# alpenlabs/dv-pari

Hardware: AMD Instinct MI355X
Metric: R1CS constraints/sec (prove) (higher is better)
Workload: dtype u32; 1 GPU; Proof::prove, synthetic dense R1CS, 2^20 constraints (BASELINE config #4); log2_constraints=20, n_wires=1048576, msm_pairs_per_proof=6291456, witness=resident in HBM, entry=dvp_prove_dev (Proof::prove with the witness resident), proofs_in_flight=1

## Files before the change

### dv-pari_amd/_native.py

```python
import ctypes as C
import os

import numpy as np

_HERE = os.path.dirname(os.path.abspath(__file__))
LIB_PATH = os.environ.get("DVP_LIB") or os.path.join(_HERE, "libdvpari_hip.so")

if not os.environ.get("DVP_NO_TORCH_PRELOAD"):
    try:
        import torch
    except Exception:
        pass

if not os.path.exists(LIB_PATH):
    raise ImportError(
        f"{LIB_PATH} is missing: build it with `python -c 'import __graft_entry__ as g; g.build()'` "
        "(hipcc --offload-arch=gfx950).  dv-pari_amd has no CPU fallback."
    )
lib = C.CDLL(LIB_PATH)

vp, u32, u64p, u8p, sz = C.c_void_p, C.c_uint32, C.c_void_p, C.c_void_p, C.c_size_t

_SIGS = {
    "dvp_strerror": (C.c_char_p, [C.c_int]),
    "dvp_version": (C.c_int, []),
    "dvp_device_count": (C.c_int, []),
    "dvp_set_device": (C.c_int, [C.c_int]),
    "dvp_set_devices": (C.c_int, [C.POINTER(C.c_int), C.c_int]),
    "dvp_points_sum_dev": (C.c_int, [vp, u32, vp, vp, vp]),
    "dvp_last_error_index": (C.c_int64, []),
    "dvp_tune_set": (C.c_int, [C.c_char_p, C.c_longlong]),
    "dvp_tune_get": (C.c_int, [C.c_char_p, C.POINTER(C.c_longlong)]),
    "dvp_tune_reset": (None, []),
    "dvp_ubench_gather": (C.c_int, [vp, C.c_size_t, C.c_int, C.POINTER(C.c_double)]),
    "dvp_prover_msm_table_ptr": (C.c_int, [vp, C.c_int, C.POINTER(vp), C.POINTER(C.c_uint64)]),
    "dvp_debug_ecfft_matrices": (C.c_int, [vp, C.c_int, C.c_int, u64p]),
    "dvp_debug_ecfft_layer": (C.c_int, [vp, u32, u64p]),
    "dvp_ubench_gf_mul": (C.c_int, [C.c_int, C.POINTER(C.c_double)]),
    "dvp_ubench_fr_mul": (C.c_int, [C.c_int, C.POINTER(C.c_double)]),
    "dvp_setup_scalars": (C.c_int, [u64p, u64p, u64p, u32, u32, u32, u32, u64p, u32, C.POINTER(vp), C.POINTER(vp), C.POINTER(vp), u64p, sz]),
    "dvp_debug_wave_trace": (C.c_int, [vp, u32]),
    "dvp_profile_enable": (None, [C.c_int]),
    "dvp_profile_reset": (None, []),
    "dvp_profile_read": (C.c_int, [C.c_char_p, C.POINTER(C.c_double), C.POINTER(C.c_uint64)]),
    "dvp_profile_round0_shapes": (C.c_int, [C.POINTER(C.c_uint64), C.POINTER(C.c_double), C.POINTER(C.c_uint64), C.c_int]),
    "dvp_ecfft_create": (C.c_int, [u32, C.c_int, u32, C.POINTER(vp)]),
    "dvp_ecfft_destroy": (None, [vp]),
    "dvp_ecfft_log2_leaves": (u32, [vp]),
    "dvp_ecfft_leaves": (C.c_int, [vp, u64p]),
    "dvp_ecfft_extend": (C.c_int, [vp, u64p, u32, u64p]),
    "dvp_ecfft_extend_dev": (C.c_int, [vp, vp, u32, vp, vp]),
    "dvp_ecfft_enter": (C.c_int, [vp, u64p, u64p]),
    "dvp_ecfft_exit": (C.c_int, [vp, u64p, u64p]),
    "dvp_ecfft_enter_dev": (C.c_int, [vp, vp, vp, vp]),
    "dvp_ecfft_exit_dev": (C.c_int, [vp, vp, vp, vp]),
    "dvp_ecfft_vanish_at": (C.c_int, [vp, C.c_int, u64p, u64p]),
    "dvp_fr_batch_inverse": (C.c_int, [u64p, sz]),
    "dvp_fr_batch_inverse_dev": (C.c_int, [vp, sz, vp]),
    "dvp_fr_vec_mul": (C.c_int, [u64p, u64p, sz, u64p]),
    "dvp_fr_vec_scale": (C.c_int, [u64p, u64p, sz, u64p]),
    "dvp_fr_vec_scalar_sub": (C.c_int, [u64p, u64p, sz, u64p]),
    "dvp_fr_vec_axpy": (C.c_int, [u64p, u64p, u64p, sz, u64p]),
    "dvp_fr_vec_dot": (C.c_int, [u64p, u64p, sz, u64p]),
    "dvp_fr_spmv": (C.c_int, [vp, vp, vp, u32, u64p, u32, u64p, u32, u64p]),
    "dvp_barycentric_eval": (C.c_int, [u64p, u64p, u64p, u64p, sz, u64p, u64p]),
    "dvp_msm_affine": (C.c_int, [u64p, u64p, u8p, sz, u64p, C.POINTER(C.c_int)]),
    "dvp_msm_affine_dev": (C.c_int, [vp, vp, vp, sz, vp, vp, vp]),
    "dvp_msm_ctx_create": (C.c_int, [u64p, u8p, sz, sz, C.POINTER(vp)]),
    "dvp_msm_ctx_destroy": (None, [vp]),
    "dvp_msm_ctx_plan": (C.c_int, [vp, C.POINTER(C.c_int), C.POINTER(C.c_int)]),
    "dvp_msm_ctx_table_bytes": (C.c_uint64, [vp, C.POINTER(C.c_int)]),
    "dvp_debug_recode_signed": (C.c_int, [vp, C.c_size_t, C.c_int, vp, C.POINTER(C.c_int)]),
    "dvp_msm_ctx_run": (C.c_int, [vp, u64p, sz, sz, u64p, C.POINTER(C.c_int)]),
    "dvp_msm_ctx_run_dev": (C.c_int, [vp, vp, sz, sz, vp, vp, vp]),
    "dvp_msm_xsk233": (C.c_int, [u8p, u8p, sz, u8p]),
    "dvp_mulgen_batch": (C.c_int, [u64p, sz, u8p]),
    "dvp_mulgen_batch_affine": (C.c_int, [u64p, sz, u64p, u8p]),
    "dvp_points_encode": (C.c_int, [u64p, u8p, sz, u8p]),
    "dvp_points_decode": (C.c_int, [u8p, sz, u64p, u8p]),
    "dvp_codec_set_rule": (C.c_int, [C.c_int]),
    "dvp_codec_get_rule": (C.c_int, []),
    "dvp_points_add": (C.c_int, [u64p, u8p, u64p, u8p, sz, u64p, u8p]),
    "dvp_prover_create": (C.c_int, [u32, u32, u32, C.POINTER(vp)]),
    "dvp_prover_destroy": (None, [vp]),
    "dvp_prover_set_coeffs": (C.c_int, [vp, u64p, u32]),
    "dvp_prover_set_matrix": (C.c_int, [vp, C.c_int, u32, vp, vp, vp]),
    "dvp_prover_set_srs_encoded": (C.c_int, [vp, C.c_int, u8p, sz]),
    "dvp_prover_set_srs_affine": (C.c_int, [vp, C.c_int, u64p, u8p, sz]),
    "dvp_prover_set_srs_affine_dev": (C.c_int, [vp, C.c_int, vp, vp, sz]),
    "dvp_prove": (C.c_int, [vp, u64p, u32, u64p, u32, u8p]),
    "dvp_prove_dev": (C.c_int, [vp, vp, u8p, vp]),
    "dvp_prove_begin": (C.c_int, [vp, vp, vp]),
    "dvp_prove_begin_partial": (C.c_int, [vp, vp, C.c_int, vp]),
    "dvp_prover_extend_count": (u32, [vp]),
    "dvp_prove_extend_vectors": (C.c_int, [vp, u32, vp]),
    "dvp_prover_extended_ptr": (C.c_int, [vp, u32, C.POINTER(vp)]),
    "dvp_prove_quotient": (C.c_int, [vp, vp]),
    "dvp_prove_mark_extended": (C.c_int, [vp, u32]),
    "dvp_prover_msm_size": (C.c_size_t, [vp, C.c_int]),
    "dvp_prover_msm_plan": (C.c_int, [vp, C.c_int, C.POINTER(C.c_int), C.POINTER(C.c_int)]),
    "dvp_prover_msm_table_bytes": (C.c_uint64, [vp, C.c_int, C.POINTER(C.c_int)]),
    "dvp_prover_msm_partial": (C.c_int, [vp, C.c_int, sz, sz, vp, vp, vp]),
    "dvp_prove_challenge": (C.c_int, [vp, vp, vp, vp]),
    "dvp_prove_challenge_partial": (C.c_int, [vp, vp, vp, C.c_size_t, C.c_size_t, C.c_size_t, C.c_size_t, vp, vp]),
    "dvp_prove_challenge_finish": (C.c_int, [vp, vp, C.c_uint32, C.c_size_t, C.c_size_t, vp]),
    "dvp_prove_finish": (C.c_int, [vp, vp, vp, u8p, vp]),
    "dvp_prover_debug_read": (C.c_int, [vp, C.c_char_p, u64p, sz]),
    "dvp_prover_debug_transcript_dev": (C.c_int, [vp, u8p, u64p, u32, u64p, u64p]),
    "dvp_prover_domains": (C.c_int, [vp, u64p, u64p]),
    "dvp_prover_domain_tables": (C.c_int, [vp, C.c_int, u64p, u64p]),
    "dvp_ecfft_domain_tables": (C.c_int, [vp, C.c_int, u64p, u64p]),
    "dvp_file_fr_vec_write": (C.c_int, [C.c_char_p, u64p, sz]),
    "dvp_file_fr_vec_read": (C.c_int, [C.c_char_p, u64p, sz, C.POINTER(C.c_size_t)]),
    "dvp_file_point_vec_write": (C.c_int, [C.c_char_p, u8p, sz]),
    "dvp_file_point_vec_read": (C.c_int, [C.c_char_p, u8p, sz, C.POINTER(C.c_size_t)]),
    "dvp_file_witness_read": (C.c_int, [C.c_char_p, u64p, sz, C.POINTER(C.c_size_t)]),
    "dvp_file_witness_write": (C.c_int, [C.c_char_p, u64p, sz]),
    "dvp_r1cs_dump_sizes": (C.c_int, [u8p, sz, C.POINTER(u32), C.POINTER(u32), C.POINTER(C.c_uint64 * 3), C.POINTER(u32)]),
    "dvp_r1cs_dump_fill": (C.c_int, [u8p, sz, u64p, C.POINTER(vp * 3), C.POINTER(vp * 3), C.POINTER(vp * 3)]),
    "dvp_fftr_sections": (C.c_int, [C.c_char_p, u32, u8p, u64p, C.POINTER(u32)]),
    "dvp_fftr_read_fr": (C.c_int, [C.c_char_p, u32, C.c_uint8, u64p, sz, C.POINTER(C.c_size_t)]),
    "dvp_fftr_write": (C.c_int, [C.c_char_p, u32, u8p, vp, u64p]),
    "dvp_setup_cache_dir": (C.c_int, [u64p, u64p, u64p, C.c_char_p, u32, C.c_int]),
    "dvp_setup_cache_dir_ex": (C.c_int, [u64p, u64p, u64p, C.c_char_p, u32, C.c_int, u64p, sz, C.POINTER(u32), C.POINTER(u32)]),
    "dvp_prover_prepares_precomputes": (C.c_int, [C.c_char_p, C.c_int, C.POINTER(u32)]),
    "dvp_ecfft_write_tree_file": (C.c_int, [vp, C.c_char_p]),
    "dvp_ecfft_check_tree_file": (C.c_int, [vp, C.c_char_p, C.c_int, C.POINTER(C.c_int), C.POINTER(C.c_int64)]),
    "dvp_prover_open_cache_dir": (C.c_int, [C.c_char_p, u32, C.POINTER(vp)]),
    "dvp_prove_cache_dir": (C.c_int, [C.c_char_p, u64p, u32, u64p, u32, u8p]),
    "dvp_cache_dir_release": (None, [C.c_char_p]),
    "dvp_cache_dir_prover": (C.c_int, [C.c_char_p, u32, C.POINTER(vp)]),
    "dvp_transcript_challenge": (C.c_int, [u8p, u64p, u32, u64p]),
    "dvp_blake3": (C.c_int, [u8p, sz, u8p]),
    "dvp_verify": (C.c_int, [u64p, u64p, u64p, u64p, u32, u8p, C.POINTER(C.c_int), C.POINTER(C.c_uint32)]),
    "dvp_verify_batch": (C.c_int, [u64p, u64p, u64p, u64p, u32, u8p, sz, u8p]),
    "dvp_verify_batch_dev": (C.c_int, [u64p, u64p, u64p, vp, u32, vp, sz, vp, vp]),
    "dvp_verify_batch_rlc": (C.c_int, [u64p, u64p, u64p, u64p, u32, u8p, sz, u8p, u8p, C.POINTER(C.c_uint32)]),
    "dvp_verify_batch_rlc_dev": (C.c_int, [u64p, u64p, u64p, vp, u32, vp, sz, u8p, vp, vp, vp]),
    "dvp_sp1_public_input": (C.c_int, [C.c_uint64, u64p]),
}
EXPORTED = []
for _name, (_res, _args) in _SIGS.items():
    try:
        _f = getattr(lib, _name)
    except AttributeError:
        continue
    _f.restype, _f.argtypes = _res, _args
    EXPORTED.append(_name)


class DvpError(RuntimeError):
    def __init__(self, status, where=""):
        self.status = status
        self.index = lib.dvp_last_error_index()
        super().__init__(f"{where}: {lib.dvp_strerror(status).decode()} (status {status}, index {self.index})")


def check(status, where=""):
    if status != 0:
        raise DvpError(status, where)


def set_devices(ids):
    ids = list(ids or [])
    arr = (C.c_int * max(len(ids), 1))(*ids)
    check(lib.dvp_set_devices(arr, len(ids)), "dvp_set_devices")


class tune:

    def __init__(self, **knobs):
        self.knobs = knobs
        self.saved = {}

    def __enter__(self):
        for k, v in self.knobs.items():
            old = C.c_longlong(0)
            check(lib.dvp_tune_get(k.encode(), C.byref(old)), f"dvp_tune_get({k})")
            self.saved[k] = old.value
            check(lib.dvp_tune_set(k.encode(), int(v)), f"dvp_tune_set({k})")
        return self

    def __exit__(self, *exc):
        for k, v in self.saved.items():
            lib.dvp_tune_set(k.encode(), v)
        self.saved = {}
        return False


def ints_to_limbs(vals, words=4) -> np.ndarray:
    out = np.empty((len(vals), words), dtype=np.uint64)
    buf = b"".join(int(v).to_bytes(8 * words, "little") for v in vals)
    out[:] = np.frombuffer(buf, dtype="<u8").reshape(len(vals), words)
    return out


def limbs_to_ints(arr) -> list:
    a = np.ascontiguousarray(arr, dtype="<u8")
    a = a.reshape(-1, a.shape[-1])
    w = a.shape[1] * 8
    raw = a.tobytes()
    return [int.from_bytes(raw[i * w:(i + 1) * w], "little") for i in range(a.shape[0])]


def ptr(a: np.ndarray):
    assert a.flags["C_CONTIGUOUS"]
    return a.ctypes.data_as(C.c_void_p)
```

### dv-pari_amd/csrc/capi.cpp

```cpp
#include "common.h"

#include <atomic>
#include <map>
#include <mutex>
#include <vector>
#include <cstring>
#include <cstdlib>

namespace dvp {
thread_local int64_t g_last_error_index = -1;
thread_local hipError_t g_last_hip_error = hipSuccess;

bool g_prof_enabled = false;
static unsigned g_prof_mask = ~0u;
static std::mutex g_prof_mu;
static double g_prof_ms[PROF_NSLOTS] = {0};
static uint64_t g_prof_n[PROF_NSLOTS] = {0};
struct Pending { int slot; hipEvent_t e0, e1; uint64_t key; };
struct Shape { double ms = 0; uint64_t n = 0; };
static std::map<uint64_t, Shape> g_prof_round0;
static std::vector<Pending> g_prof_pending;
static const char* kProfNames[PROF_NSLOTS] = {"msm_affine_round0", "msm_total", "extend_total", "prove_total", "msm_affine_rest", "msm_sort", "msm_tail"};

ProfScope::ProfScope(int slot_, hipStream_t st_, uint64_t key_) : slot(slot_), st(st_), key(key_) {
  if (!g_prof_enabled || slot_ < 0 || !((g_prof_mask >> slot_) & 1u)) return;
  if (hipEventCreate(&e0) != hipSuccess || hipEventCreate(&e1) != hipSuccess) { e0 = e1 = nullptr; return; }
  (void)hipEventRecord(e0, st);
}
void ProfScope::stop() {
  if (!e0) return;
  (void)hipEventRecord(e1, st);
  std::lock_guard<std::mutex> g(g_prof_mu);
  g_prof_pending.push_back({slot, e0, e1, key});
  e0 = e1 = nullptr;
}
void prof_collect() {
  std::lock_guard<std::mutex> g(g_prof_mu);
  for (auto& p : g_prof_pending) {
    float ms = 0;
    if (hipEventSynchronize(p.e1) == hipSuccess && hipEventElapsedTime(&ms, p.e0, p.e1) == hipSuccess) {
      g_prof_ms[p.slot] += ms;
      g_prof_n[p.slot] += (p.slot == PROF_MSM_AFFINE_REST && p.key) ? p.key : 1;
      if (p.slot == PROF_MSM_ACCUM_AFFINE && p.key) { Shape& sh = g_prof_round0[p.key]; sh.ms += ms; sh.n += 1; }
    }
    (void)hipEventDestroy(p.e0);
    (void)hipEventDestroy(p.e1);
  }
  g_prof_pending.clear();
}

static std::atomic<uint64_t> g_host_waits[2];
void count_host_wait(int kind) { g_host_waits[kind & 1].fetch_add(1, std::memory_order_relaxed); }

static void tune_from_env(Tune& t) {
  t = Tune();
  auto geti = [](const char* name, long long dflt) { const char* e = getenv(name); return e ? atoll(e) : dflt; };
  t.msm_c = geti("DVP_MSM_C", t.msm_c);
  t.msm_k = geti("DVP_MSM_K", t.msm_k);
  t.msm_fixed_c = geti("DVP_MSM_FIXED_C", t.msm_fixed_c);
  t.fx_hi = geti("DVP_FX_HI", t.fx_hi);
  const char* m = getenv("DVP_MSM_MODE");
  t.msm_proj = (m && !strcmp(m, "proj")) ? 1 : 0;
  t.msm_aff_min = geti("DVP_MSM_AFF_MIN", t.msm_aff_min);
  t.msm_hex_max = geti("DVP_MSM_HEX_MAX", t.msm_hex_max);
  t.msm_round_pipeline = geti("DVP_MSM_ROUND_PIPELINE", t.msm_round_pipeline);
  t.msm_sort_fused = geti("DVP_MSM_SORT_FUSED", t.msm_sort_fused);
  t.msm_bucket_pairs_max = geti("DVP_MSM_BUCKET_PAIRS_MAX", t.msm_bucket_pairs_max);
  t.msm_aff_bmax = geti("DVP_MSM_AFF_BMAX", t.msm_aff_bmax);
  t.msm_aff_bmin = geti("DVP_MSM_AFF_BMIN", t.msm_aff_bmin);
  t.ecfft_radix4 = geti("DVP_ECFFT_RADIX4", t.ecfft_radix4);
  t.ecfft_fold = geti("DVP_ECFFT_FOLD", t.ecfft_fold);
  t.msm_accum_fast = geti("DVP_MSM_ACCUM_FAST", t.msm_accum_fast);
  t.msm_tail_groups = geti("DVP_MSM_TAIL_GROUPS", t.msm_tail_groups);
  t.msm_accum_hex_max = geti("DVP_MSM_ACCUM_HEX_MAX", t.msm_accum_hex_max);
  t.gf_inv_tabs = geti("DVP_GF_INV_TABS", t.gf_inv_tabs);
  t.msm_ws_slots = geti("DVP_MSM_WS_SLOTS", t.msm_ws_slots);
  t.msm_gate_min = geti("DVP_MSM_GATE_MIN", t.msm_gate_min);
  t.msm_aff_tpb = geti("DVP_MSM_AFF_TPB", t.msm_aff_tpb);
  t.cache_replicas = geti("DVP_CACHE_REPLICAS", t.cache_replicas);
  t.msm_quad_max = geti("DVP_MSM_QUAD_MAX", t.msm_quad_max);
  t.msm_accum_quad_max = geti("DVP_MSM_ACCUM_QUAD_MAX", t.msm_accum_quad_max);
  t.msm_fixed_min = geti("DVP_MSM_FIXED_MIN", t.msm_fixed_min);
  t.horner_max_pub = geti("DVP_HORNER_MAX_PUB", t.horner_max_pub);
  t.fr_bi_shape = geti("DVP_FR_BI_SHAPE", t.fr_bi_shape);
  t.msm_aligned_signed = geti("DVP_MSM_ALIGNED_SIGNED", t.msm_aligned_signed);
  t.prove_host_transcript = geti("DVP_PROVE_HOST_TRANSCRIPT", t.prove_host_transcript);
}
static std::mutex g_dev_mu;
static std::vector<int> g_devices;
std::vector<int> mgpu_devices() {
  std::lock_guard<std::mutex> g(g_dev_mu);
  return g_devices;
}
Tune& tune() {
  static Tune t = [] { Tune x; tune_from_env(x); return x; }();
  return t;
}
}

static long long* tune_slot(const char* name) {
  dvp::Tune& t = dvp::tune();
  struct { const char* n; long long* v; } tab[] = {
      {"DVP_MSM_C", &t.msm_c}, {"DVP_MSM_K", &t.msm_k}, {"DVP_MSM_FIXED_C", &t.msm_fixed_c}, {"DVP_FX_HI", &t.fx_hi},
      {"DVP_MSM_PROJ", &t.msm_proj}, {"DVP_MSM_AFF_MIN", &t.msm_aff_min}, {"DVP_MSM_HEX_MAX", &t.msm_hex_max}, {"DVP_MSM_ROUND_PIPELINE", &t.msm_round_pipeline}, {"DVP_MSM_SORT_FUSED", &t.msm_sort_fused}, {"DVP_MSM_BUCKET_PAIRS_MAX", &t.msm_bucket_pairs_max}, {"DVP_MSM_AFF_BMAX", &t.msm_aff_bmax}, {"DVP_MSM_AFF_BMIN", &t.msm_aff_bmin}, {"DVP_ECFFT_RADIX4", &t.ecfft_radix4}, {"DVP_ECFFT_FOLD", &t.ecfft_fold}, {"DVP_MSM_ACCUM_FAST", &t.msm_accum_fast}, {"DVP_MSM_TAIL_GROUPS", &t.msm_tail_groups}, {"DVP_MSM_ACCUM_HEX_MAX", &t.msm_accum_hex_max}, {"DVP_GF_INV_TABS", &t.gf_inv_tabs}, {"DVP_MSM_WS_SLOTS", &t.msm_ws_slots}, {"DVP_MSM_GATE_MIN", &t.msm_gate_min}, {"DVP_MSM_AFF_TPB", &t.msm_aff_tpb}, {"DVP_CACHE_REPLICAS", &t.cache_replicas},
      {"DVP_MSM_QUAD_MAX", &t.msm_quad_max}, {"DVP_MSM_ACCUM_QUAD_MAX", &t.msm_accum_quad_max}, {"DVP_MSM_FIXED_MIN", &t.msm_fixed_min}, {"DVP_HORNER_MAX_PUB", &t.horner_max_pub}, {"DVP_FR_BI_SHAPE", &t.fr_bi_shape},
      {"DVP_MSM_ALIGNED_SIGNED", &t.msm_aligned_signed}, {"DVP_PROVE_HOST_TRANSCRIPT", &t.prove_host_transcript}};
  for (auto& e : tab)
    if (!strcmp(name, e.n)) return e.v;
  return nullptr;
}
extern "C" int dvp_tune_set(const char* name, long long value) {
  long long* v = name ? tune_slot(name) : nullptr;
  if (!v) return DVP_EINVAL;
  *v = value;
  return DVP_OK;
}
extern "C" int dvp_tune_get(const char* name, long long* value) {
  long long* v = name ? tune_slot(name) : nullptr;
  if (!v || !value) return DVP_EINVAL;
  *value = *v;
  return DVP_OK;
}
extern "C" void dvp_tune_reset(void) { dvp::tune_from_env(dvp::tune()); }

extern "C" void dvp_profile_enable(int on) {
  dvp::g_prof_mask = on == 2 ? (1u << dvp::PROF_MSM_ACCUM_AFFINE) : ~0u;
  dvp::g_prof_enabled = on != 0;
}
extern "C" void dvp_profile_reset(void) {
  dvp::prof_collect();
  std::lock_guard<std::mutex> g(dvp::g_prof_mu);
  for (int i = 0; i < dvp::PROF_NSLOTS; ++i) { dvp::g_prof_ms[i] = 0; dvp::g_prof_n[i] = 0; }
  dvp::g_prof_round0.clear();
  dvp::g_host_waits[0] = 0;
  dvp::g_host_waits[1] = 0;
}
extern "C" int dvp_profile_round0_shapes(uint64_t* pairs, double* total_ms, uint64_t* launches, int cap) {
  if (cap < 0 || (cap > 0 && (!pairs || !total_ms || !launches))) return DVP_EINVAL;
  dvp::prof_collect();
  std::lock_guard<std::mutex> g(dvp::g_prof_mu);
  int k = 0;
  for (auto& e : dvp::g_prof_round0) {
    if (k < cap) { pairs[k] = e.first; total_ms[k] = e.second.ms; launches[k] = e.second.n; }
    ++k;
  }
  return k;
}
extern "C" int dvp_profile_read(const char* name, double* total_ms, uint64_t* launches) {
  if (!name || !total_ms || !launches) return DVP_EINVAL;
  if (!strcmp(name, "host_waits_stream") || !strcmp(name, "host_waits_side")) {
    *total_ms = 0;
    *launches = dvp::g_host_waits[name[11] == 's' && name[12] == 'i' ? 1 : 0].load();
    return DVP_OK;
  }
  dvp::prof_collect();
  std::lock_guard<std::mutex> g(dvp::g_prof_mu);
  for (int i = 0; i < dvp::PROF_NSLOTS; ++i)
    if (!strcmp(name, dvp::kProfNames[i])) { *total_ms = dvp::g_prof_ms[i]; *launches = dvp::g_prof_n[i]; return DVP_OK; }
  return DVP_EINVAL;
}

extern "C" const char* dvp_strerror(int s) {
  switch (s) {
    case DVP_OK: return "ok";
    case DVP_EINVAL: return "invalid argument (size, null pointer or non-canonical field element)";
    case DVP_EDECODE: return "invalid xsk233 point encoding";
    case DVP_EUNSAT: return "R1CS constraint not satisfied by the witness";
    case DVP_EHIP: return "HIP runtime error";
    case DVP_EIO: return "I/O error";
    case DVP_ENOMEM: return "out of memory";
    case DVP_ECHALLENGE: return "Fiat-Shamir challenge lies in the evaluation domain";
    default: return "unknown status";
  }
}

extern "C" int dvp_version(void) { return 100; }

extern "C" int dvp_device_count(void) {
  int n = 0;
  hipError_t e = hipGetDeviceCount(&n);
  if (e != hipSuccess) return DVP_EHIP;
  return n;
}

extern "C" int dvp_set_devices(const int* ids, int n) {
  int cnt = 0;
  DVP_HIP(hipGetDeviceCount(&cnt));
  if (n < 0 || n > 64 || (n > 0 && !ids)) return DVP_EINVAL;
  for (int i = 0; i < n; ++i)
    if (ids[i] < 0 || ids[i] >= cnt) return DVP_EINVAL;
  std::lock_guard<std::mutex> g(dvp::g_dev_mu);
  dvp::g_devices.assign(ids, ids + (n > 1 ? n : 0));
  return DVP_OK;
}

extern "C" int dvp_set_device(int id) {
  DVP_HIP(hipSetDevice(id));
  return DVP_OK;
}

extern "C" int64_t dvp_last_error_index(void) { return dvp::g_last_error_index; }
```

### dv-pari_amd/csrc/common.h

```cpp
#pragma once
#include <hip/hip_runtime.h>
#include <stdint.h>
#include <stdio.h>

#include <vector>

#include "../../include/dvpari_internal.h"

namespace dvp {

extern thread_local int64_t g_last_error_index;
extern thread_local hipError_t g_last_hip_error;

inline int hip_fail(hipError_t e, const char* what, const char* file, int line) {
  g_last_hip_error = e;
  fprintf(stderr, "[dvpari] HIP error %d (%s) at %s:%d: %s\n", (int)e, hipGetErrorString(e), file, line, what);
  return DVP_EHIP;
}

#define DVP_HIP(call)                                                        \
  do {                                                                       \
    hipError_t _e = (call);                                                  \
    if (_e != hipSuccess) return ::dvp::hip_fail(_e, #call, __FILE__, __LINE__); \
  } while (0)

#define DVP_TRY(call)        \
  do {                       \
    int _s = (call);         \
    if (_s != DVP_OK) return _s; \
  } while (0)

struct DevBuf {
  void* p = nullptr;
  size_t bytes = 0;
  DevBuf() = default;
  DevBuf(const DevBuf&) = delete;
  DevBuf& operator=(const DevBuf&) = delete;
  ~DevBuf() { release(); }
  int alloc(size_t n) {
    release();
    if (n == 0) n = 16;
    hipError_t e = hipMalloc(&p, n);
    if (e != hipSuccess) {
      p = nullptr;
      return hip_fail(e, "hipMalloc", __FILE__, __LINE__);
    }
    bytes = n;
    return DVP_OK;
  }
  void release() {
    if (p) (void)hipFree(p);
    p = nullptr;
    bytes = 0;
  }
  template <class T>
  T* as() const {
    return reinterpret_cast<T*>(p);
  }
};

struct Tune {
  long long msm_c = 0;
  long long msm_k = 0;
  long long msm_fixed_c = 0;
  long long fx_hi = -1;
  long long msm_proj = 0;
  long long msm_aff_min = 1ll << 19;
  long long msm_gate_min = 1;
  long long msm_ws_slots = 2;
  long long cache_replicas = 1;
  long long msm_aff_tpb = 256;
  long long msm_aff_bmin = 8;
  long long msm_aff_bmax = 136;
  long long ecfft_radix4 = 3;
  long long ecfft_fold = 1;
  long long msm_accum_fast = 1;
  long long msm_tail_groups = 1;
  long long msm_accum_hex_max = -1;
  long long gf_inv_tabs = 1;
  long long msm_accum_quad_max = 0;
  long long msm_bucket_pairs_max = 12;
  long long msm_sort_fused = 1;
  long long msm_round_pipeline = 2;
  long long msm_hex_max = -1;
  long long msm_quad_max = 0;
  long long msm_fixed_min = 1ll << 16;
  long long fr_bi_shape = 6;
  long long horner_max_pub = -1;
  long long prove_host_transcript = 0;
  long long msm_aligned_signed = 1;
};
Tune& tune();

std::vector<int> mgpu_devices();

inline unsigned cdiv(size_t a, size_t b) { return (unsigned)((a + b - 1) / b); }

enum ProfSlot { PROF_MSM_ACCUM_AFFINE = 0, PROF_MSM_TOTAL, PROF_EXTEND_TOTAL, PROF_PROVE_TOTAL, PROF_MSM_AFFINE_REST, PROF_MSM_SORT, PROF_MSM_TAIL, PROF_NSLOTS };
extern bool g_prof_enabled;
struct ProfScope {
  int slot;
  hipStream_t st;
  hipEvent_t e0 = nullptr, e1 = nullptr;
  uint64_t key = 0;
  ProfScope(int slot_, hipStream_t st_, uint64_t key_ = 0);
  void stop();
};
void prof_collect();
void count_host_wait(int kind);

}
```

### dv-pari_amd/csrc/msm.hip

```cpp
#include <algorithm>
#include <cstdlib>
#include <cstring>
#include <atomic>
#include <chrono>
#include <mutex>
#include <type_traits>
#include <vector>

#include "common.h"
#include "k233.cuh"
#include "tau.cuh"
#include "codec.cuh"

namespace dvp {

constexpr uint32_t FXW_VALID = 0x80000000u, FXW_KEY_MASK = 0xfffffu, FXW_NEG = 0x10000000u, ITEM_NEG = 0x80000000u;
constexpr int FXW_ROW_SHIFT = 20;
__host__ __device__ __forceinline__ uint32_t fxw_key(uint32_t d) { return d & FXW_KEY_MASK; }
__host__ __device__ __forceinline__ uint32_t fxw_row(uint32_t d) { return (d >> FXW_ROW_SHIFT) & 0xffu; }

template <class DIGIT>
__global__ void __launch_bounds__(256)
k_recode(const uint32_t* __restrict__ scalars, const uint8_t* __restrict__ inf, uint32_t n, int c, int W, int n_narrow,
         DIGIT* __restrict__ digits, unsigned long long* __restrict__ err) {
  uint32_t i = blockIdx.x * blockDim.x + threadIdx.x;
  if (i >= n) return;
  uint32_t s[8];
#pragma unroll
  for (int k = 0; k < 8; ++k) s[k] = scalars[(size_t)i * 8 + k];
  bool skip = inf && inf[i];
  if (!tau_scalar_is_canonical(s)) {
    atomicMin(err, (unsigned long long)i);
    skip = true;
  }
  uint32_t r0[5], r1[5];
  tau_partial_reduce(s, r0, r1);
  if (skip) {
#pragma unroll
    for (int k = 0; k < 5; ++k) r0[k] = r1[k] = 0;
  }
  const int total = W * c - n_narrow;
  uint64_t buf = 0;
  int nb = 0, w = 0, width = n_narrow > 0 ? c - 1 : c;
  for (int done = 0; done < total; done += 16) {
    buf |= (uint64_t)tau_step16(r0, r1) << nb;
    nb += 16;
    while (nb >= width && w < W) {
      const uint32_t dv = (uint32_t)(buf & ((1ull << width) - 1));
      if (sizeof(DIGIT) == 4)
        digits[(size_t)w * n + i] = (DIGIT)(dv ? (FXW_VALID | ((uint32_t)w << FXW_ROW_SHIFT) | dv) : 0u);
      else
        digits[(size_t)w * n + i] = (DIGIT)dv;
      buf >>= width;
      nb -= width;
      ++w;
      width = w < n_narrow ? c - 1 : c;
    }
  }
  uint32_t rest = (uint32_t)buf | (uint32_t)(buf >> 32);
#pragma unroll
  for (int k = 0; k < 5; ++k) rest |= r0[k] | r1[k];
  if (rest) atomicMin(err, (unsigned long long)i | (1ull << 62));
}

template <class F>
__device__ __forceinline__ uint32_t fx_recode_signed_each(const uint32_t* s , int c, int W, int n_narrow, F&& f) {
  uint32_t carry = 0;
  int bit = 0;
#pragma unroll 1
  for (int w = 0; w < W; ++w) {
    const int width = w < n_narrow ? c - 1 : c;
    const uint32_t half = 1u << (width - 1), mask = (1u << width) - 1;
    const int wd = bit >> 5, sh = bit & 31;
    uint32_t lo = wd < 8 ? s[wd] : 0u, hi = wd + 1 < 9 ? s[wd + 1] : 0u;
    uint32_t d = (uint32_t)((((uint64_t)hi << 32) | lo) >> sh) & mask;
    bit += width;
    d += carry;
    carry = 0;
    uint32_t word = 0;
    if (d > mask) {
      carry = 1;
    } else if (d > half) {
      carry = 1;
      d = (1u << width) - d;
      word = FXW_VALID | FXW_NEG | ((uint32_t)w << FXW_ROW_SHIFT) | d;
    } else if (d) {
      word = FXW_VALID | ((uint32_t)w << FXW_ROW_SHIFT) | (d & ((1u << (c - 1)) - 1));
    }
    f(w, word);
  }
  return carry;
}
__device__ __forceinline__ bool fx_load_scalar(const uint32_t* __restrict__ scalars, const uint8_t* __restrict__ inf, uint32_t i, uint32_t* s,
                                               unsigned long long* __restrict__ err, bool report) {
#pragma unroll
  for (int k = 0; k < 8; ++k) s[k] = scalars[(size_t)i * 8 + k];
  s[8] = 0;
  bool skip = inf && inf[i];
  if (!tau_scalar_is_canonical(s)) {
    if (report) atomicMin(err, (unsigned long long)i);
    skip = true;
  }
  return !skip;
}
__global__ void __launch_bounds__(256)
k_recode_signed(const uint32_t* __restrict__ scalars, const uint8_t* __restrict__ inf, uint32_t n, int c, int W, int n_narrow,
                uint32_t* __restrict__ words, unsigned long long* __restrict__ err) {
  uint32_t i = blockIdx.x * blockDim.x + threadIdx.x;
  if (i >= n) return;
  uint32_t s[9];
  const bool live = fx_load_scalar(scalars, inf, i, s, err, true);
  const uint32_t carry = fx_recode_signed_each(s, c, W, n_narrow, [&](int w, uint32_t word) { words[(size_t)w * n + i] = live ? word : 0u; });
  if (carry && live) atomicMin(err, (unsigned long long)i | (1ull << 62));
}

constexpr int SCAN_TPB = 256, SCAN_EPT = 4, SCAN_BLK = SCAN_TPB * SCAN_EPT;

template <int NW>
__device__ __forceinline__ uint32_t block_scan_waves(uint32_t v, uint32_t* total, uint32_t* sh) {
  const int t = threadIdx.x, lane = t & 63, w = t >> 6;
  uint32_t x = v;
#pragma unroll
  for (int o = 1; o < 64; o <<= 1) {
    const uint32_t y = (uint32_t)__shfl_up((int)x, o);
    if (lane >= o) x += y;
  }
  if (lane == 63) sh[w] = x;
  __syncthreads();
  if (w == 0) {
    uint32_t z = lane < NW ? sh[lane] : 0u;
#pragma unroll
    for (int o = 1; o < NW; o <<= 1) {
      const uint32_t y = (uint32_t)__shfl_up((int)z, o);
      if (lane >= o) z += y;
    }
    if (lane < NW) sh[16 + lane] = z;
  }
  __syncthreads();
  const uint32_t base = w ? sh[16 + w - 1] : 0u;
  *total = sh[16 + NW - 1];
  __syncthreads();
  return base + x - v;
}
__device__ __forceinline__ uint32_t block_exclusive_scan(uint32_t v, uint32_t* total, uint32_t* sh) {
  return block_scan_waves<SCAN_TPB / 64>(v, total, sh);
}

template <bool PAD2>
__global__ void __launch_bounds__(SCAN_TPB) k_scan_local(const uint32_t* __restrict__ in, uint32_t* __restrict__ out,
                                                         uint32_t* __restrict__ bsum, uint32_t m) {
  __shared__ uint32_t sh[SCAN_TPB];
  uint32_t base = blockIdx.x * SCAN_BLK + threadIdx.x * SCAN_EPT;
  uint32_t v[SCAN_EPT], s = 0;
#pragma unroll
  for (int k = 0; k < SCAN_EPT; ++k) {
    v[k] = (base + k < m) ? in[base + k] : 0;
    if (PAD2) v[k] = (v[k] + 1u) & ~1u;
    s += v[k];
  }
  uint32_t tot;
  uint32_t ex = block_exclusive_scan(s, &tot, sh);
#pragma unroll
  for (int k = 0; k < SCAN_EPT; ++k) {
    if (base + k < m) out[base + k] = ex;
    ex += v[k];
  }
  if (threadIdx.x == 0) bsum[blockIdx.x] = tot;
}

__global__ void __launch_bounds__(SCAN_TPB) k_scan_local_div(const uint32_t* __restrict__ in, uint32_t K, uint32_t* __restrict__ vout,
                                                             uint32_t* __restrict__ out, uint32_t* __restrict__ bsum, uint32_t m) {
  __shared__ uint32_t sh[SCAN_TPB];
  uint32_t base = blockIdx.x * SCAN_BLK + threadIdx.x * SCAN_EPT;
  uint32_t v[SCAN_EPT], s = 0;
#pragma unroll
  for (int k = 0; k < SCAN_EPT; ++k) {
    v[k] = (base + k < m) ? (in[base + k] + K - 1) / K : 0;
    if (base + k < m) vout[base + k] = v[k];
    s += v[k];
  }
  uint32_t tot;
  uint32_t ex = block_exclusive_scan(s, &tot, sh);
#pragma unroll
  for (int k = 0; k < SCAN_EPT; ++k) {
    if (base + k < m) out[base + k] = ex;
    ex += v[k];
  }
  if (threadIdx.x == 0) bsum[blockIdx.x] = tot;
}

__global__ void __launch_bounds__(SCAN_TPB) k_scan_bsums(uint32_t* __restrict__ bsum, uint32_t nb, uint32_t* total_out) {
  __shared__ uint32_t sh[SCAN_TPB];
  uint32_t carry = 0;
  for (uint32_t base = 0; base < nb; base += SCAN_TPB) {
    uint32_t idx = base + threadIdx.x;
    uint32_t v = idx < nb ? bsum[idx] : 0;
    uint32_t tot;
    uint32_t ex = block_exclusive_scan(v, &tot, sh);
    if (idx < nb) bsum[idx] = ex + carry;
    carry += tot;
  }
  if (threadIdx.x == 0) *total_out = carry;
}

__global__ void __launch_bounds__(SCAN_TPB) k_scan_add(uint32_t* __restrict__ out, const uint32_t* __restrict__ bsum, uint32_t m) {
  uint32_t base = blockIdx.x * SCAN_BLK + threadIdx.x * SCAN_EPT;
  uint32_t add = bsum[blockIdx.x];
#pragma unroll
  for (int k = 0; k < SCAN_EPT; ++k)
    if (base + k < m) out[base + k] += add;
}

constexpr uint32_t SCAN_FOLD_NB = 64;
__global__ void __launch_bounds__(SCAN_TPB) k_scan_add_fold(uint32_t* __restrict__ out, const uint32_t* __restrict__ bsum_raw, uint32_t m,
                                                           uint32_t* __restrict__ total_out) {
  uint32_t add = 0;
  for (uint32_t b = 0; b < blockIdx.x; ++b) add += bsum_raw[b];
  const uint32_t base = blockIdx.x * SCAN_BLK + threadIdx.x * SCAN_EPT;
#pragma unroll
  for (int k = 0; k < SCAN_EPT; ++k)
    if (base + k < m) out[base + k] += add;
  if (blockIdx.x == gridDim.x - 1 && threadIdx.x == 0) *total_out = add + bsum_raw[blockIdx.x];
}

static int scan_exclusive(const uint32_t* in, uint32_t* out, uint32_t m, uint32_t* bsum, hipStream_t st, bool pad2 = false) {
  uint32_t nb = cdiv(m, SCAN_BLK);
  if (pad2)
    hipLaunchKernelGGL(k_scan_local<true>, dim3(nb), dim3(SCAN_TPB), 0, st, in, out, bsum, m);
  else
    hipLaunchKernelGGL(k_scan_local<false>, dim3(nb), dim3(SCAN_TPB), 0, st, in, out, bsum, m);
  if (nb <= SCAN_FOLD_NB)
    hipLaunchKernelGGL(k_scan_add_fold, dim3(nb), dim3(SCAN_TPB), 0, st, out, bsum, m, out + m);
  else {
    hipLaunchKernelGGL(k_scan_bsums, dim3(1), dim3(SCAN_TPB), 0, st, bsum, nb, out + m);
    hipLaunchKernelGGL(k_scan_add, dim3(nb), dim3(SCAN_TPB), 0, st, out, bsum, m);
  }
  DVP_HIP(hipGetLastError());
  return DVP_OK;
}

static int scan_exclusive_div(const uint32_t* in, uint32_t K, uint32_t* vout, uint32_t* out, uint32_t m, uint32_t* bsum, hipStream_t st) {
  uint32_t nb = cdiv(m, SCAN_BLK);
  hipLaunchKernelGGL(k_scan_local_div, dim3(nb), dim3(SCAN_TPB), 0, st, in, K, vout, out, bsum, m);
  if (nb <= SCAN_FOLD_NB)
    hipLaunchKernelGGL(k_scan_add_fold, dim3(nb), dim3(SCAN_TPB), 0, st, out, bsum, m, out + m);
  else {
    hipLaunchKernelGGL(k_scan_bsums, dim3(1), dim3(SCAN_TPB), 0, st, bsum, nb, out + m);
    hipLaunchKernelGGL(k_scan_add, dim3(nb), dim3(SCAN_TPB), 0, st, out, bsum, m);
  }
  DVP_HIP(hipGetLastError());
  return DVP_OK;
}

constexpr uint32_t SORT_CHUNK = 32768;
constexpr int SORT_TPB = 1024;

__global__ void __launch_bounds__(SORT_TPB)
k_hist_local(const uint16_t* __restrict__ digits, uint32_t n, int c, uint16_t* __restrict__ hist) {
  extern __shared__ uint32_t lds_cnt[];
  const uint32_t chunk = blockIdx.x, w = blockIdx.y, nb = 1u << c, nchunks = gridDim.x;
  for (uint32_t k = threadIdx.x; k < (nb >> 1); k += SORT_TPB) lds_cnt[k] = 0;
  __syncthreads();
  uint32_t lo = chunk * SORT_CHUNK, hi = min(n, lo + SORT_CHUNK);
  const uint16_t* dg = digits + (size_t)w * n;
  for (uint32_t i = lo + threadIdx.x; i < hi; i += SORT_TPB) {
    uint32_t d = dg[i];
    if (d) atomicAdd(&lds_cnt[d >> 1], 1u << (16 * (d & 1)));
  }
  __syncthreads();
  uint32_t* out = (uint32_t*)(hist + ((size_t)w * nchunks + chunk) * nb);
  for (uint32_t k = threadIdx.x; k < (nb >> 1); k += SORT_TPB) out[k] = lds_cnt[k];
}

__global__ void __launch_bounds__(256)
k_hist_scan(const uint16_t* __restrict__ hist, uint32_t nchunks, int c, int W, uint32_t* __restrict__ chunk_off,
            uint32_t* __restrict__ cnt) {
  uint32_t key = blockIdx.x * blockDim.x + threadIdx.x;
  uint32_t nb = 1u << c;
  if (key >= ((uint32_t)W << c)) return;
  uint32_t w = key >> c, b = key & (nb - 1);
  uint32_t run = 0;
  for (uint32_t ch = 0; ch < nchunks; ++ch) {
    size_t idx = ((size_t)w * nchunks + ch) * nb + b;
    uint32_t v = hist[idx];
    chunk_off[idx] = run;
    run += v;
  }
  cnt[key] = run;
}

__global__ void __launch_bounds__(SORT_TPB)
k_scatter_local(const uint16_t* __restrict__ digits, uint32_t n, int c, const uint32_t* __restrict__ off,
                const uint32_t* __restrict__ chunk_off, uint32_t* __restrict__ items) {
  extern __shared__ uint32_t lds_cur[];
  const uint32_t chunk = blockIdx.x, w = blockIdx.y, nb = 1u << c, nchunks = gridDim.x;
  const uint32_t* co = chunk_off + ((size_t)w * nchunks + chunk) * nb;
  const uint32_t* of = off + ((size_t)w << c);
  for (uint32_t k = threadIdx.x; k < nb; k += SORT_TPB) lds_cur[k] = of[k] + co[k];
  __syncthreads();
  uint32_t lo = chunk * SORT_CHUNK, hi = min(n, lo + SORT_CHUNK);
  const uint16_t* dg = digits + (size_t)w * n;
  for (uint32_t i = lo + threadIdx.x; i < hi; i += SORT_TPB) {
    uint32_t d = dg[i];
    if (d) items[atomicAdd(&lds_cur[d], 1u)] = i;
  }
}

constexpr int FX_C_MAX = 20, FX_NP_MAX = 1 << (FX_C_MAX / 2);
constexpr uint32_t FX_CHUNK = 8192;
struct FxBits {
  int lo, hi;
  __host__ __device__ uint32_t np() const { return 1u << hi; }
};

__global__ void __launch_bounds__(SORT_TPB)
k_part_hist(const uint32_t* __restrict__ digits, size_t total, FxBits fb, uint32_t* __restrict__ phist) {
  __shared__ uint32_t h[FX_NP_MAX];
  const uint32_t FX_NP = fb.np();
  const int FX_LO = fb.lo;
  for (uint32_t k = threadIdx.x; k < FX_NP; k += SORT_TPB) h[k] = 0;
  __syncthreads();
  size_t lo = (size_t)blockIdx.x * FX_CHUNK, hi = min(total, lo + FX_CHUNK);
  for (size_t e = lo + threadIdx.x; e < hi; e += SORT_TPB) {
    uint32_t d = digits[e];
    if (d) atomicAdd(&h[fxw_key(d) >> FX_LO], 1u);
  }
  __syncthreads();
  for (uint32_t k = threadIdx.x; k < FX_NP; k += SORT_TPB) phist[(size_t)blockIdx.x * FX_NP + k] = h[k];
}
constexpr uint32_t FX_SCAN_CB = 32;
__global__ void __launch_bounds__(256)
k_part_scan_chunks(const uint32_t* __restrict__ phist, uint32_t nblk, FxBits fb, uint32_t* __restrict__ pbase, uint32_t* __restrict__ ctot, uint32_t nch) {
  const uint32_t FX_NP = fb.np();
  const uint32_t ch = blockIdx.x, b0 = ch * FX_SCAN_CB, b1 = min(nblk, b0 + FX_SCAN_CB);
  for (uint32_t part = threadIdx.x; part < FX_NP; part += 256) {
    uint32_t run = 0;
#pragma unroll 8
    for (uint32_t b = b0; b < b1; ++b) {
      const uint32_t v = phist[(size_t)b * FX_NP + part];
      pbase[(size_t)b * FX_NP + part] = run;
      run += v;
    }
    ctot[(size_t)part * nch + ch] = run;
  }
}
__global__ void __launch_bounds__(256)
k_part_scan_totals(uint32_t* __restrict__ ctot, uint32_t nch, FxBits fb, uint32_t* __restrict__ pcount) {
  const uint32_t part = (blockIdx.x * 256 + threadIdx.x) >> 6, lane = threadIdx.x & 63u;
  if (part >= fb.np()) return;
  uint32_t* row = ctot + (size_t)part * nch;
  uint32_t carry = 0;
  for (uint32_t base = 0; base < nch; base += 64) {
    const uint32_t idx = base + lane;
    const uint32_t v = idx < nch ? row[idx] : 0;
    uint32_t x = v;
#pragma unroll
    for (int o = 1; o < 64; o <<= 1) {
      const uint32_t y = __shfl_up(x, o);
      if ((int)lane >= o) x += y;
    }
    if (idx < nch) row[idx] = carry + x - v;
    carry += __shfl(x, 63);
  }
  if (lane == 0) pcount[part] = carry;
}
__global__ void __launch_bounds__(FX_NP_MAX)
k_part_starts(const uint32_t* __restrict__ pcount, FxBits fb, uint32_t* __restrict__ pstart, uint32_t* __restrict__ cstart) {
  __shared__ uint32_t sp[FX_NP_MAX], sc[FX_NP_MAX];
  const uint32_t FX_NP = fb.np(), t = threadIdx.x;
  uint32_t pc = t < FX_NP ? pcount[t] : 0, cc = (pc + FX_CHUNK - 1) / FX_CHUNK;
  sp[t] = pc;
  sc[t] = cc;
  __syncthreads();
  for (uint32_t o = 1; o < FX_NP_MAX; o <<= 1) {
    uint32_t a = t >= o ? sp[t - o] : 0, b = t >= o ? sc[t - o] : 0;
    __syncthreads();
    sp[t] += a;
    sc[t] += b;
    __syncthreads();
  }
  if (t < FX_NP) {
    pstart[t] = sp[t] - pc;
    cstart[t] = sc[t] - cc;
  }
  if (t == FX_NP - 1) {
    pstart[FX_NP] = sp[t];
    cstart[FX_NP] = sc[t];
  }
}
__global__ void __launch_bounds__(SORT_TPB)
k_part_scatter(const uint32_t* __restrict__ digits, size_t total, uint32_t n, uint32_t n_total, uint32_t i0, FxBits fb,
               const uint32_t* __restrict__ pbase, const uint32_t* __restrict__ cbase, uint32_t nch, const uint32_t* __restrict__ pstart,
               uint16_t* __restrict__ plo, uint32_t* __restrict__ pid) {
  __shared__ uint32_t cur[FX_NP_MAX];
  const uint32_t FX_NP = fb.np();
  const int FX_LO = fb.lo;
  const uint32_t ch = blockIdx.x / FX_SCAN_CB;
  for (uint32_t k = threadIdx.x; k < FX_NP; k += SORT_TPB) cur[k] = pstart[k] + cbase[(size_t)k * nch + ch] + pbase[(size_t)blockIdx.x * FX_NP + k];
  __syncthreads();
  size_t lo = (size_t)blockIdx.x * FX_CHUNK, hi = min(total, lo + FX_CHUNK);
  for (size_t e = lo + threadIdx.x; e < hi; e += SORT_TPB) {
    uint32_t d = digits[e];
    if (!d) continue;
    const uint32_t i = (uint32_t)(e % n), key = fxw_key(d);
    uint32_t pos = atomicAdd(&cur[key >> FX_LO], 1u);
    plo[pos] = (uint16_t)(key & ((1u << FX_LO) - 1));
    pid[pos] = (fxw_row(d) * n_total + i0 + i) | ((d & FXW_NEG) ? ITEM_NEG : 0u);
  }
}
__device__ __forceinline__ uint32_t fx_chunk_partition(const uint32_t* __restrict__ cstart, uint32_t FX_NP, uint32_t g) {
  uint32_t lo = 0, hi = FX_NP;
  while (hi - lo > 1) {
    uint32_t mid = (lo + hi) >> 1;
    if (cstart[mid] <= g) lo = mid; else hi = mid;
  }
  return lo;
}
__global__ void __launch_bounds__(SORT_TPB)
k_hist_local2(const uint16_t* __restrict__ plo, const uint32_t* __restrict__ pstart, const uint32_t* __restrict__ cstart, FxBits fb,
              uint16_t* __restrict__ hist) {
  extern __shared__ uint32_t lds_cnt[];
  const uint32_t FX_NP = fb.np();
  const uint32_t g = blockIdx.x, nb = 1u << fb.lo;
  if (g >= cstart[FX_NP]) return;
  for (uint32_t k = threadIdx.x; k < (nb >> 1); k += SORT_TPB) lds_cnt[k] = 0;
  __syncthreads();
  uint32_t hi = fx_chunk_partition(cstart, FX_NP, g);
  uint32_t lo_e = pstart[hi] + (g - cstart[hi]) * FX_CHUNK, hi_e = min(pstart[hi + 1], lo_e + FX_CHUNK);
  auto count = [&](uint32_t d) { atomicAdd(&lds_cnt[d >> 1], 1u << (16 * (d & 1))); };
  const uint32_t body_lo = min(hi_e, (lo_e + 7u) & ~7u), body_hi = max(body_lo, hi_e & ~7u);
  for (uint32_t j = lo_e + threadIdx.x; j < body_lo; j += SORT_TPB) count(plo[j]);
  for (uint32_t j = body_lo + 8u * threadIdx.x; j < body_hi; j += 8u * SORT_TPB) {
    const uint4 v = *(const uint4*)(plo + j);
    count(v.x & 0xffffu); count(v.x >> 16); count(v.y & 0xffffu); count(v.y >> 16);
    count(v.z & 0xffffu); count(v.z >> 16); count(v.w & 0xffffu); count(v.w >> 16);
  }
  for (uint32_t j = body_hi + threadIdx.x; j < hi_e; j += SORT_TPB) count(plo[j]);
  __syncthreads();
  uint32_t* out = (uint32_t*)(hist + (size_t)g * nb);
  for (uint32_t k = threadIdx.x; k < (nb >> 1); k += SORT_TPB) out[k] = lds_cnt[k];
}
__global__ void __launch_bounds__(256)
k_hist_scan2(const uint16_t* __restrict__ hist, const uint32_t* __restrict__ cstart, FxBits fb, uint32_t* __restrict__ chunk_off,
             uint32_t* __restrict__ cnt) {
  uint32_t key = blockIdx.x * blockDim.x + threadIdx.x;
  if (key >= (1u << (fb.lo + fb.hi))) return;
  const uint32_t nb = 1u << fb.lo;
  uint32_t hi = key >> fb.lo, b = key & (nb - 1);
  uint32_t run = 0;
  for (uint32_t g = cstart[hi]; g < cstart[hi + 1]; ++g) {
    size_t idx = (size_t)g * nb + b;
    uint32_t v = hist[idx];
    chunk_off[idx] = run;
    run += v;
  }
  cnt[key] = run;
}
__global__ void __launch_bounds__(SORT_TPB)
k_scatter_local2(const uint16_t* __restrict__ plo, const uint32_t* __restrict__ pid, const uint32_t* __restrict__ pstart,
                 const uint32_t* __restrict__ cstart, FxBits fb, const uint32_t* __restrict__ off, const uint32_t* __restrict__ chunk_off,
                 uint32_t* __restrict__ items) {
  extern __shared__ uint32_t lds_cur[];
  const uint32_t FX_NP = fb.np();
  const int FX_LO = fb.lo;
  const uint32_t g = blockIdx.x, nb = 1u << FX_LO;
  if (g >= cstart[FX_NP]) return;
  uint32_t hi = fx_chunk_partition(cstart, FX_NP, g);
  const uint32_t* co = chunk_off + (size_t)g * nb;
  const uint32_t* of = off + ((size_t)hi << FX_LO);
  for (uint32_t k = threadIdx.x; k < nb; k += SORT_TPB) lds_cur[k] = of[k] + co[k];
  __syncthreads();
  uint32_t lo_e = pstart[hi] + (g - cstart[hi]) * FX_CHUNK, hi_e = min(pstart[hi + 1], lo_e + FX_CHUNK);
  for (uint32_t j = lo_e + threadIdx.x; j < hi_e; j += SORT_TPB) items[atomicAdd(&lds_cur[plo[j]], 1u)] = pid[j];
}

__device__ __forceinline__ uint32_t block_scan_tpb(uint32_t v, uint32_t* sh, uint32_t* total) {
  return block_scan_waves<SORT_TPB / 64>(v, total, sh);
}
constexpr unsigned FX_STAGE1_LDS = (2 * FX_NP_MAX + SORT_TPB + 2 * FX_CHUNK) * 4;
constexpr unsigned FX_STAGE2_LDS = (2 * FX_NP_MAX + SORT_TPB + FX_CHUNK) * 4 + FX_CHUNK * 2;

__global__ void __launch_bounds__(SORT_TPB)
k_part_scatter_staged(const uint32_t* __restrict__ digits, size_t total, uint32_t n, uint32_t n_total, uint32_t i0, FxBits fb,
                      const uint32_t* __restrict__ phist, const uint32_t* __restrict__ pbase, const uint32_t* __restrict__ cbase, uint32_t nch,
                      const uint32_t* __restrict__ pstart, uint16_t* __restrict__ plo, uint32_t* __restrict__ pid) {
  extern __shared__ uint32_t lds_st[];
  uint32_t* cur = lds_st;
  uint32_t* gdst = cur + FX_NP_MAX;
  uint32_t* sh = gdst + FX_NP_MAX;
  uint32_t* st_d = sh + SORT_TPB;
  uint32_t* st_id = st_d + FX_CHUNK;
  const uint32_t FX_NP = fb.np(), t = threadIdx.x;
  const int FX_LO = fb.lo;
  const size_t hb = (size_t)blockIdx.x * FX_NP;
  uint32_t h = t < FX_NP ? phist[hb + t] : 0, tot;
  uint32_t ex = block_scan_tpb(h, sh, &tot);
  if (t < FX_NP) {
    cur[t] = ex;
    gdst[t] = pstart[t] + cbase[(size_t)t * nch + blockIdx.x / FX_SCAN_CB] + pbase[hb + t] - ex;
  }
  __syncthreads();
  const size_t lo = (size_t)blockIdx.x * FX_CHUNK, hi = min(total, lo + FX_CHUNK);
  const uint32_t w0 = (uint32_t)(lo / n);
  for (size_t e = lo + t; e < hi; e += SORT_TPB) {
    uint32_t d = digits[e];
    if (!d) continue;
    size_t i = e - (size_t)w0 * n;
    while (i >= n) i -= n;
    const uint32_t key = fxw_key(d);
    uint32_t pos = atomicAdd(&cur[key >> FX_LO], 1u);
    st_d[pos] = key;
    st_id[pos] = (fxw_row(d) * n_total + i0 + (uint32_t)i) | ((d & FXW_NEG) ? ITEM_NEG : 0u);
  }
  __syncthreads();
  const uint32_t mask = (1u << FX_LO) - 1;
  for (uint32_t pos = t; pos < tot; pos += SORT_TPB) {
    uint32_t d = st_d[pos], dst = gdst[d >> FX_LO] + pos;
    plo[dst] = (uint16_t)(d & mask);
    pid[dst] = st_id[pos];
  }
}

__global__ void __launch_bounds__(SORT_TPB)
k_part_hist_signed(const uint32_t* __restrict__ scalars, const uint8_t* __restrict__ inf, uint32_t n, int c, int W, int n_narrow, uint32_t S,
                   FxBits fb, uint32_t* __restrict__ phist, unsigned long long* __restrict__ err) {
  __shared__ uint32_t h[FX_NP_MAX];
  const uint32_t FX_NP = fb.np();
  const int FX_LO = fb.lo;
  for (uint32_t k = threadIdx.x; k < FX_NP; k += SORT_TPB) h[k] = 0;
  __syncthreads();
  const uint32_t lo = blockIdx.x * S, hi = min(n, lo + S);
  for (uint32_t i = lo + threadIdx.x; i < hi; i += SORT_TPB) {
    uint32_t s[9];
    if (!fx_load_scalar(scalars, inf, i, s, err, true)) continue;
    const uint32_t carry = fx_recode_signed_each(s, c, W, n_narrow, [&](int, uint32_t word) {
      if (word) atomicAdd(&h[fxw_key(word) >> FX_LO], 1u);
    });
    if (carry) atomicMin(err, (unsigned long long)i | (1ull << 62));
  }
  __syncthreads();
  for (uint32_t k = threadIdx.x; k < FX_NP; k += SORT_TPB) phist[(size_t)blockIdx.x * FX_NP + k] = h[k];
}
template <bool STAGED>
__global__ void __launch_bounds__(SORT_TPB)
k_part_scatter_signed(const uint32_t* __restrict__ scalars, const uint8_t* __restrict__ inf, uint32_t n, int c, int W, int n_narrow, uint32_t S,
                      uint32_t n_total, uint32_t i0, FxBits fb, const uint32_t* __restrict__ phist, const uint32_t* __restrict__ pbase,
                      const uint32_t* __restrict__ cbase, uint32_t nch, const uint32_t* __restrict__ pstart, uint16_t* __restrict__ plo,
                      uint32_t* __restrict__ pid) {
  extern __shared__ uint32_t lds_st[];
  uint32_t* cur = lds_st;
  uint32_t* gdst = cur + FX_NP_MAX;
  uint32_t* sh = gdst + FX_NP_MAX;
  uint32_t* st_d = sh + SORT_TPB;
  uint32_t* st_id = st_d + FX_CHUNK;
  const uint32_t FX_NP = fb.np(), t = threadIdx.x;
  const int FX_LO = fb.lo;
  const size_t hb = (size_t)blockIdx.x * FX_NP;
  const uint32_t mask = (1u << FX_LO) - 1;
  uint32_t tot = 0;
  const uint32_t ch = blockIdx.x / FX_SCAN_CB;
  if (STAGED) {
    uint32_t h = t < FX_NP ? phist[hb + t] : 0;
    uint32_t ex = block_scan_tpb(h, sh, &tot);
    if (t < FX_NP) {
      cur[t] = ex;
      gdst[t] = pstart[t] + cbase[(size_t)t * nch + ch] + pbase[hb + t] - ex;
    }
  } else {
    for (uint32_t k = t; k < FX_NP; k += SORT_TPB) cur[k] = pstart[k] + cbase[(size_t)k * nch + ch] + pbase[hb + k];
  }
  __syncthreads();
  const uint32_t lo = blockIdx.x * S, hi = min(n, lo + S);
  for (uint32_t i = lo + t; i < hi; i += SORT_TPB) {
    uint32_t s[9];
    if (!fx_load_scalar(scalars, inf, i, s, nullptr, false)) continue;
    fx_recode_signed_each(s, c, W, n_narrow, [&](int w, uint32_t word) {
      if (!word) return;
      const uint32_t key = fxw_key(word);
      const uint32_t id = ((uint32_t)w * n_total + i0 + i) | ((word & FXW_NEG) ? ITEM_NEG : 0u);
      const uint32_t pos = atomicAdd(&cur[key >> FX_LO], 1u);
      if (STAGED) {
        st_d[pos] = key;
        st_id[pos] = id;
      } else {
        plo[pos] = (uint16_t)(key & mask);
        pid[pos] = id;
      }
    });
  }
  if (!STAGED) return;
  __syncthreads();
  for (uint32_t pos = t; pos < tot; pos += SORT_TPB) {
    uint32_t d = st_d[pos], dst = gdst[d >> FX_LO] + pos;
    plo[dst] = (uint16_t)(d & mask);
    pid[dst] = st_id[pos];
  }
}

__global__ void __launch_bounds__(SORT_TPB)
k_scatter_local2_staged(const uint16_t* __restrict__ plo, const uint32_t* __restrict__ pid, const uint32_t* __restrict__ pstart,
                        const uint32_t* __restrict__ cstart, FxBits fb, const uint32_t* __restrict__ off,
                        const uint32_t* __restrict__ chunk_off, const uint16_t* __restrict__ hist, uint32_t* __restrict__ items) {
  extern __shared__ uint32_t lds_st[];
  uint32_t* cur = lds_st;
  uint32_t* gdst = cur + FX_NP_MAX;
  uint32_t* sh = gdst + FX_NP_MAX;
  uint32_t* st_id = sh + SORT_TPB;
  uint16_t* st_b = (uint16_t*)(st_id + FX_CHUNK);
  const uint32_t FX_NP = fb.np(), t = threadIdx.x;
  const int FX_LO = fb.lo;
  const uint32_t g = blockIdx.x, nb = 1u << FX_LO;
  if (g >= cstart[FX_NP]) return;
  const uint32_t hi = fx_chunk_partition(cstart, FX_NP, g);
  uint32_t h = t < nb ? hist[(size_t)g * nb + t] : 0, tot;
  uint32_t ex = block_scan_tpb(h, sh, &tot);
  if (t < nb) {
    cur[t] = ex;
    gdst[t] = off[((size_t)hi << FX_LO) + t] + chunk_off[(size_t)g * nb + t] - ex;
  }
  __syncthreads();
  const uint32_t lo_e = pstart[hi] + (g - cstart[hi]) * FX_CHUNK, hi_e = min(pstart[hi + 1], lo_e + FX_CHUNK);
  auto place = [&](uint32_t b, uint32_t id) {
    const uint32_t pos = atomicAdd(&cur[b], 1u);
    st_id[pos] = id;
    st_b[pos] = (uint16_t)b;
  };
  const uint32_t body_lo = min(hi_e, (lo_e + 7u) & ~7u), body_hi = max(body_lo, hi_e & ~7u);
  for (uint32_t j = lo_e + t; j < body_lo; j += SORT_TPB) place(plo[j], pid[j]);
  for (uint32_t j = body_lo + 8u * t; j < body_hi; j += 8u * SORT_TPB) {
    const uint4 k = *(const uint4*)(plo + j), a = *(const uint4*)(pid + j), c = *(const uint4*)(pid + j + 4);
    place(k.x & 0xffffu, a.x); place(k.x >> 16, a.y); place(k.y & 0xffffu, a.z); place(k.y >> 16, a.w);
    place(k.z & 0xffffu, c.x); place(k.z >> 16, c.y); place(k.w & 0xffffu, c.z); place(k.w >> 16, c.w);
  }
  for (uint32_t j = body_hi + t; j < hi_e; j += SORT_TPB) place(plo[j], pid[j]);
  __syncthreads();
  for (uint32_t pos = t; pos < tot; pos += SORT_TPB) items[gdst[st_b[pos]] + pos] = st_id[pos];
}

__global__ void __launch_bounds__(256)
k_frob_table(const Aff* __restrict__ bases, uint32_t n, int FX_C, int FX_W, int n_narrow, Aff* __restrict__ table) {
  uint32_t i = blockIdx.x * blockDim.x + threadIdx.x;
  if (i >= n) return;
  Aff p = bases[i];
  table[i] = p;
#pragma unroll 1
  for (int w = 1; w < FX_W; ++w) {
    int width = (w - 1) < n_narrow ? FX_C - 1 : FX_C;
    p.x = gf_sqr_n(p.x, width);
    p.y = gf_sqr_n(p.y, width);
    table[(size_t)w * n + i] = p;
  }
}

__global__ void __launch_bounds__(256) __attribute__((amdgpu_waves_per_eu(3, 3)))
k_dbl_table(const Aff* __restrict__ bases, uint32_t n, int c, int W, int n_narrow, GfSqrTables T, Aff* __restrict__ table, Gf* __restrict__ zs,
            Gf* __restrict__ pre) {
  extern __shared__ char lds_raw[];
  GfLdsK L = gf_ldsk_init(lds_raw);
  uint32_t i = blockIdx.x * blockDim.x + threadIdx.x;
  if (i >= n) return;
  const Aff p0 = bases[i];
  table[i] = p0;
  Ld p = ld_from_aff(p0);
  Gf run = gf_one();
#pragma unroll 1
  for (int w = 1; w < W; ++w) {
    const int width = (w - 1) < n_narrow ? c - 1 : c;
#pragma unroll 1
    for (int k = 0; k < width; ++k) p = ld_dbl(p, L);
    Aff raw;
    raw.x = p.X;
    raw.y = p.Y;
    table[(size_t)w * n + i] = raw;
    zs[(size_t)(w - 1) * n + i] = p.Z;
    pre[(size_t)(w - 1) * n + i] = run;
    run = gf_mul(run, p.Z, L);
  }
  Gf inv = gf_inv_fast(run, T, L);
#pragma unroll 1
  for (int w = W - 1; w >= 1; --w) {
    const Gf z = zs[(size_t)(w - 1) * n + i];
    Gf zi, inv_next;
    gf_mul2(pre[(size_t)(w - 1) * n + i], z, inv, L, zi, inv_next);
    inv = inv_next;
    Aff a = table[(size_t)w * n + i];
    a.x = gf_mul(a.x, zi, L);
    a.y = gf_mul(a.y, gf_sqr(zi), L);
    table[(size_t)w * n + i] = a;
  }
}

constexpr int EC_TPB = 256;
constexpr unsigned EC_LDS = (EC_TPB / 64) * GF_LDSK_BYTES_PER_WAVE;
constexpr unsigned EC_LDS_Q = (EC_TPB / 64) * GF_LDS_BYTES_PER_WAVE;
constexpr uint32_t MERGE_HEX_MAX = 8192;
constexpr uint32_t MERGE_QUAD_MAX = 16384;

template <class LT> struct MergeMul;
template <> struct MergeMul<GfLdsK> { static __device__ __forceinline__ GfLdsK init(char* l) { return gf_ldsk_init(l); } static __device__ __forceinline__ bool lead(const GfLdsK&) { return true; } };
template <> struct MergeMul<GfLdsQ> { static __device__ __forceinline__ GfLdsQ init(char* l) { return gf_ldsq_init(l); } static __device__ __forceinline__ bool lead(const GfLdsQ& c) { return c.r == 0; } };
template <> struct MergeMul<GfLdsH> { static __device__ __forceinline__ GfLdsH init(char* l) { return gf_ldsh_init(l); } static __device__ __forceinline__ bool lead(const GfLdsH& c) { return c.r == 0; } };
__device__ __forceinline__ uint32_t find_key(const uint32_t* __restrict__ toff, uint32_t nkeys, uint32_t tid) {
  uint32_t lo = 0, hi = nkeys;
  while (hi - lo > 1) {
    uint32_t mid = (lo + hi) >> 1;
    if (toff[mid] <= tid) lo = mid; else hi = mid;
  }
  return lo;
}

constexpr uint32_t ACCUM_QUAD_MAX = 49152;
constexpr uint32_t ACCUM_HEX_MAX = 32768;
template <bool INDIRECT, bool QUAD>
__global__ void __launch_bounds__(EC_TPB) __attribute__((amdgpu_waves_per_eu(2, 2)))
k_accum_affine(const Aff* __restrict__ bases, const uint32_t* __restrict__ items, const uint32_t* __restrict__ cnt,
               const uint32_t* __restrict__ off, const uint32_t* __restrict__ toff, uint32_t nkeys, uint32_t K,
               Ld* __restrict__ out, uint32_t sign_mask) {
  extern __shared__ char lds_raw[];
  uint32_t tid = blockIdx.x * blockDim.x + threadIdx.x;
  if (QUAD) tid >>= 2;
  if (tid >= toff[nkeys]) return;
  uint32_t key = find_key(toff, nkeys, tid);
  uint32_t j = tid - toff[key];
  uint32_t start = off[key] + j * K;
  uint32_t len = min(K, cnt[key] - j * K);
  auto item_point = [&](uint32_t v) -> Aff {
    Aff q = bases[v & ~sign_mask];
    if (v & sign_mask) q.y = gf_add(q.y, q.x);
    return q;
  };
  Aff first = INDIRECT ? item_point(items[start]) : bases[start];
  Ld acc = (!INDIRECT && gf_is_zero(first.x)) ? ld_infinity() : ld_from_aff(first);
  if (QUAD) {
    GfLdsQ L = gf_ldsq_init(lds_raw);
#pragma unroll 1
    for (uint32_t t = 1; t < len; ++t) {
      Aff q = INDIRECT ? item_point(items[start + t]) : bases[start + t];
      if (!INDIRECT && gf_is_zero(q.x)) continue;
      ld_madd_ip(acc, q, L);
    }
    if (L.r == 0) out[tid] = acc;
  } else {
    GfLdsK L = gf_ldsk_init(lds_raw);
#pragma unroll 1
    for (uint32_t t = 1; t < len; ++t) {
      Aff q = INDIRECT ? item_point(items[start + t]) : bases[start + t];
      if (!INDIRECT && gf_is_zero(q.x)) continue;
      ld_madd_ip(acc, q, L);
    }
    out[tid] = acc;
  }
}

template <bool INDIRECT, bool QUAD>
__global__ void __launch_bounds__(EC_TPB) __attribute__((amdgpu_waves_per_eu(2, 2)))
k_accum_affine_fast(const Aff* __restrict__ bases, const uint32_t* __restrict__ items, const uint32_t* __restrict__ cnt,
                    const uint32_t* __restrict__ off, const uint32_t* __restrict__ toff, uint32_t nkeys, uint32_t K,
                    Ld* __restrict__ out, uint32_t sign_mask, uint32_t* __restrict__ rest_n, uint32_t* __restrict__ rest) {
  extern __shared__ char lds_raw[];
  using LT = typename std::conditional<QUAD, GfLdsQ, GfLdsK>::type;
  LT L = MergeMul<LT>::init(lds_raw);
  uint32_t tid = blockIdx.x * blockDim.x + threadIdx.x;
  if (QUAD) tid >>= 2;
  if (tid >= toff[nkeys]) return;
  const uint32_t key = find_key(toff, nkeys, tid);
  const uint32_t j = tid - toff[key];
  const uint32_t start = off[key] + j * K;
  const uint32_t len = min(K, cnt[key] - j * K);
  auto point = [&](uint32_t t) -> Aff {
    if (!INDIRECT) return bases[start + t];
    const uint32_t v = items[start + t];
    Aff q = bases[v & ~sign_mask];
    if (v & sign_mask) q.y = gf_add(q.y, q.x);
    return q;
  };
  const Aff first = point(0);
  bool ok = INDIRECT || !gf_is_zero(first.x);
  Ld acc = ld_from_aff(first);
  if (ok && len > 1) {
    const Aff q = point(1);
    ok = (INDIRECT || !gf_is_zero(q.x)) && !gf_eq(first.x, q.x);
    if (ok) ld_add_aff_aff(first, q, acc, L);
  }
#pragma unroll 1
  for (uint32_t t = 2; t < len && ok; ++t) {
    const Aff q = point(t);
    if (!INDIRECT && gf_is_zero(q.x)) continue;
    ok = ld_madd_fast(acc, q, L);
  }
  if (!MergeMul<LT>::lead(L)) return;
  if (ok)
    out[tid] = acc;
  else
    rest[atomicAdd(rest_n, 1u)] = tid;
}
template <bool INDIRECT>
__global__ void __launch_bounds__(EC_TPB) __attribute__((amdgpu_waves_per_eu(2, 2)))
k_accum_affine_rest(const Aff* __restrict__ bases, const uint32_t* __restrict__ items, const uint32_t* __restrict__ cnt,
                    const uint32_t* __restrict__ off, const uint32_t* __restrict__ toff, uint32_t nkeys, uint32_t K,
                    Ld* __restrict__ out, uint32_t sign_mask, const uint32_t* __restrict__ rest_n, const uint32_t* __restrict__ rest) {
  extern __shared__ char lds_raw[];
  GfLdsK L = gf_ldsk_init(lds_raw);
  const uint32_t r = blockIdx.x * blockDim.x + threadIdx.x;
  if (r >= *rest_n) return;
  const uint32_t tid = rest[r];
  const uint32_t key = find_key(toff, nkeys, tid);
  const uint32_t j = tid - toff[key];
  const uint32_t start = off[key] + j * K;
  const uint32_t len = min(K, cnt[key] - j * K);
  auto point = [&](uint32_t t) -> Aff {
    if (!INDIRECT) return bases[start + t];
    const uint32_t v = items[start + t];
    Aff q = bases[v & ~sign_mask];
    if (v & sign_mask) q.y = gf_add(q.y, q.x);
    return q;
  };
  const Aff first = point(0);
  Ld acc = (!INDIRECT && gf_is_zero(first.x)) ? ld_infinity() : ld_from_aff(first);
#pragma unroll 1
  for (uint32_t t = 1; t < len; ++t) {
    const Aff q = point(t);
    if (!INDIRECT && gf_is_zero(q.x)) continue;
    ld_madd_ip(acc, q, L);
  }
  out[tid] = acc;
}

template <int GROUP>
__global__ void __launch_bounds__(EC_TPB) __attribute__((amdgpu_waves_per_eu(2, 2)))
k_accum_proj(const Ld* __restrict__ in, const uint32_t* __restrict__ cnt, const uint32_t* __restrict__ off,
             const uint32_t* __restrict__ toff, uint32_t nkeys, uint32_t K, Ld* __restrict__ out) {
  extern __shared__ char lds_raw[];
  uint32_t tid = blockIdx.x * blockDim.x + threadIdx.x;
  tid /= (uint32_t)GROUP;
  if (tid >= toff[nkeys]) return;
  uint32_t key = find_key(toff, nkeys, tid);
  uint32_t j = tid - toff[key];
  uint32_t start = off[key] + j * K;
  uint32_t len = min(K, cnt[key] - j * K);
  Ld acc = in[start];
  using LT = typename std::conditional<GROUP == 16, GfLdsH, typename std::conditional<GROUP == 4, GfLdsQ, GfLdsK>::type>::type;
  LT L = MergeMul<LT>::init(lds_raw);
#pragma unroll 1
  for (uint32_t t = 1; t < len; ++t) {
    if (!ld_add_nodbl(acc, in[start + t], L)) {
      acc = in[start + t];
      acc = ld_dbl(acc, L);
    }
  }
  if (MergeMul<LT>::lead(L)) out[tid] = acc;
}

__global__ void __launch_bounds__(EC_TPB) __attribute__((amdgpu_waves_per_eu(2, 2)))
k_bucket_pairs(const Aff* __restrict__ pts, const uint32_t* __restrict__ cnt, const uint32_t* __restrict__ off, uint32_t nkeys,
               Ld* __restrict__ A, uint32_t* __restrict__ rest_n, uint32_t* __restrict__ rest) {
  extern __shared__ char lds_raw[];
  GfLdsK L = gf_ldsk_init(lds_raw);
  const uint32_t key = blockIdx.x * blockDim.x + threadIdx.x;
  if (key >= nkeys) return;
  const uint32_t c = cnt[key];
  if (c == 0) {
    A[key] = ld_infinity();
    return;
  }
  const uint32_t o = off[key];
  const Aff p = pts[o];
  if (c == 1) {
    A[key] = gf_is_zero(p.x) ? ld_infinity() : ld_from_aff(p);
    return;
  }
  Aff q = pts[o + 1];
  bool ok = !(gf_is_zero(p.x) || gf_is_zero(q.x) || gf_eq(p.x, q.x));
  Ld r;
  if (ok) {
    ld_add_aff_aff(p, q, r, L);
#pragma unroll 1
    for (uint32_t t = 2; t < c && ok; ++t) {
      q = pts[o + t];
      if (gf_is_zero(q.x)) continue;
      ok = ld_madd_fast(r, q, L);
    }
  }
  if (ok)
    A[key] = r;
  else
    rest[atomicAdd(rest_n, 1u)] = key;
}
__global__ void __launch_bounds__(EC_TPB) __attribute__((amdgpu_waves_per_eu(2, 2)))
k_bucket_rest(const Aff* __restrict__ pts, const uint32_t* __restrict__ cnt, const uint32_t* __restrict__ off,
              const uint32_t* __restrict__ rest_n, const uint32_t* __restrict__ rest, Ld* __restrict__ A) {
  extern __shared__ char lds_raw[];
  GfLdsK L = gf_ldsk_init(lds_raw);
  const uint32_t tid = blockIdx.x * blockDim.x + threadIdx.x;
  if (tid >= *rest_n) return;
  const uint32_t key = rest[tid];
  const uint32_t c = cnt[key], o = off[key];
  const Aff first = pts[o];
  Ld acc = gf_is_zero(first.x) ? ld_infinity() : ld_from_aff(first);
#pragma unroll 1
  for (uint32_t t = 1; t < c; ++t) {
    const Aff q = pts[o + t];
    if (gf_is_zero(q.x)) continue;
    ld_madd_ip(acc, q, L);
  }
  A[key] = acc;
}

__global__ void __launch_bounds__(256)
k_build_sqr_tables(Gf* __restrict__ tabs ) {
  uint32_t tid = blockIdx.x * blockDim.x + threadIdx.x;
  if (tid >= 6 * 30 * 256) return;
  uint32_t which = tid / (30 * 256), e = tid - which * 30 * 256, pos = e >> 8, byte = e & 255;
  Gf v = gf_zero();
  v.w[pos >> 2] = byte << (8 * (pos & 3));
  if (pos == 29) v.w[7] &= 0x1FFu;
  if (which == 3) {
    tabs[tid] = gf_halftrace(v);
    return;
  }
  const int k = which == 0 ? 29 : which == 1 ? 58 : which == 2 ? 116 : which == 4 ? 14 : 7;
  tabs[tid] = gf_sqr_n(v, k);
}
static std::mutex g_sqr_mu;
static Gf* g_sqr_tab[16] = {nullptr};
int gf_sqr_tables(GfSqrTables* out, hipStream_t st) {
  int dev;
  DVP_HIP(hipGetDevice(&dev));
  if (dev < 0 || dev >= 16) return DVP_EINVAL;
  std::lock_guard<std::mutex> g(g_sqr_mu);
  if (!g_sqr_tab[dev]) {
    Gf* t;
    DVP_HIP(hipMalloc((void**)&t, (size_t)6 * 30 * 256 * sizeof(Gf)));
    hipLaunchKernelGGL(k_build_sqr_tables, dim3(cdiv(6 * 30 * 256, 256)), dim3(256), 0, st, t);
    DVP_HIP(hipGetLastError());
    DVP_HIP(hipStreamSynchronize(st));
    g_sqr_tab[dev] = t;
  }
  out->t29 = g_sqr_tab[dev];
  out->t58 = g_sqr_tab[dev] + 30 * 256;
  out->t116 = g_sqr_tab[dev] + 2 * 30 * 256;
  out->th = g_sqr_tab[dev] + 3 * 30 * 256;
  const long long tabs = tune().gf_inv_tabs;
  out->t14 = tabs >= 1 ? g_sqr_tab[dev] + 4 * 30 * 256 : nullptr;
  out->t7 = tabs >= 2 ? g_sqr_tab[dev] + 5 * 30 * 256 : nullptr;
  return DVP_OK;
}

constexpr uint32_t AFF_NONE = 0xffffffffu;
constexpr uint32_t DESC_PAIR = 0x80000000u;

__global__ void __launch_bounds__(256)
k_post_sort(uint32_t* __restrict__ items, const uint32_t* __restrict__ cnt, const uint32_t* __restrict__ off , uint32_t nkeys,
            uint32_t* __restrict__ ocnt, uint32_t* __restrict__ ooff , uint32_t* __restrict__ d_max) {
  const uint32_t k = blockIdx.x * blockDim.x + threadIdx.x;
  uint32_t m = 0;
  if (k <= nkeys) {
    const uint32_t o = off[k];
    ooff[k] = o >> 1;
    if (k < nkeys) {
      const uint32_t c = cnt[k];
      if (c & 1) items[o + c] = AFF_NONE;
      ocnt[k] = (c + 1) >> 1;
      m = c;
    }
  }
  for (int o = 32; o > 0; o >>= 1) m = max(m, (uint32_t)__shfl_xor((int)m, o));
  if ((threadIdx.x & 63) == 0 && m) atomicMax(d_max, m);
}
__global__ void __launch_bounds__(256)
k_round0_offsets(const uint32_t* __restrict__ cnt, const uint32_t* __restrict__ off , uint32_t nkeys,
                 uint32_t* __restrict__ ocnt, uint32_t* __restrict__ ooff ) {
  uint32_t k = blockIdx.x * blockDim.x + threadIdx.x;
  if (k > nkeys) return;
  ooff[k] = off[k] >> 1;
  if (k < nkeys) ocnt[k] = (cnt[k] + 1) >> 1;
}

__global__ void __launch_bounds__(SCAN_TPB) k_mscan_local(const uint32_t* __restrict__ cnt0, uint32_t m, int R, uint32_t* __restrict__ rp,
                                                          uint32_t* __restrict__ bs ) {
  __shared__ uint32_t sh[SCAN_TPB];
  const uint32_t base = blockIdx.x * SCAN_BLK + threadIdx.x * SCAN_EPT;
  uint32_t v[SCAN_EPT];
#pragma unroll
  for (int k = 0; k < SCAN_EPT; ++k) v[k] = (base + k < m) ? cnt0[base + k] : 0;
  {
    uint32_t mx = 0;
#pragma unroll
    for (int k = 0; k < SCAN_EPT; ++k) mx = max(mx, v[k]);
    for (int d = 32; d > 0; d >>= 1) mx = max(mx, (uint32_t)__shfl_xor((int)mx, d));
    if ((threadIdx.x & 63) == 0) sh[threadIdx.x >> 6] = mx;
    __syncthreads();
    if (threadIdx.x == 0) {
      for (int w = 1; w < SCAN_TPB / 64; ++w) mx = max(mx, sh[w]);
      bs[(size_t)R * gridDim.x + blockIdx.x] = mx;
    }
    __syncthreads();
  }
  for (int r = 1; r <= R; ++r) {
    uint32_t* c = rp + (size_t)(2 * (r - 1)) * ((size_t)m + 1);
    uint32_t* o = c + ((size_t)m + 1);
    uint32_t s = 0;
#pragma unroll
    for (int k = 0; k < SCAN_EPT; ++k) {
      v[k] = (v[k] + 1u) >> 1;
      s += v[k];
    }
    uint32_t tot;
    uint32_t ex = block_exclusive_scan(s, &tot, sh);
#pragma unroll
    for (int k = 0; k < SCAN_EPT; ++k) {
      if (base + k < m) {
        c[base + k] = v[k];
        o[base + k] = ex;
      }
      ex += v[k];
    }
    if (threadIdx.x == 0) bs[(size_t)(r - 1) * gridDim.x + blockIdx.x] = tot;
  }
}
__global__ void __launch_bounds__(SCAN_TPB) k_mscan_bsums(uint32_t* __restrict__ bs, uint32_t nb, uint32_t m, uint32_t* __restrict__ rp,
                                                          uint32_t* __restrict__ off0 ,
                                                          uint32_t* __restrict__ dmax ) {
  __shared__ uint32_t sh[SCAN_TPB];
  const int r = blockIdx.x + 1;
  uint32_t* row = bs + (size_t)(r - 1) * nb;
  uint32_t carry = 0;
  for (uint32_t base = 0; base < nb; base += SCAN_TPB) {
    uint32_t idx = base + threadIdx.x;
    uint32_t v = idx < nb ? row[idx] : 0;
    uint32_t tot;
    uint32_t ex = block_exclusive_scan(v, &tot, sh);
    if (idx < nb) row[idx] = ex + carry;
    carry += tot;
  }
  if (threadIdx.x == 0) {
    rp[(size_t)(2 * (r - 1) + 1) * ((size_t)m + 1) + m] = carry;
    if (r == 1 && off0) off0[m] = 2u * carry;
  }
  if (r == 1 && dmax) {
    const uint32_t* bm = bs + (size_t)gridDim.x * nb;
    uint32_t mx = 0;
    for (uint32_t i = threadIdx.x; i < nb; i += SCAN_TPB) mx = max(mx, bm[i]);
    for (int d = 32; d > 0; d >>= 1) mx = max(mx, (uint32_t)__shfl_xor((int)mx, d));
    __syncthreads();
    if ((threadIdx.x & 63) == 0) sh[threadIdx.x >> 6] = mx;
    __syncthreads();
    if (threadIdx.x == 0) {
      for (int w = 1; w < SCAN_TPB / 64; ++w) mx = max(mx, sh[w]);
      *dmax = mx;
    }
  }
}
__global__ void __launch_bounds__(SCAN_TPB) k_mscan_add(uint32_t* __restrict__ rp, const uint32_t* __restrict__ bs, uint32_t m, int R,
                                                        const uint32_t* __restrict__ cnt0, uint32_t* __restrict__ off0, uint32_t* __restrict__ items) {
  const uint32_t base = blockIdx.x * SCAN_BLK + threadIdx.x * SCAN_EPT;
  for (int r = 1; r <= R; ++r) {
    uint32_t* o = rp + (size_t)(2 * (r - 1) + 1) * ((size_t)m + 1);
    const uint32_t add = bs[(size_t)(r - 1) * gridDim.x + blockIdx.x];
    if (r == 1 && off0) {
#pragma unroll
      for (int k = 0; k < SCAN_EPT; ++k)
        if (base + k < m) {
          const uint32_t v = o[base + k] + add, c = cnt0[base + k];
          o[base + k] = v;
          off0[base + k] = 2u * v;
          if (c & 1u) items[2u * v + c] = AFF_NONE;
        }
      continue;
    }
#pragma unroll
    for (int k = 0; k < SCAN_EPT; ++k)
      if (base + k < m) o[base + k] += add;
  }
}
struct DescPlan {
  unsigned long long at[40];
};
template <int LPK>
__global__ void __launch_bounds__(1024)
k_round_desc_all(const uint32_t* __restrict__ rp, uint32_t nkeys, int R, DescPlan plan, uint32_t* __restrict__ desc) {
  const uint32_t gid = blockIdx.x * blockDim.x + threadIdx.x;
  const uint32_t key = gid / LPK, lane = gid % LPK;
  if (key >= nkeys) return;
  const size_t stride = (size_t)nkeys + 1;
  for (int r0 = 1; r0 < R; r0 += 8) {
    uint32_t cr[8], o[8], oo[8];
#pragma unroll
    for (int q = 0; q < 8; ++q) {
      const int r = r0 + q;
      if (r < R) {
        const uint32_t* c = rp + (size_t)(2 * (r - 1)) * stride;
        cr[q] = c[key];
        o[q] = c[stride + key];
        oo[q] = c[3 * stride + key];
      } else {
        cr[q] = 0; o[q] = 0; oo[q] = 0;
      }
    }
#pragma unroll
    for (int q = 0; q < 8; ++q) {
      const int r = r0 + q;
      if (r >= R) break;
      const uint32_t nout = (cr[q] + 1) >> 1;
      uint32_t* d = desc + plan.at[r];
      for (uint32_t j = lane; j < nout; j += LPK) d[oo[q] + j] = (o[q] + 2 * j) | ((2 * j + 1 < cr[q]) ? DESC_PAIR : 0u);
    }
  }
}

template <int LPK>
__global__ void __launch_bounds__(256)
k_round_desc(const uint32_t* __restrict__ cnt, const uint32_t* __restrict__ off, const uint32_t* __restrict__ ooff ,
             uint32_t nkeys, uint32_t* __restrict__ desc) {
  const uint32_t gid = blockIdx.x * blockDim.x + threadIdx.x;
  const uint32_t key = gid / LPK, lane = gid % LPK;
  if (key >= nkeys) return;
  const uint32_t c = cnt[key], o = off[key], oo = ooff[key], nout = (c + 1) >> 1;
  for (uint32_t j = lane; j < nout; j += LPK) desc[oo + j] = (o + 2 * j) | ((2 * j + 1 < c) ? DESC_PAIR : 0u);
}

#ifndef AFF_PRIO
#define AFF_PRIO 1
#endif
#ifndef AFF_XY
#define AFF_XY 1
#endif
__device__ __forceinline__ void aff_set_prio(uint32_t v) {
  switch (v % 3u) {
    case 0: __builtin_amdgcn_s_setprio(0); break;
    case 1: __builtin_amdgcn_s_setprio(1); break;
    default: __builtin_amdgcn_s_setprio(2); break;
  }
}
constexpr uint32_t AFF_BMAX = 136;
__device__ __forceinline__ uint32_t aff_slots_per_thread(uint32_t total, uint32_t cap, uint32_t bmax_bmin) {
  const uint32_t bmax = bmax_bmin & 0xffu, bmin = (bmax_bmin >> 8) & 0xffu;
  const uint32_t units = (total + cap - 1) / cap;
  const uint32_t R = (units + bmax - 1) / bmax;
  const uint32_t B = R ? (units + R - 1) / R : 1;
  return B < bmin ? bmin : B;
}
struct WaveTrace {
  unsigned long long* buf;
  uint32_t cap, tag;
};
template <bool FIRST, bool TRACE = false>
__global__ void __launch_bounds__(EC_TPB) __attribute__((amdgpu_waves_per_eu(3, 3)))
k_affine_round(const Aff* __restrict__ pts, const uint2* __restrict__ desc, const uint32_t* __restrict__ total_ptr ,
               uint32_t cap, uint32_t bmax, GfSqrTables T, Gf* __restrict__ prefix, Aff* __restrict__ out, uint32_t sign_mask, WaveTrace wt) {
  extern __shared__ char lds_raw[];
  unsigned long long tr_t0 = 0, tr_c0 = 0, tr_t1 = 0, tr_t2 = 0;
  if (TRACE) { tr_t0 = wall_clock64(); tr_c0 = clock64(); }
  GfLdsK L = gf_ldsk_init(lds_raw);
#if AFF_PRIO
  const uint32_t wslot = __builtin_amdgcn_s_getreg(((4 - 1) << 11) | 4);
#endif
  const uint32_t sm = FIRST ? sign_mask : 0u;
  auto ldx = [&](uint32_t v) -> Gf { return pts[v & ~sm].x; };
  auto ldy = [&](uint32_t v, const Gf& x) -> Gf {
    Gf y = pts[v & ~sm].y;
    if (v & sm) y = gf_add(y, x);
    return y;
  };
  const uint32_t total = *total_ptr;
  const int B = (int)aff_slots_per_thread(total, cap, bmax);
  const uint32_t nthr = (total + B - 1) / B;
  const uint32_t tid = blockIdx.x * blockDim.x + threadIdx.x;
  if (tid >= nthr) return;
  const uint2 none = make_uint2(AFF_NONE, AFF_NONE);
  auto ld_desc = [&](int k) -> uint2 {
    const uint32_t sk = (uint32_t)k * nthr + tid;
    const bool ok = k >= 0 && k < B && sk < total;
    if (FIRST) {
      uint2 v = none;
      if (ok) v = desc[sk];
      return v;
    }
    const uint32_t d = ((const uint32_t*)desc)[ok ? sk : 0u], a = d & ~DESC_PAIR;
    return make_uint2(ok ? a : AFF_NONE, (ok && (d & DESC_PAIR)) ? a + 1 : AFF_NONE);
  };
  const Gf one = gf_one();
  Gf run = one;
  {
    uint2 d0 = ld_desc(0), d1 = ld_desc(1);
    Gf xa = gf_zero(), xb = gf_zero();
    if (d0.y != AFF_NONE) { xa = ldx(d0.x); xb = ldx(d0.y); }
#pragma unroll 1
    for (int k = 0; k < B; ++k) {
#if AFF_PRIO
      aff_set_prio(wslot + (uint32_t)k);
#endif
      const uint2 d2 = ld_desc(k + 2);
      Gf nxa = gf_zero(), nxb = gf_zero();
      if (d1.y != AFF_NONE) { nxa = ldx(d1.x); nxb = ldx(d1.y); }
      Gf den = one;
      if (d0.y != AFF_NONE && !gf_is_zero(xa) && !gf_is_zero(xb)) {
        Gf dd = gf_add(xa, xb);
        if (!gf_is_zero(dd)) den = dd;
        else if (gf_eq(ldy(d0.x, xa), ldy(d0.y, xb))) den = xa;
      }
      prefix[(size_t)k * nthr + tid] = run;
      run = gf_mul(run, den, L);
      d0 = d1; d1 = d2; xa = nxa; xb = nxb;
    }
  }
  if (TRACE) tr_t1 = wall_clock64();
  Gf inv = gf_inv_fast(run, T, L);
  if (TRACE) tr_t2 = wall_clock64();
  {
    uint2 e0 = ld_desc(B - 1), e1 = ld_desc(B - 2);
    Gf px = gf_zero(), qx = gf_zero(), pre = one;
    if (e0.x != AFF_NONE) px = ldx(e0.x);
    if (e0.y != AFF_NONE) { qx = ldx(e0.y); pre = prefix[(size_t)(B - 1) * nthr + tid]; }
#if AFF_XY
    Gf py = gf_zero(), qy = gf_zero();
    if (e0.x != AFF_NONE) py = ldy(e0.x, px);
    if (e0.y != AFF_NONE) qy = ldy(e0.y, qx);
#endif
#pragma unroll 1
    for (int k = B - 1; k >= 0; --k) {
#if AFF_PRIO
      aff_set_prio(wslot + (uint32_t)k);
#endif
      const uint2 e2 = ld_desc(k - 2);
#if AFF_XY
      Gf npx = gf_zero(), nqx = gf_zero(), npy = gf_zero(), nqy = gf_zero(), npre = one;
      if (e1.x != AFF_NONE) { npx = ldx(e1.x); npy = ldy(e1.x, npx); }
      if (e1.y != AFF_NONE) { nqx = ldx(e1.y); nqy = ldy(e1.y, nqx); npre = prefix[(size_t)(k - 1) * nthr + tid]; }
#else
      Gf py = gf_zero(), qy = gf_zero();
      if (e0.x != AFF_NONE) py = ldy(e0.x, px);
      if (e0.y != AFF_NONE) qy = ldy(e0.y, qx);
      Gf npx = gf_zero(), nqx = gf_zero(), npre = one;
      if (e1.x != AFF_NONE) npx = ldx(e1.x);
      if (e1.y != AFF_NONE) { nqx = ldx(e1.y); npre = prefix[(size_t)(k - 1) * nthr + tid]; }
#endif
      if (e0.x != AFF_NONE) {
        const uint32_t sidx = (uint32_t)k * nthr + tid;
        Gf ox = px, oy = py;
        if (e0.y != AFF_NONE) {
          if (gf_is_zero(px)) { ox = qx; oy = qy; }
          else if (!gf_is_zero(qx)) {
            Gf dd = gf_add(px, qx);
            const bool same_x = gf_is_zero(dd);
            const bool dbl = same_x && gf_eq(py, qy);
            if (same_x && !dbl) {
              ox = gf_zero(); oy = gf_zero();
            } else {
              Gf den = dbl ? px : dd;
              Gf dinv, inv_next;
              gf_mul2(pre, den, inv, L, dinv, inv_next);
              inv = inv_next;
              Gf num = dbl ? py : gf_add(py, qy);
              Gf lam = gf_mul(num, dinv, L);
              if (dbl) lam = gf_add(lam, px);
              ox = gf_add(gf_add(gf_sqr(lam), lam), dd);
              oy = gf_add(gf_add(gf_mul(gf_add(px, ox), lam, L), ox), py);
            }
          }
        }
        out[sidx].x = ox; out[sidx].y = oy;
      }
      e0 = e1; e1 = e2; px = npx; qx = nqx; pre = npre;
#if AFF_XY
      py = npy; qy = nqy;
#endif
    }
  }
#if AFF_PRIO
  __builtin_amdgcn_s_setprio(0);
#endif
  if (TRACE) {
    const unsigned long long t3 = wall_clock64(), c3 = clock64();
    if ((threadIdx.x & 63u) == 0) {
      const unsigned long long i = atomicAdd(wt.buf, 1ull);
      if (i < wt.cap) {
        unsigned long long* r = wt.buf + 8 + 8 * i;
        r[0] = tr_t0; r[1] = tr_t1; r[2] = tr_t2; r[3] = t3;
        r[4] = tr_c0; r[5] = c3;
        r[6] = (unsigned long long)__builtin_amdgcn_s_getreg((31 << 11) | 4) | ((unsigned long long)__builtin_amdgcn_s_getreg((31 << 11) | 20) << 32);
        r[7] = (unsigned long long)blockIdx.x | ((unsigned long long)wt.tag << 32) | ((unsigned long long)(uint32_t)B << 48);
      }
    }
  }
}

__global__ void __launch_bounds__(256)
k_bucket_gather_aff(const Aff* __restrict__ in, const uint32_t* __restrict__ cnt, const uint32_t* __restrict__ off,
                    uint32_t nkeys, Ld* __restrict__ A) {
  uint32_t k = blockIdx.x * blockDim.x + threadIdx.x;
  if (k >= nkeys) return;
  Ld r = ld_infinity();
  if (cnt[k]) {
    Aff p = in[off[k]];
    if (!gf_is_zero(p.x)) r = ld_from_aff(p);
  }
  A[k] = r;
}
__global__ void __launch_bounds__(256)
k_bucket_gather_items(const Aff* __restrict__ bases, const uint32_t* __restrict__ items, const uint32_t* __restrict__ cnt,
                      const uint32_t* __restrict__ off, uint32_t nkeys, Ld* __restrict__ A, uint32_t sign_mask) {
  uint32_t k = blockIdx.x * blockDim.x + threadIdx.x;
  if (k >= nkeys) return;
  Ld r = ld_infinity();
  if (cnt[k]) {
    const uint32_t v = items[off[k]];
    Aff q = bases[v & ~sign_mask];
    if (v & sign_mask) q.y = gf_add(q.y, q.x);
    r = ld_from_aff(q);
  }
  A[k] = r;
}

__global__ void __launch_bounds__(256)
k_bucket_gather(const Ld* __restrict__ in, const uint32_t* __restrict__ cnt, const uint32_t* __restrict__ off,
                uint32_t nkeys, Ld* __restrict__ A) {
  uint32_t k = blockIdx.x * blockDim.x + threadIdx.x;
  if (k >= nkeys) return;
  A[k] = cnt[k] ? in[off[k]] : ld_infinity();
}

template <int GROUP, bool FIRST>
__global__ void __launch_bounds__(EC_TPB) __attribute__((amdgpu_waves_per_eu(GROUP > 1 ? 1 : 2, 2))) k_merge(Ld* __restrict__ A, int j, uint32_t total , Ld* __restrict__ save0 ) {
  using LT = typename std::conditional<GROUP == 1, GfLdsK, typename std::conditional<GROUP == 4, GfLdsQ, GfLdsH>::type>::type;
  extern __shared__ char lds_raw[];
  uint32_t tid = blockIdx.x * blockDim.x + threadIdx.x;
  tid /= (uint32_t)GROUP;
  if (tid >= total) return;
  uint32_t blk = tid / (uint32_t)(j + 1), s = tid - blk * (uint32_t)(j + 1);
  size_t base = (size_t)blk << (j + 1);
  Ld l = A[base + s], r = A[base + ((size_t)1 << j) + s];
  LT L = MergeMul<LT>::init(lds_raw);
  const bool lead = MergeMul<LT>::lead(L);
  if (FIRST) {
    if (save0 && tid == 0 && lead) *save0 = l;
    lam_from_ld(l, L);
    lam_from_ld(r, L);
  }
  if (lead && s == 0 && j != 1) A[base + 1 + j] = r;
  if (!lam_add_ip(l, r, L)) {
    l = A[base + s];
    if (FIRST) lam_from_ld(l, L);
    lam_dbl_ip(l, L);
  }
  if (lead) A[base + s] = l;
}

__global__ void __launch_bounds__(EC_TPB) k_tail_groups(const Ld* __restrict__ A, int c, int W, int n_narrow, GfSqrTables T, Ld* __restrict__ buf ,
                                                        Ld* __restrict__ part) {
  extern __shared__ char lds_raw[];
  GfLdsH H = gf_ldsh_init(lds_raw);
  const uint32_t cnt0 = (uint32_t)(W * c), g0 = blockIdx.x * 16u;
  const uint32_t cntl = min(16u, cnt0 - g0);
  Ld* in = buf + g0;
  Ld* out = buf + cnt0 + g0;
  {
    const uint32_t row = threadIdx.x >> 4;
    if (row < cntl) {
      const uint32_t tid = g0 + row;
      const uint32_t w = tid / (uint32_t)c, t = tid - w * (uint32_t)c;
      const int k = (int)(w * (uint32_t)c) - min((int)w, n_narrow) + (int)t;
      Ld p = A[((size_t)w << c) + 1 + t];
      lam_to_ld(p, H);
      const uint32_t sel = H.r < 5u ? 0u : (H.r < 10u ? 1u : 2u);
      Gf v = sel == 0u ? p.X : (sel == 1u ? p.Y : p.Z);
      v = gf_sqr_n_fast(v, k, T);
      const int lane0 = (int)(threadIdx.x & 63u) - (int)H.r;
#pragma unroll
      for (int q = 0; q < 8; ++q) {
        p.X.w[q] = (uint32_t)__shfl((int)v.w[q], lane0);
        p.Y.w[q] = (uint32_t)__shfl((int)v.w[q], lane0 + 5);
        p.Z.w[q] = (uint32_t)__shfl((int)v.w[q], lane0 + 10);
      }
      if (H.r == 0) in[row] = p;
    }
  }
  __syncthreads();
  uint32_t cnt = cntl;
  while (cnt > 1) {
    const uint32_t half = (cnt + 1) / 2;
    const uint32_t i = threadIdx.x >> 4;
    if (i < half) {
      Ld a = in[2 * i];
      if (2 * i + 1 < cnt) ld_add_ip(a, in[2 * i + 1], H);
      if (H.r == 0) out[i] = a;
    }
    __syncthreads();
    Ld* t = in; in = out; out = t;
    cnt = half;
  }
  if (threadIdx.x == 0) part[blockIdx.x] = in[0];
}

template <bool HEX>
__global__ void __launch_bounds__(EC_TPB) k_tail(const Ld* __restrict__ A, int c, int W, int n_narrow, GfSqrTables T, Ld* __restrict__ buf,
                                                 uint32_t* __restrict__ out_xy, uint32_t* __restrict__ out_inf, uint8_t* __restrict__ out_enc, int rule,
                                                 unsigned long long* __restrict__ ctrl , unsigned long long* __restrict__ err_dst) {
  using LT = typename std::conditional<HEX, GfLdsH, GfLdsQ>::type;
  constexpr int GS = HEX ? 4 : 2;
  constexpr uint32_t NG = EC_TPB >> GS;
  extern __shared__ char lds_raw[];
  LT L = MergeMul<LT>::init(lds_raw);
  const uint32_t grp = threadIdx.x >> GS;
  const uint32_t cnt0 = (uint32_t)(W * c);
  Ld* in = buf;
  Ld* out = buf + cnt0;
  if (n_narrow == -4) {
  } else if (n_narrow == -3) {
    for (uint32_t q = 0; q * NG < cnt0; ++q) {
      const uint32_t idx = q * NG + ((q & 1u) ? NG - 1 - grp : grp);
      if (idx >= cnt0) continue;
      const uint32_t pt = cnt0 - 1 - idx;
      Ld p = pt + 1 < cnt0 ? A[1 + pt] : buf[2 * cnt0];
      if (pt + 1 < cnt0) lam_to_ld(p, L);
#pragma unroll 1
      for (uint32_t k = 0; k < pt; ++k) p = ld_dbl(p, L);
      if (L.r == 0) in[pt] = p;
    }
  } else {
    for (uint32_t tid = threadIdx.x; tid < cnt0; tid += EC_TPB) {
      uint32_t w = tid / (uint32_t)c, t = tid - w * (uint32_t)c;
      int k = (int)(w * (uint32_t)c) - min((int)w, n_narrow) + (int)t;
      Ld p = A[((size_t)w << c) + 1 + t];
      p.Y = gf_mul(p.X, gf_add(p.Y, p.X));
      p.X = gf_sqr_n_fast(p.X, k, T);
      p.Y = gf_sqr_n_fast(p.Y, k, T);
      p.Z = gf_sqr_n_fast(p.Z, k, T);
      in[tid] = p;
    }
  }
  __syncthreads();
  uint32_t cnt = cnt0;
  while (cnt > 1 && (HEX || (cnt + 1) / 2 > EC_TPB / 16)) {
    const uint32_t half = (cnt + 1) / 2;
    for (uint32_t i = grp; i < half; i += NG) {
      Ld a = in[2 * i];
      if (2 * i + 1 < cnt) ld_add_ip(a, in[2 * i + 1], L);
      if (L.r == 0) out[i] = a;
    }
    __syncthreads();
    Ld* t = in; in = out; out = t;
    cnt = half;
  }
  GfLdsH H;
  H.l = L.l;
  H.r = threadIdx.x & 15u;
  while (cnt > 1) {
    const uint32_t half = (cnt + 1) / 2;
    for (uint32_t i = threadIdx.x >> 4; i < half; i += EC_TPB / 16) {
      Ld a = in[2 * i];
      if (2 * i + 1 < cnt) ld_add_ip(a, in[2 * i + 1], H);
      if (H.r == 0) out[i] = a;
    }
    __syncthreads();
    Ld* t = in; in = out; out = t;
    cnt = half;
  }
  if (threadIdx.x >= 16) return;
  Aff a;
  Ld p = in[0];
  const bool fin = !ld_is_inf(p);
  a.x = gf_zero();
  a.y = gf_zero();
  Gf w = gf_zero();
  if (fin) {
    if (out_enc && !gf_is_zero(p.X)) {
      const Gf inv = gf_inv_fast(gf_mul(p.X, p.Z, H), T, H);
      const Gf zi = gf_mul(inv, p.X, H);
      a.x = gf_mul(p.X, zi, H);
      a.y = gf_mul(p.Y, gf_sqr(zi), H);
      const Gf lam1 = gf_add(gf_add(a.x, gf_mul(p.Y, inv, H)), gf_one());
      w = gf_sqr_tab_wide(gf_sqr_tab_wide(lam1, T.t116), T.t116);
      if (rule) w = codec_present(w, rule, T);
    } else {
      Gf zi = gf_inv_fast(p.Z, T, H);
      a.x = gf_mul(p.X, zi, H);
      a.y = gf_mul(p.Y, gf_sqr(zi), H);
      if (out_enc) {
        const Gf lam1 = gf_add(gf_add(a.x, gf_mul(a.y, gf_inv_fast(a.x, T, H), H)), gf_one());
        w = gf_sqr_tab_wide(gf_sqr_tab_wide(lam1, T.t116), T.t116);
        if (rule) w = codec_present(w, rule, T);
      }
    }
  }
  if (threadIdx.x != 0) return;
#pragma unroll
  for (int k = 0; k < 8; ++k) {
    out_xy[k] = a.x.w[k];
    out_xy[8 + k] = a.y.w[k];
  }
  *out_inf = fin ? 0u : 1u;
  if (out_enc) store30(out_enc, w, rule);
  const unsigned long long e = ctrl[0];
  if (err_dst) *err_dst = e;
  ctrl[2] = e;
  ctrl[0] = ~0ull;
  ctrl[1] = 0ull;
}

__global__ void __launch_bounds__(64) k_sum_points(const char* __restrict__ pts, uint32_t pt_stride_bytes, const uint32_t* __restrict__ inf, uint32_t n,
                                                  uint32_t inf_stride, GfSqrTables T, uint32_t* __restrict__ out_xy, uint32_t* __restrict__ out_inf) {
  extern __shared__ char lds_raw[];
  GfLdsQ L = gf_ldsq_init(lds_raw);
  if (threadIdx.x >= 4 || blockIdx.x != 0) return;
  Ld acc = ld_infinity();
#pragma unroll 1
  for (uint32_t i = 0; i < n; ++i) {
    if (inf[(size_t)i * inf_stride]) continue;
    Aff q = *(const Aff*)(pts + (size_t)i * pt_stride_bytes);
    ld_madd_ip(acc, q, L);
  }
  Aff a;
  a.x = gf_zero();
  a.y = gf_zero();
  const bool fin = !ld_is_inf(acc);
  if (fin) {
    Gf zi = gf_inv_fast(acc.Z, T, L);
    a.x = gf_mul(acc.X, zi, L);
    a.y = gf_mul(acc.Y, gf_sqr(zi), L);
  }
  if (threadIdx.x != 0) return;
#pragma unroll
  for (int k = 0; k < 8; ++k) {
    out_xy[k] = a.x.w[k];
    out_xy[8 + k] = a.y.w[k];
  }
  *out_inf = fin ? 0u : 1u;
}

__global__ void __launch_bounds__(EC_TPB) __attribute__((amdgpu_waves_per_eu(3, 3))) k_ubench_mul(Gf* __restrict__ out, int reps) {
  extern __shared__ char lds_raw[];
  GfLdsK L = gf_ldsk_init(lds_raw);
  const uint32_t t = threadIdx.x + blockIdx.x * blockDim.x;
  Gf x, y;
#pragma unroll
  for (int i = 0; i < 8; ++i) { x.w[i] = t * 2654435761u + i; y.w[i] = t * 40503u + 7 * i; }
  x.w[7] &= 0x1ff; y.w[7] &= 0x1ff;
#pragma unroll 1
  for (int r = 0; r < reps; ++r) { x = gf_mul(x, y, L); y.w[0] ^= x.w[3]; }
  out[t] = x;
}

static std::mutex g_wave_trace_mu;
static unsigned long long* g_wave_trace_buf = nullptr;
static uint32_t g_wave_trace_cap = 0;
static std::atomic<uint32_t> g_wave_trace_tag{0};
static void wave_trace_snapshot(unsigned long long** buf, uint32_t* cap) {
  std::lock_guard<std::mutex> g(g_wave_trace_mu);
  *buf = g_wave_trace_buf;
  *cap = g_wave_trace_cap;
}

struct MsmWorkspace {
  std::mutex mu;
  void* p = nullptr;
  size_t bytes = 0;
  int device = -1;
  hipStream_t aux = nullptr;
  hipEvent_t ev = nullptr;
  hipEvent_t ev_heavy = nullptr;
  hipEvent_t ev_busy = nullptr;
  hipStream_t busy_stream = nullptr;
  bool busy_valid = false;
  bool ctrl_clean = false;
  bool busy_for(hipStream_t st) { return busy_valid && busy_stream != st && hipEventQuery(ev_busy) == hipErrorNotReady; }
  uint32_t* pinned = nullptr;
  hipStream_t side = nullptr;
  hipEvent_t ev_pre = nullptr;
  std::vector<hipEvent_t> ev_side;
  int ensure_side(size_t rounds) {
    if (!side) {
      DVP_HIP(hipStreamCreateWithFlags(&side, hipStreamNonBlocking));
      DVP_HIP(hipEventCreateWithFlags(&ev_pre, hipEventDisableTiming));
    }
    while (ev_side.size() < rounds) {
      hipEvent_t b = nullptr;
      DVP_HIP(hipEventCreateWithFlags(&b, hipEventDisableTiming));
      ev_side.push_back(b);
    }
    return DVP_OK;
  }
  int ensure_aux() {
    if (aux) return DVP_OK;
    DVP_HIP(hipStreamCreateWithFlags(&aux, hipStreamNonBlocking));
    DVP_HIP(hipEventCreateWithFlags(&ev, hipEventDisableTiming));
    DVP_HIP(hipEventCreateWithFlags(&ev_heavy, hipEventDisableTiming));
    DVP_HIP(hipEventCreateWithFlags(&ev_busy, hipEventDisableTiming));
    DVP_HIP(hipHostMalloc((void**)&pinned, 64, hipHostMallocDefault));
    return DVP_OK;
  }
  int ensure(size_t need, std::atomic<size_t>& dev_max) {
    size_t seen = dev_max.load();
    while (seen < need && !dev_max.compare_exchange_weak(seen, need)) {}
    if (seen > need) need = seen;
    int dev;
    DVP_HIP(hipGetDevice(&dev));
    if (p && (dev != device || bytes < need)) {
      if (ev_busy) (void)hipEventSynchronize(ev_busy);
      (void)hipFree(p);
      p = nullptr;
      bytes = 0;
    }
    if (!p) {
      DVP_HIP(hipMalloc(&p, need));
      ctrl_clean = false;
      bytes = need;
      device = dev;
    }
    return DVP_OK;
  }
};
constexpr int MSM_MAX_DEVICES = 16;
constexpr int MSM_WS_SLOTS = 2;
static MsmWorkspace g_ws_dev[MSM_MAX_DEVICES][MSM_WS_SLOTS];
static std::atomic<size_t> g_ws_need[MSM_MAX_DEVICES];
struct HeavyGate {
  std::mutex mu;
  hipEvent_t last = nullptr;
};
static HeavyGate g_heavy[MSM_MAX_DEVICES];

struct MsmPlan {
  uint32_t n;
  int c, W, n_narrow;
  uint32_t K, nkeys;
  size_t e_max, t1_max, t2_max;
};

static MsmPlan msm_plan(size_t n, const struct MsmFixedCtx* fx);
struct MsmFixedCtx {
  Aff* table = nullptr;
  uint32_t n_total = 0;
  int c = FX_C_MAX, W = TAU_DIGITS / FX_C_MAX, n_narrow = 0;
  void set_c(int cc) {
    c = cc;
    int w_main = (234 + cc - 1) / cc;
    n_narrow = w_main * cc - 234;
    W = w_main + 1;
  }
  bool signed_digits = false;
  void set_c_signed(int cc) {
    for (;; --cc) {
      W = (234 + cc - 1) / cc;
      n_narrow = W * cc - 234;
      if (n_narrow < W || cc <= 2) break;
    }
    c = cc;
    signed_digits = true;
  }
  int rows() const { return W; }
  int key_bits() const { return signed_digits ? c - 1 : c; }
  int hi_bits = -1;
  FxBits bits() const { FxBits b; b.hi = hi_bits; b.lo = key_bits() - b.hi; return b; }
};
static MsmPlan msm_plan(size_t n, const MsmFixedCtx* fx) {
  const bool fixed = fx != nullptr;
  MsmPlan p;
  p.n = (uint32_t)n;
  auto windows = [](int c, int* n_narrow) {
    int w_main = (234 + c - 1) / c;
    *n_narrow = w_main * c - 234;
    return w_main + (TAU_DIGITS - 234 + c - 1) / c;
  };
  double best = 1e300;
  p.c = 4;
  int nn;
  for (int c = 4; c <= 15; ++c) {
    int W = windows(c, &nn);
    double cost = W * (8.4 * (double)n + 28.0 * (double)(1u << c));
    if (cost < best) { best = cost; p.c = c; }
  }
  const bool small_latency = !fixed && n >= ((size_t)1 << 15) && n <= ((size_t)1 << 18);
  if (small_latency) p.c = 10;
  if (!fixed && n > ((size_t)1 << 18) && n <= ((size_t)1 << 19)) p.c = 13;
  if (tune().msm_c >= 2 && tune().msm_c <= 15) p.c = (int)tune().msm_c;
  p.W = windows(p.c, &p.n_narrow);
  p.nkeys = (uint32_t)p.W << p.c;
  if (fixed) {
    p.c = fx->c;
    p.W = fx->W;
    p.n_narrow = fx->n_narrow;
    p.nkeys = 1u << fx->key_bits();
  }
  p.e_max = n * (size_t)p.W;
  uint32_t K = (uint32_t)(p.e_max / 262144);
  if (K < 8) K = 8;
  if (K > 16) K = 16;
  if (!fixed && n <= ((size_t)1 << 18)) K = 4;
  if (small_latency) K = 8;
  if (!fixed && n > ((size_t)1 << 18) && n <= ((size_t)1 << 19)) K = 8;
  if (fixed) K = 8;
  if (tune().msm_k >= 2 && tune().msm_k <= 64) K = (uint32_t)tune().msm_k;
  p.K = K;
  p.t1_max = p.e_max / K + p.nkeys + 1;
  p.t2_max = p.t1_max / K + p.nkeys + 1;
  return p;
}

static size_t align_up(size_t v) { return (v + 255) & ~(size_t)255; }

static int msm_core(const void* d_scalars, const void* d_bases, const void* d_inf, size_t n, const MsmFixedCtx* fx, uint32_t i0,
                    void* d_out_xy, void* d_out_inf, hipStream_t st, void* d_out_enc = nullptr ,
                    void* h_copy = nullptr, const void* d_copy = nullptr, size_t copy_bytes = 0 ,
                    unsigned long long* d_err_defer = nullptr ) {
  if (n == 0 && d_err_defer) {
    DVP_HIP(hipMemsetAsync(d_out_xy, 0, 64, st));
    if (d_out_enc) DVP_HIP(hipMemsetAsync(d_out_enc, 0, 30, st));
    DVP_HIP(hipMemsetAsync(d_out_inf, 0, 4, st));
    DVP_HIP(hipMemsetAsync(d_out_inf, 1, 1, st));
    DVP_HIP(hipMemsetAsync(d_err_defer, 0xff, 8, st));
    return DVP_OK;
  }
  if (n == 0) {
    DVP_HIP(hipMemsetAsync(d_out_xy, 0, 64, st));
    if (d_out_enc) DVP_HIP(hipMemsetAsync(d_out_enc, 0, 30, st));
    if (h_copy) DVP_HIP(hipMemcpyAsync(h_copy, d_copy, copy_bytes, hipMemcpyDeviceToHost, st));
    uint32_t one = 1;
    DVP_HIP(hipMemcpyAsync(d_out_inf, &one, 4, hipMemcpyHostToDevice, st));
    DVP_HIP(hipStreamSynchronize(st));
    return DVP_OK;
  }
  if (n > (1u << 27)) return DVP_EINVAL;
  const uint32_t sign_mask = (fx && fx->signed_digits) ? ITEM_NEG : 0u;
  {
    const MsmPlan pl = msm_plan(n, fx);
    const uint64_t tab = fx ? (uint64_t)fx->rows() * fx->n_total : (uint64_t)n;
    if ((uint64_t)pl.e_max >= 0xfffffff0ull || tab >= (sign_mask ? 0x7ffffff0ull : 0xfffffff0ull)) return DVP_EINVAL;
  }
  int cur_dev = 0;
  DVP_HIP(hipGetDevice(&cur_dev));
  if (cur_dev < 0 || cur_dev >= MSM_MAX_DEVICES) return DVP_EINVAL;
  {
    static std::mutex attr_mu;
    static bool attr_done[MSM_MAX_DEVICES] = {false};
    std::lock_guard<std::mutex> ga(attr_mu);
    if (!attr_done[cur_dev]) {
      hipError_t attr_err = hipFuncSetAttribute((const void*)k_scatter_local, hipFuncAttributeMaxDynamicSharedMemorySize, 131072);
      if (attr_err == hipSuccess)
        attr_err = hipFuncSetAttribute((const void*)k_hist_local, hipFuncAttributeMaxDynamicSharedMemorySize, 65536);
      if (attr_err == hipSuccess)
        attr_err = hipFuncSetAttribute((const void*)k_scatter_local2, hipFuncAttributeMaxDynamicSharedMemorySize, 131072);
      if (attr_err == hipSuccess)
        attr_err = hipFuncSetAttribute((const void*)k_hist_local2, hipFuncAttributeMaxDynamicSharedMemorySize, 65536);
      if (attr_err == hipSuccess)
        attr_err = hipFuncSetAttribute((const void*)k_part_scatter_staged, hipFuncAttributeMaxDynamicSharedMemorySize, FX_STAGE1_LDS);
      if (attr_err == hipSuccess)
        attr_err = hipFuncSetAttribute((const void*)k_part_scatter_signed<true>, hipFuncAttributeMaxDynamicSharedMemorySize, FX_STAGE1_LDS);
      if (attr_err == hipSuccess)
        attr_err = hipFuncSetAttribute((const void*)k_scatter_local2_staged, hipFuncAttributeMaxDynamicSharedMemorySize, FX_STAGE2_LDS);
      const void* ec[] = {(const void*)k_accum_affine<true, false>, (const void*)k_accum_affine<false, false>, (const void*)k_accum_affine<true, true>,
                          (const void*)k_accum_affine<false, true>, (const void*)k_accum_proj<1>, (const void*)k_accum_proj<4>, (const void*)k_accum_proj<16>,
                          (const void*)k_accum_affine_fast<true, false>, (const void*)k_accum_affine_fast<false, false>, (const void*)k_accum_affine_fast<true, true>,
                          (const void*)k_accum_affine_fast<false, true>, (const void*)k_accum_affine_rest<true>, (const void*)k_accum_affine_rest<false>,
                          (const void*)k_tail_groups, (const void*)k_merge<1, false>, (const void*)k_merge<4, false>, (const void*)k_merge<16, false>, (const void*)k_merge<1, true>, (const void*)k_merge<4, true>, (const void*)k_merge<16, true>,
                          (const void*)k_affine_round<true, false>, (const void*)k_affine_round<false, false>, (const void*)k_affine_round<true, true>,
                          (const void*)k_affine_round<false, true>, (const void*)k_sum_points, (const void*)k_tail<false>, (const void*)k_tail<true>,
                          (const void*)k_bucket_pairs, (const void*)k_bucket_rest};
      for (const void* f : ec)
        if (attr_err == hipSuccess) attr_err = hipFuncSetAttribute(f, hipFuncAttributeMaxDynamicSharedMemorySize, EC_LDS_Q);
      DVP_HIP(attr_err);
      attr_done[cur_dev] = true;
    }
  }
  MsmPlan p = msm_plan(n, fx);
  const FxBits fb = fx ? fx->bits() : FxBits{0, 0};
  const uint32_t FX_NP = fb.np();
  std::unique_lock<std::mutex> g;
  int ws_slot = 0;
  const int ws_slots = tune().msm_ws_slots >= 1 && tune().msm_ws_slots <= MSM_WS_SLOTS ? (int)tune().msm_ws_slots : 1;
  for (int pass = 0; pass < 2 && !g.owns_lock(); ++pass)
    for (int sl = 0; sl < ws_slots && !g.owns_lock(); ++sl) {
      g = std::unique_lock<std::mutex>(g_ws_dev[cur_dev][sl].mu, std::try_to_lock);
      if (g.owns_lock() && pass == 0 && g_ws_dev[cur_dev][sl].busy_for(st)) g.unlock();
      if (g.owns_lock()) ws_slot = sl;
    }
  if (!g.owns_lock()) g = std::unique_lock<std::mutex>(g_ws_dev[cur_dev][0].mu);
  MsmWorkspace& g_ws = g_ws_dev[cur_dev][ws_slot];
  if (g_ws.busy_valid) {
    if (g_ws.busy_stream != st) DVP_HIP(hipStreamWaitEvent(st, g_ws.ev_busy, 0));
    g_ws.busy_valid = false;
  }
  size_t o = 0;
  auto carve = [&](size_t bytes) { size_t r = o; o = align_up(o + bytes); return r; };
  size_t o_err = carve(32);
  size_t o_digits = carve(fx ? 16 : (size_t)p.W * n * 2);
  const bool fused1 = fx && fx->signed_digits && tune().msm_sort_fused != 0;
  const uint32_t fx_S = fused1 ? (FX_CHUNK / (uint32_t)p.W > 0 ? FX_CHUNK / (uint32_t)p.W : 1u) : 0u;
  const uint32_t fx_nblk = fused1 ? cdiv(n, fx_S) : cdiv(p.e_max, FX_CHUNK);
  size_t o_digits32 = carve(fx && !fused1 ? p.e_max * 4 : 16);
  size_t o_plo = carve(fx ? p.e_max * 2 : 16);
  size_t o_pid = carve(fx ? p.e_max * 4 : 16);
  size_t o_phist = carve(fx ? (size_t)fx_nblk * FX_NP * 4 : 16);
  size_t o_pbase = carve(fx ? (size_t)fx_nblk * FX_NP * 4 : 16);
  const uint32_t fx_nch = cdiv(fx_nblk, FX_SCAN_CB);
  size_t o_ctot = carve(fx ? (size_t)FX_NP * fx_nch * 4 : 16);
  size_t o_pstart = carve((FX_NP_MAX + 1) * 4 * 3);
  size_t o_cnt = carve(((size_t)p.nkeys + 1) * 4);
  size_t o_off = carve(((size_t)p.nkeys + 1) * 4);
  size_t o_ntask = carve(((size_t)p.nkeys + 1) * 4);
  size_t o_toff = carve(((size_t)p.nkeys + 1) * 4);
  size_t o_cnt2 = carve(((size_t)p.nkeys + 1) * 4);
  size_t o_off2 = carve(((size_t)p.nkeys + 1) * 4);
  size_t o_bsum = carve(((size_t)p.nkeys / SCAN_BLK + 8) * 4);
  size_t o_items = carve((p.e_max + (size_t)p.nkeys + 2) * 4);
  const size_t sort_cells = fx ? ((size_t)(fx_nblk + FX_NP + 1) << fb.lo) : ((size_t)p.W * cdiv(n, SORT_CHUNK) << p.c);
  size_t o_hist16 = carve(sort_cells * 2);
  size_t o_choff = carve(sort_cells * 4);
  size_t o_bufA = carve(p.t1_max * sizeof(Ld));
  size_t o_bufB = carve(p.t2_max * sizeof(Ld));
  const Tune tn = tune();
  const bool affine_mode = !tn.msm_proj;
  const size_t affA_n = p.e_max / 2 + p.nkeys + 1, affB_n = p.e_max / 4 + p.nkeys + 1;
  size_t o_affA = carve(affine_mode ? affA_n * sizeof(Aff) : 16);
  size_t o_affB = carve(affine_mode ? affB_n * sizeof(Aff) : 16);
  size_t o_prefix = carve(affine_mode ? (affA_n + 256) * sizeof(Gf) : 16);
  const size_t aff_min = (size_t)(tn.msm_aff_min > 0 ? tn.msm_aff_min : 1);
  const size_t e_est = (size_t)n * (size_t)((fx && fx->signed_digits) ? p.W : (234 + p.c - 1) / p.c);
  int ra_plan = 0;
  while (affine_mode && ra_plan < 40 && (e_est >> (ra_plan + 1)) >= aff_min) ++ra_plan;
  const bool pipelined = affine_mode && tn.msm_round_pipeline != 0 && ra_plan >= 2 && e_est >= 4 * (size_t)p.nkeys;
  const bool side_stream = pipelined && tn.msm_round_pipeline == 1;
  std::vector<size_t> desc_at((size_t)ra_plan + 1, 0);
  size_t desc_n = affA_n + 64;
  if (pipelined) {
    size_t cap_r = p.e_max + p.nkeys, at = 0;
    for (int r = 0; r < ra_plan; ++r) {
      const size_t out_max = cap_r / 2 + p.nkeys + 1;
      if (r >= 1) { desc_at[r] = at; at += out_max + 64; }
      cap_r = out_max;
    }
    if (at > desc_n) desc_n = at;
  }
  size_t o_gdesc = carve(affine_mode ? desc_n * sizeof(uint32_t) : 16);
  size_t o_rp = carve(pipelined ? (size_t)ra_plan * 2 * ((size_t)p.nkeys + 1) * 4 : 16);
  size_t o_bsum2 = carve(((size_t)((ra_plan > 0 ? ra_plan : 1) + 1) * ((size_t)p.nkeys / SCAN_BLK + 1) + 8) * 4);
  size_t o_bkt = carve((size_t)p.nkeys * sizeof(Ld));
  const size_t rest_cap = (size_t)p.nkeys + 2 + p.e_max / (size_t)(p.K > 0 ? p.K : 1);
  size_t o_rest = carve(rest_cap * 4);
  const uint32_t tail_groups = ((uint32_t)(p.W * p.c) + 15u) / 16u;
  size_t o_tail = carve(((size_t)2 * p.W * p.c + 1 + 2 * (size_t)tail_groups) * sizeof(Ld));
  DVP_TRY(g_ws.ensure(o, g_ws_need[cur_dev]));
  char* base = (char*)g_ws.p;
  auto* err = (unsigned long long*)(base + o_err);
  auto* digits = (uint16_t*)(base + o_digits);
  auto* digits32 = (uint32_t*)(base + o_digits32);
  auto* plo = (uint16_t*)(base + o_plo);
  auto* pid = (uint32_t*)(base + o_pid);
  auto* phist = (uint32_t*)(base + o_phist);
  auto* pbase = (uint32_t*)(base + o_pbase);
  auto* ctot = (uint32_t*)(base + o_ctot);
  auto* pstart = (uint32_t*)(base + o_pstart);
  auto* cstart = pstart + FX_NP_MAX + 1;
  auto* pcount = cstart + FX_NP_MAX + 1;
  auto* cnt = (uint32_t*)(base + o_cnt);
  auto* off = (uint32_t*)(base + o_off);
  auto* ntask = (uint32_t*)(base + o_ntask);
  auto* toff = (uint32_t*)(base + o_toff);
  auto* cnt2 = (uint32_t*)(base + o_cnt2);
  auto* off2 = (uint32_t*)(base + o_off2);
  auto* bsum = (uint32_t*)(base + o_bsum);
  auto* items = (uint32_t*)(base + o_items);
  auto* hist16 = (uint16_t*)(base + o_hist16);
  auto* chunk_off = (uint32_t*)(base + o_choff);
  Ld* bufA = (Ld*)(base + o_bufA);
  Ld* bufB = (Ld*)(base + o_bufB);
  Ld* bkt = (Ld*)(base + o_bkt);
  Aff* affA = (Aff*)(base + o_affA);
  Aff* affB = (Aff*)(base + o_affB);
  Gf* prefix = (Gf*)(base + o_prefix);
  uint32_t* gdesc = (uint32_t*)(base + o_gdesc);
  auto* rp = (uint32_t*)(base + o_rp);
  auto* bsum2 = (uint32_t*)(base + o_bsum2);
  Ld* tail = (Ld*)(base + o_tail);
  auto* rest_list = (uint32_t*)(base + o_rest);
  const uint32_t nk = p.nkeys;

  auto bookkeep = [&](int r, const uint32_t* ic, const uint32_t* io, uint32_t* oc, uint32_t* oo, uint32_t* dsc, hipStream_t s, uint32_t* bs) -> int {
    DVP_TRY(scan_exclusive_div(ic, 2u, oc, oo, nk, bs, s));
    const size_t per_key = (e_est >> (r + 1)) / nk;
#define DVP_DESC_LAUNCH(LPK) hipLaunchKernelGGL((k_round_desc<LPK>), dim3(cdiv((size_t)nk * LPK, 256)), dim3(256), 0, s, ic, io, oo, nk, dsc)
    if (per_key >= 48) DVP_DESC_LAUNCH(64); else if (per_key >= 8) DVP_DESC_LAUNCH(16); else DVP_DESC_LAUNCH(4);
#undef DVP_DESC_LAUNCH
    return DVP_OK;
  };
  auto rc = [&](int r) -> uint32_t* { return r == 0 ? cnt : rp + (size_t)(2 * (r - 1)) * ((size_t)nk + 1); };
  auto ro = [&](int r) -> uint32_t* { return r == 0 ? off : rp + (size_t)(2 * (r - 1) + 1) * ((size_t)nk + 1); };
  int prepared = 0;
  uint32_t* d_max = (uint32_t*)(err + 1);
  uint32_t* rest_n = d_max + 1;
  auto read_max = [&]() -> int {
    DVP_TRY(g_ws.ensure_aux());
    DVP_HIP(hipEventRecord(g_ws.ev, st));
    DVP_HIP(hipStreamWaitEvent(g_ws.aux, g_ws.ev, 0));
    DVP_HIP(hipMemcpyAsync(g_ws.pinned, d_max, 4, hipMemcpyDeviceToHost, g_ws.aux));
    return DVP_OK;
  };
  const bool sort_done_by_mscan = pipelined && !side_stream;
  auto prepare_rounds = [&]() -> int {
    if (!pipelined) return DVP_OK;
    hipStream_t bk = st;
    if (side_stream) {
      DVP_TRY(g_ws.ensure_side(1));
      DVP_HIP(hipEventRecord(g_ws.ev_pre, st));
      DVP_HIP(hipStreamWaitEvent(g_ws.side, g_ws.ev_pre, 0));
      bk = g_ws.side;
    }
    const uint32_t nb = cdiv(nk, SCAN_BLK);
    uint32_t* off0 = side_stream ? nullptr : off;
    hipLaunchKernelGGL(k_mscan_local, dim3(nb), dim3(SCAN_TPB), 0, bk, cnt, nk, ra_plan, rp, bsum2);
    hipLaunchKernelGGL(k_mscan_bsums, dim3(ra_plan), dim3(SCAN_TPB), 0, bk, bsum2, nb, nk, rp, off0, off0 ? d_max : (uint32_t*)nullptr);
    if (off0) DVP_TRY(read_max());
    hipLaunchKernelGGL(k_mscan_add, dim3(nb), dim3(SCAN_TPB), 0, bk, rp, bsum2, nk, ra_plan, (const uint32_t*)cnt, off0, items);
    DescPlan plan;
    for (int q = 0; q < 40; ++q) plan.at[q] = q < ra_plan ? desc_at[q] : 0;
    const size_t per_key = (e_est >> 2) / nk;
    if (per_key >= 48)
      hipLaunchKernelGGL((k_round_desc_all<64>), dim3(cdiv((size_t)nk * 64, 1024)), dim3(1024), 0, bk, rp, nk, ra_plan, plan, gdesc);
    else if (per_key >= 8)
      hipLaunchKernelGGL((k_round_desc_all<16>), dim3(cdiv((size_t)nk * 16, 1024)), dim3(1024), 0, bk, rp, nk, ra_plan, plan, gdesc);
    else
      hipLaunchKernelGGL((k_round_desc_all<4>), dim3(cdiv((size_t)nk * 4, 1024)), dim3(1024), 0, bk, rp, nk, ra_plan, plan, gdesc);
    if (side_stream) DVP_HIP(hipEventRecord(g_ws.ev_side[0], g_ws.side));
    DVP_HIP(hipGetLastError());
    prepared = ra_plan;
    return DVP_OK;
  };
  ProfScope ps_total(PROF_MSM_TOTAL, st);
  ProfScope ps_sort(PROF_MSM_SORT, st);
  if (!g_ws.ctrl_clean) {
    DVP_HIP(hipMemsetAsync(err, 0xff, 8, st));
    DVP_HIP(hipMemsetAsync(err + 1, 0, 8, st));
  }
  g_ws.ctrl_clean = false;
  if (fused1)
    ;
  else if (fx && fx->signed_digits)
    hipLaunchKernelGGL(k_recode_signed, dim3(cdiv(n, 256)), dim3(256), 0, st, (const uint32_t*)d_scalars, (const uint8_t*)d_inf, (uint32_t)n,
                       p.c, p.W, p.n_narrow, digits32, err);
  else if (fx)
    hipLaunchKernelGGL((k_recode<uint32_t>), dim3(cdiv(n, 256)), dim3(256), 0, st, (const uint32_t*)d_scalars, (const uint8_t*)d_inf,
                       (uint32_t)n, p.c, p.W, p.n_narrow, digits32, err);
  else
    hipLaunchKernelGGL((k_recode<uint16_t>), dim3(cdiv(n, 256)), dim3(256), 0, st, (const uint32_t*)d_scalars, (const uint8_t*)d_inf,
                       (uint32_t)n, p.c, p.W, p.n_narrow, digits, err);
  if (fx) {
    const uint32_t gmax = fx_nblk + FX_NP;
    if (fused1)
      hipLaunchKernelGGL(k_part_hist_signed, dim3(fx_nblk), dim3(SORT_TPB), 0, st, (const uint32_t*)d_scalars, (const uint8_t*)d_inf, (uint32_t)n,
                         p.c, p.W, p.n_narrow, fx_S, fb, phist, err);
    else
      hipLaunchKernelGGL(k_part_hist, dim3(fx_nblk), dim3(SORT_TPB), 0, st, digits32, p.e_max, fb, phist);
    hipLaunchKernelGGL(k_part_scan_chunks, dim3(fx_nch), dim3(256), 0, st, phist, fx_nblk, fb, pbase, ctot, fx_nch);
    hipLaunchKernelGGL(k_part_scan_totals, dim3(cdiv((size_t)FX_NP * 64, 256)), dim3(256), 0, st, ctot, fx_nch, fb, pcount);
    hipLaunchKernelGGL(k_part_starts, dim3(1), dim3(FX_NP_MAX), 0, st, pcount, fb, pstart, cstart);
    const bool staged1 = FX_NP >= 64;
    const bool staged2 = fb.lo <= 10;
    if (fused1 && staged1)
      hipLaunchKernelGGL(k_part_scatter_signed<true>, dim3(fx_nblk), dim3(SORT_TPB), FX_STAGE1_LDS, st, (const uint32_t*)d_scalars,
                         (const uint8_t*)d_inf, (uint32_t)n, p.c, p.W, p.n_narrow, fx_S, fx->n_total, i0, fb, phist, pbase, ctot, fx_nch, pstart, plo, pid);
    else if (fused1)
      hipLaunchKernelGGL(k_part_scatter_signed<false>, dim3(fx_nblk), dim3(SORT_TPB), (2 * FX_NP_MAX + SORT_TPB) * 4, st, (const uint32_t*)d_scalars,
                         (const uint8_t*)d_inf, (uint32_t)n, p.c, p.W, p.n_narrow, fx_S, fx->n_total, i0, fb, phist, pbase, ctot, fx_nch, pstart, plo, pid);
    else if (staged1)
      hipLaunchKernelGGL(k_part_scatter_staged, dim3(fx_nblk), dim3(SORT_TPB), FX_STAGE1_LDS, st, digits32, p.e_max, (uint32_t)n,
                         fx->n_total, i0, fb, phist, pbase, ctot, fx_nch, pstart, plo, pid);
    else
      hipLaunchKernelGGL(k_part_scatter, dim3(fx_nblk), dim3(SORT_TPB), 0, st, digits32, p.e_max, (uint32_t)n, fx->n_total, i0, fb, pbase,
                         ctot, fx_nch, pstart, plo, pid);
    hipLaunchKernelGGL(k_hist_local2, dim3(gmax), dim3(SORT_TPB), (1u << fb.lo) * 2, st, plo, pstart, cstart, fb, hist16);
    hipLaunchKernelGGL(k_hist_scan2, dim3(cdiv(nk, 256)), dim3(256), 0, st, hist16, cstart, fb, chunk_off, cnt);
    DVP_TRY(prepare_rounds());
    if (!sort_done_by_mscan) DVP_TRY(scan_exclusive(cnt, off, nk, bsum, st, true));
    if (staged2)
      hipLaunchKernelGGL(k_scatter_local2_staged, dim3(gmax), dim3(SORT_TPB), FX_STAGE2_LDS, st, plo, pid, pstart, cstart, fb, off,
                         chunk_off, hist16, items);
    else
      hipLaunchKernelGGL(k_scatter_local2, dim3(gmax), dim3(SORT_TPB), (1u << fb.lo) * 4, st, plo, pid, pstart, cstart, fb, off, chunk_off, items);
  } else {
    const uint32_t nchunks = cdiv(n, SORT_CHUNK), nb = 1u << p.c;
    hipLaunchKernelGGL(k_hist_local, dim3(nchunks, p.W), dim3(SORT_TPB), (nb >> 1) * 4, st, digits, (uint32_t)n, p.c, hist16);
    hipLaunchKernelGGL(k_hist_scan, dim3(cdiv(nk, 256)), dim3(256), 0, st, hist16, nchunks, p.c, p.W, chunk_off, cnt);
    DVP_TRY(prepare_rounds());
    if (!sort_done_by_mscan) DVP_TRY(scan_exclusive(cnt, off, nk, bsum, st, true));
    hipLaunchKernelGGL(k_scatter_local, dim3(nchunks, p.W), dim3(SORT_TPB), nb * 4, st, digits, (uint32_t)n, p.c, off, chunk_off, items);
  }
  ps_sort.stop();
  uint32_t* pc[3] = {cnt, ntask, cnt2};
  uint32_t* po[3] = {off, toff, off2};
  bool r0_offsets_ready = false;
  if (!sort_done_by_mscan) {
    hipLaunchKernelGGL(k_post_sort, dim3(cdiv(nk + 1, 256)), dim3(256), 0, st, items, cnt, off, nk, pc[1], po[1], d_max);
    r0_offsets_ready = true;
    DVP_TRY(read_max());
  }
  int cur = 0;
  const Aff* bases0 = fx ? fx->table : (const Aff*)d_bases;
  const Aff* pts_in = bases0;
  size_t cap = p.e_max + nk;
  GfSqrTables Tsq;
  DVP_TRY(gf_sqr_tables(&Tsq, st));
  int n_cu = 256, blk_per_cu = 3;
  DVP_HIP(hipDeviceGetAttribute(&n_cu, hipDeviceAttributeMultiprocessorCount, cur_dev));
  const uint32_t aff_tpb = (tn.msm_aff_tpb == 64 || tn.msm_aff_tpb == 128 || tn.msm_aff_tpb == 256) ? (uint32_t)tn.msm_aff_tpb : (uint32_t)EC_TPB;
  const uint32_t aff_lds = (aff_tpb / 64) * GF_LDSK_BYTES_PER_WAVE;
  DVP_HIP(hipOccupancyMaxActiveBlocksPerMultiprocessor(&blk_per_cu, (const void*)k_affine_round<false, false>, (int)aff_tpb, aff_lds));
  if (blk_per_cu < 1) blk_per_cu = 1;
  const uint32_t aff_cap = (uint32_t)n_cu * (uint32_t)blk_per_cu * aff_tpb;
  const uint32_t aff_bmax_only = tn.msm_aff_bmax >= 1 && tn.msm_aff_bmax <= 255 ? (uint32_t)tn.msm_aff_bmax : AFF_BMAX;
  const uint32_t aff_bmin = tn.msm_aff_bmin >= 1 && (uint32_t)tn.msm_aff_bmin <= aff_bmax_only ? (uint32_t)tn.msm_aff_bmin : 1u;
  const uint32_t aff_bmax = aff_bmax_only | (aff_bmin << 8);
  unsigned long long* wt_buf = nullptr;
  uint32_t wt_cap = 0;
  wave_trace_snapshot(&wt_buf, &wt_cap);
  const bool wt_on = wt_buf != nullptr;
  auto launch_round = [&](int r, const uint32_t* d_total, const uint2* dsc) -> int {
    size_t out_max = cap / 2 + nk + 1;
    Aff* outp = (r & 1) ? affB : affA;
    const uint32_t r_max = cdiv(cdiv(out_max, aff_cap), aff_bmax_only);
    const uint32_t grid = r_max * (aff_cap / aff_tpb) + 1;
    {
      ProfScope ps0(r == 0 ? PROF_MSM_ACCUM_AFFINE : -1, st, (uint64_t)n);
      WaveTrace wt{wt_buf, wt_cap, g_wave_trace_tag.fetch_add(wt_on ? 1u : 0u)};
      if (r == 0 && wt.buf)
        hipLaunchKernelGGL((k_affine_round<true, true>), dim3(grid), dim3(aff_tpb), aff_lds, st, pts_in, dsc, d_total, aff_cap, aff_bmax, Tsq, prefix, outp, sign_mask, wt);
      else if (r == 0)
        hipLaunchKernelGGL((k_affine_round<true, false>), dim3(grid), dim3(aff_tpb), aff_lds, st, pts_in, dsc, d_total, aff_cap, aff_bmax, Tsq, prefix, outp, sign_mask, wt);
      else if (wt.buf)
        hipLaunchKernelGGL((k_affine_round<false, true>), dim3(grid), dim3(aff_tpb), aff_lds, st, pts_in, dsc, d_total, aff_cap, aff_bmax, Tsq, prefix, outp, 0u, wt);
      else
        hipLaunchKernelGGL((k_affine_round<false, false>), dim3(grid), dim3(aff_tpb), aff_lds, st, pts_in, dsc, d_total, aff_cap, aff_bmax, Tsq, prefix, outp, 0u, wt);
      ps0.stop();
    }
    pts_in = outp;
    cap = out_max;
    return DVP_OK;
  };
  auto run_round = [&](int r) -> int {
    if (pipelined) {
      if (r == 0 && side_stream) DVP_HIP(hipStreamWaitEvent(st, g_ws.ev_side[0], 0));
      DVP_TRY(launch_round(r, ro(r + 1) + nk, r == 0 ? (const uint2*)items : (const uint2*)(const void*)(gdesc + desc_at[r])));
      return DVP_OK;
    }
    const int nxt = (cur + 1) % 3;
    if (r == 0) {
      if (!(r0_offsets_ready && cur == 0))
        hipLaunchKernelGGL(k_round0_offsets, dim3(cdiv(nk + 1, 256)), dim3(256), 0, st, pc[cur], po[cur], nk, pc[nxt], po[nxt]);
    } else
      DVP_TRY(bookkeep(r, pc[cur], po[cur], pc[nxt], po[nxt], gdesc, st, bsum));
    DVP_TRY(launch_round(r, po[nxt] + nk, r == 0 ? (const uint2*)items : (const uint2*)(const void*)gdesc));
    cur = nxt;
    return DVP_OK;
  };
  int launched = 0;
  std::unique_lock<std::mutex> heavy;
  if (ws_slots > 1 && affine_mode) {
    heavy = std::unique_lock<std::mutex>(g_heavy[cur_dev].mu);
    if (g_heavy[cur_dev].last && g_heavy[cur_dev].last != g_ws.ev_heavy) DVP_HIP(hipStreamWaitEvent(st, g_heavy[cur_dev].last, 0));
  }
  if (affine_mode && (e_est >> 1) >= aff_min && e_est >= 4 * (size_t)nk) {
    DVP_TRY(run_round(0));
    launched = 1;
  }
  DVP_HIP(hipStreamSynchronize(g_ws.aux));
  count_host_wait(launched ? 1 : 0);
  const uint32_t max_cnt = *g_ws.pinned;
  int ra = 0;
  if (affine_mode)
    while (((uint64_t)1 << ra) < max_cnt && (e_est >> (ra + 1)) >= aff_min) ++ra;
  if (ra < launched) ra = launched;
  int r_evt = -1;
  if (heavy.owns_lock() && ra > 0) {
    const size_t gate_min = tn.msm_gate_min > 0 ? (size_t)tn.msm_gate_min : 1;
    r_evt = 0;
    while (r_evt + 1 < ra && (e_est >> (r_evt + 2)) >= gate_min) ++r_evt;
  }
  auto gate_event = [&]() -> int {
    DVP_HIP(hipEventRecord(g_ws.ev_heavy, st));
    g_heavy[cur_dev].last = g_ws.ev_heavy;
    return DVP_OK;
  };
  if (r_evt >= 0 && r_evt < launched) DVP_TRY(gate_event());
  {
    int r = launched;
    if (r == 0 && ra > 0) {
      DVP_TRY(run_round(0));
      if (r_evt == 0) DVP_TRY(gate_event());
      r = 1;
    }
    ProfScope ps_rest(ra > r ? PROF_MSM_AFFINE_REST : -1, st, (uint64_t)(ra > r ? ra - r : 0));
    for (; r < ra; ++r) {
      DVP_TRY(run_round(r));
      if (r == r_evt) DVP_TRY(gate_event());
    }
    ps_rest.stop();
  }
  if (pipelined && prepared) {
    if (!launched && side_stream) DVP_HIP(hipStreamWaitEvent(st, g_ws.ev_side[0], 0));
    pc[0] = rc(ra); po[0] = ro(ra);
    cur = 0;
  }
  if (heavy.owns_lock()) heavy.unlock();
  uint64_t rem_max = ((uint64_t)max_cnt + ((uint64_t)1 << ra) - 1) >> ra;
  if (rem_max <= 1) {
    if (ra == 0)
      hipLaunchKernelGGL(k_bucket_gather_items, dim3(cdiv(nk, 256)), dim3(256), 0, st, bases0, items, cnt, off, nk, bkt, sign_mask);
    else
      hipLaunchKernelGGL(k_bucket_gather_aff, dim3(cdiv(nk, 256)), dim3(256), 0, st, pts_in, pc[cur], po[cur], nk, bkt);
  } else if (ra > 0 && rem_max <= (uint64_t)(tn.msm_bucket_pairs_max >= 0 ? tn.msm_bucket_pairs_max : 0)) {
    hipLaunchKernelGGL(k_bucket_pairs, dim3(cdiv(nk, EC_TPB)), dim3(EC_TPB), EC_LDS, st, pts_in, pc[cur], po[cur], nk, bkt, rest_n, rest_list);
    hipLaunchKernelGGL(k_bucket_rest, dim3(cdiv(nk, EC_TPB)), dim3(EC_TPB), EC_LDS, st, pts_in, pc[cur], po[cur], rest_n, rest_list, bkt);
  } else {
    int nxt = (cur + 1) % 3;
    DVP_TRY(scan_exclusive_div(pc[cur], p.K, pc[nxt], po[nxt], nk, bsum, st));
    size_t tmax = cap / p.K + nk + 1;
    const size_t accum_quad_max = tn.msm_accum_quad_max > 0 ? (size_t)tn.msm_accum_quad_max : ACCUM_QUAD_MAX;
    const size_t accum_hex_max = tn.msm_accum_hex_max >= 0 ? (size_t)tn.msm_accum_hex_max : ACCUM_HEX_MAX;
    const bool accum_fast = tn.msm_accum_fast != 0 && tmax <= rest_cap;
#define DVP_ACCUM_AFFINE(IND)                                                                                                                  \
  do {                                                                                                                                         \
    if (accum_fast) {                                                                                                                          \
      if (tmax <= accum_quad_max)                                                                                                              \
        hipLaunchKernelGGL((k_accum_affine_fast<IND, true>), dim3(cdiv(4 * tmax, EC_TPB)), dim3(EC_TPB), EC_LDS_Q, st, pts_in, items, pc[cur], \
                           po[cur], po[nxt], nk, p.K, bufA, sign_mask, rest_n, rest_list);                                                    \
      else                                                                                                                                     \
        hipLaunchKernelGGL((k_accum_affine_fast<IND, false>), dim3(cdiv(tmax, EC_TPB)), dim3(EC_TPB), EC_LDS, st, pts_in, items, pc[cur],      \
                           po[cur], po[nxt], nk, p.K, bufA, sign_mask, rest_n, rest_list);                                                    \
      hipLaunchKernelGGL((k_accum_affine_rest<IND>), dim3(cdiv(tmax, EC_TPB)), dim3(EC_TPB), EC_LDS, st, pts_in, items, pc[cur], po[cur],       \
                         po[nxt], nk, p.K, bufA, sign_mask, rest_n, rest_list);                                                                \
    } else if (tmax <= accum_quad_max)                                                                                                         \
      hipLaunchKernelGGL((k_accum_affine<IND, true>), dim3(cdiv(4 * tmax, EC_TPB)), dim3(EC_TPB), EC_LDS_Q, st, pts_in, items, pc[cur], po[cur], \
                         po[nxt], nk, p.K, bufA, sign_mask);                                                                                   \
    else                                                                                                                                       \
      hipLaunchKernelGGL((k_accum_affine<IND, false>), dim3(cdiv(tmax, EC_TPB)), dim3(EC_TPB), EC_LDS, st, pts_in, items, pc[cur], po[cur],     \
                         po[nxt], nk, p.K, bufA, sign_mask);                                                                                   \
  } while (0)
    if (ra == 0) {
      ProfScope ps0(PROF_MSM_ACCUM_AFFINE, st);
      DVP_ACCUM_AFFINE(true);
      ps0.stop();
    } else
      DVP_ACCUM_AFFINE(false);
#undef DVP_ACCUM_AFFINE
    cur = nxt;
    cap = tmax;
    Ld *in = bufA, *outb = bufB;
    for (uint64_t left = (rem_max + p.K - 1) / p.K; left > 1; left = (left + p.K - 1) / p.K) {
      nxt = (cur + 1) % 3;
      DVP_TRY(scan_exclusive_div(pc[cur], p.K, pc[nxt], po[nxt], nk, bsum, st));
      tmax = cap / p.K + nk + 1;
      if (left <= p.K && tmax <= accum_hex_max)
        hipLaunchKernelGGL(k_accum_proj<16>, dim3(cdiv(16 * tmax, EC_TPB)), dim3(EC_TPB), EC_LDS_Q, st, in, pc[cur], po[cur], po[nxt], nk, p.K, outb);
      else if (tmax <= accum_quad_max)
        hipLaunchKernelGGL(k_accum_proj<4>, dim3(cdiv(4 * tmax, EC_TPB)), dim3(EC_TPB), EC_LDS_Q, st, in, pc[cur], po[cur], po[nxt], nk, p.K, outb);
      else
        hipLaunchKernelGGL(k_accum_proj<1>, dim3(cdiv(tmax, EC_TPB)), dim3(EC_TPB), EC_LDS, st, in, pc[cur], po[cur], po[nxt], nk, p.K, outb);
      cap = tmax;
      cur = nxt;
      Ld* t = in; in = outb; outb = t;
    }
    hipLaunchKernelGGL(k_bucket_gather, dim3(cdiv(nk, 256)), dim3(256), 0, st, in, pc[cur], po[cur], nk, bkt);
  }
  ProfScope ps_tail(PROF_MSM_TAIL, st);
  const int merge_levels = fx ? fx->key_bits() : p.c;
  Ld* save0 = sign_mask ? tail + 2 * (size_t)p.c : nullptr;
  for (int j = 0; j < merge_levels; ++j) {
    uint32_t total = (nk >> (j + 1)) * (uint32_t)(j + 1);
    const uint32_t quad_max = tn.msm_quad_max > 0 ? (uint32_t)tn.msm_quad_max : MERGE_QUAD_MAX;
    const uint32_t hex_max = tn.msm_hex_max >= 0 ? (uint32_t)tn.msm_hex_max : MERGE_HEX_MAX;
#define DVP_MERGE(G, F, LDSB) hipLaunchKernelGGL((k_merge<G, F>), dim3(cdiv((size_t)G * total, EC_TPB)), dim3(EC_TPB), LDSB, st, bkt, j, total, save0)
    if (total <= hex_max) { if (j == 0) DVP_MERGE(16, true, EC_LDS_Q); else DVP_MERGE(16, false, EC_LDS_Q); }
    else if (total <= quad_max) { if (j == 0) DVP_MERGE(4, true, EC_LDS_Q); else DVP_MERGE(4, false, EC_LDS_Q); }
    else { if (j == 0) DVP_MERGE(1, true, EC_LDS); else DVP_MERGE(1, false, EC_LDS); }
#undef DVP_MERGE
  }
  const int w_tail = fx ? 1 : p.W;
  uint32_t cntT = (uint32_t)(w_tail * p.c);
  Ld* ta = tail;
  if (sign_mask && tn.msm_hex_max != 0)
    hipLaunchKernelGGL(k_tail<true>, dim3(1), dim3(EC_TPB), EC_LDS_Q, st, bkt, p.c, w_tail, -3, Tsq, ta, (uint32_t*)d_out_xy, (uint32_t*)d_out_inf,
                       (uint8_t*)d_out_enc, d_out_enc ? dvp_codec_get_rule() : 0, err, d_err_defer);
  else if (!sign_mask && cntT > 32 && tn.msm_tail_groups != 0) {
    Ld* part = tail + 2 * (size_t)cntT + 1;
    const int nparts = (int)cdiv(cntT, 16);
    hipLaunchKernelGGL(k_tail_groups, dim3(nparts), dim3(EC_TPB), EC_LDS_Q, st, bkt, p.c, w_tail, fx ? 0 : p.n_narrow, Tsq, ta, part);
    hipLaunchKernelGGL(k_tail<false>, dim3(1), dim3(EC_TPB), EC_LDS_Q, st, bkt, nparts, 1, -4, Tsq, part, (uint32_t*)d_out_xy,
                       (uint32_t*)d_out_inf, (uint8_t*)d_out_enc, d_out_enc ? dvp_codec_get_rule() : 0, err, d_err_defer);
  } else
    hipLaunchKernelGGL(k_tail<false>, dim3(1), dim3(EC_TPB), EC_LDS_Q, st, bkt, p.c, w_tail, sign_mask ? -3 : (fx ? 0 : p.n_narrow), Tsq, ta, (uint32_t*)d_out_xy,
                       (uint32_t*)d_out_inf, (uint8_t*)d_out_enc, d_out_enc ? dvp_codec_get_rule() : 0, err, d_err_defer);
  ps_tail.stop();
  ps_total.stop();
  DVP_HIP(hipGetLastError());
  g_ws.ctrl_clean = true;
  if (d_err_defer) {
    DVP_HIP(hipEventRecord(g_ws.ev_busy, st));
    g_ws.busy_stream = st;
    g_ws.busy_valid = true;
    return DVP_OK;
  }
  volatile unsigned long long* h_err = (volatile unsigned long long*)(g_ws.pinned + 2);
  if (h_copy) DVP_HIP(hipMemcpyAsync(h_copy, d_copy, copy_bytes, hipMemcpyDeviceToHost, st));
  DVP_HIP(hipMemcpyAsync((void*)h_err, err + 2, 8, hipMemcpyDeviceToHost, st));
  DVP_HIP(hipStreamSynchronize(st));
  count_host_wait(0);
  const unsigned long long e = *h_err;
  if (e != ~0ull) {
    g_last_error_index = (int64_t)(e & 0xffffffffull);
    return DVP_EINVAL;
  }
  return DVP_OK;
}

int msm_sum_points_dev(const void* d_pts, uint32_t pt_stride_bytes, const void* d_inf32, uint32_t n, uint32_t inf_stride, void* d_out_xy,
                       void* d_out_inf, hipStream_t st) {
  GfSqrTables Tsq;
  DVP_TRY(gf_sqr_tables(&Tsq, st));
  hipLaunchKernelGGL(k_sum_points, dim3(1), dim3(64), GF_LDS_BYTES_PER_WAVE, st, (const char*)d_pts, pt_stride_bytes, (const uint32_t*)d_inf32, n,
                     inf_stride, Tsq, (uint32_t*)d_out_xy, (uint32_t*)d_out_inf);
  DVP_HIP(hipGetLastError());
  return DVP_OK;
}

int msm_affine_dev(const void* d_scalars, const void* d_bases, const void* d_inf, size_t n, void* d_out_xy,
                   void* d_out_inf, hipStream_t st) {
  return msm_core(d_scalars, d_bases, d_inf, n, nullptr, 0, d_out_xy, d_out_inf, st);
}

void msm_fixed_destroy(MsmFixedCtx* c);
static int msm_fixed_build(const Aff* d_bases, uint32_t n_total, size_t range_hint, MsmFixedCtx** out, hipError_t* alloc_err) {
  MsmFixedCtx* c = new MsmFixedCtx();
  c->n_total = n_total;
  double best = 1e300;
  int best_c = 8;
  const bool signed_aligned = tune().msm_aligned_signed != 0;
  if (signed_aligned) {
    for (int cc = 8; cc <= FX_C_MAX + 1; ++cc) {
      MsmFixedCtx probe;
      probe.set_c_signed(cc);
      if (probe.c != cc) continue;
      const int kb = cc - 1;
      const double per_scalar = (double)probe.W;
      double cost = per_scalar * (double)range_hint * 5.6 + 10.0 * (double)(1u << kb) + (kb > 18 ? 25.0 * (double)((1u << kb) - (1u << 18)) : 0.0);
      if (cost < best) { best = cost; best_c = cc; }
    }
    if (tune().msm_fixed_c >= 8 && tune().msm_fixed_c <= FX_C_MAX + 1) best_c = (int)tune().msm_fixed_c;
    c->set_c_signed(best_c);
  } else {
    for (int cc = 8; cc <= FX_C_MAX; ++cc) {
      const double per_scalar = (double)((234 + cc - 1) / cc);
      double cost = per_scalar * (double)range_hint * 5.6 + 10.0 * (double)(1u << cc) + (cc > 18 ? 25.0 * (double)((1u << cc) - (1u << 18)) : 0.0);
      if (cost < best) { best = cost; best_c = cc; }
    }
    if (tune().msm_fixed_c >= 8 && tune().msm_fixed_c <= FX_C_MAX) best_c = (int)tune().msm_fixed_c;
    c->set_c(best_c);
  }
  const int kb = c->key_bits();
  c->hi_bits = kb / 2;
  if (int h = (int)tune().fx_hi; h >= 0 && h <= 10 && kb - h <= 15 && kb - h >= 1) c->hi_bits = h;
  hipError_t e = hipMalloc((void**)&c->table, (size_t)c->rows() * n_total * sizeof(Aff));
  *alloc_err = e;
  if (e == hipSuccess) {
    if (c->signed_digits) {
      GfSqrTables Tsq;
      int rc_t = gf_sqr_tables(&Tsq, 0);
      if (rc_t != DVP_OK) { msm_fixed_destroy(c); return rc_t; }
      e = hipFuncSetAttribute((const void*)k_dbl_table, hipFuncAttributeMaxDynamicSharedMemorySize, EC_LDS);
      Gf* scratch = nullptr;
      const size_t per = (size_t)(c->W > 1 ? c->W - 1 : 1) * n_total;
      if (e == hipSuccess) e = hipMalloc((void**)&scratch, 2 * per * sizeof(Gf));
      if (e == hipSuccess) {
        hipLaunchKernelGGL(k_dbl_table, dim3(cdiv(n_total, 256)), dim3(256), EC_LDS, 0, d_bases, n_total, c->c, c->W, c->n_narrow, Tsq, c->table,
                           scratch, scratch + per);
        e = hipGetLastError();
        if (e == hipSuccess) e = hipDeviceSynchronize();
      }
      if (scratch) (void)hipFree(scratch);
    } else
      hipLaunchKernelGGL(k_frob_table, dim3(cdiv(n_total, 256)), dim3(256), 0, 0, d_bases, n_total, c->c, c->W, c->n_narrow, c->table);
    if (e == hipSuccess) e = hipGetLastError();
  }
  if (e == hipSuccess) e = hipDeviceSynchronize();
  if (e != hipSuccess) {
    c->table = *alloc_err == hipSuccess ? c->table : nullptr;
    msm_fixed_destroy(c);
    return hip_fail(e, "msm_fixed_create", __FILE__, __LINE__);
  }
  *out = c;
  return DVP_OK;
}
int msm_fixed_create(const Aff* d_bases, uint32_t n_total, size_t range_hint, MsmFixedCtx** out) {
  if ((uint64_t)n_total * 32 >= 0xfffffff0ull) return DVP_EINVAL;
  hipError_t alloc_err = hipSuccess;
  return msm_fixed_build(d_bases, n_total, range_hint, out, &alloc_err);
}
int msm_fixed_info(const MsmFixedCtx* c, int* cbits, int* windows) {
  if (!c) return DVP_EINVAL;
  *cbits = c->c;
  *windows = c->W;
  return DVP_OK;
}
const void* msm_fixed_table_ptr(const MsmFixedCtx* c) { return c ? (const void*)c->table : nullptr; }
uint64_t msm_fixed_table_bytes(const MsmFixedCtx* c, int* signed_flavour) {
  if (signed_flavour) *signed_flavour = c && c->signed_digits ? 1 : 0;
  return c ? (uint64_t)c->rows() * c->n_total * sizeof(Aff) : 0;
}
void msm_fixed_destroy(MsmFixedCtx* c) {
  if (!c) return;
  if (c->table) (void)hipFree(c->table);
  delete c;
}
int msm_fixed_dev(const MsmFixedCtx* c, const void* d_scalars, const void* d_inf, uint32_t lo, uint32_t hi, void* d_out_xy,
                  void* d_out_inf, hipStream_t st) {
  if (!c || lo > hi || hi > c->n_total) return DVP_EINVAL;
  return msm_core(d_scalars, nullptr, d_inf, hi - lo, c, lo, d_out_xy, d_out_inf, st);
}
int msm_fixed_dev_enc(const MsmFixedCtx* c, const void* d_scalars, const void* d_inf, uint32_t lo, uint32_t hi, void* d_out_xy,
                      void* d_out_inf, void* d_out_enc, void* h_copy, const void* d_copy, size_t copy_bytes, hipStream_t st,
                      unsigned long long* d_err_defer) {
  if (!c || lo > hi || hi > c->n_total) return DVP_EINVAL;
  return msm_core(d_scalars, nullptr, d_inf, hi - lo, c, lo, d_out_xy, d_out_inf, st, d_out_enc, h_copy, d_copy, copy_bytes, d_err_defer);
}
int msm_affine_dev_enc(const void* d_scalars, const void* d_bases, const void* d_inf, size_t n, void* d_out_xy, void* d_out_inf,
                       void* d_out_enc, void* h_copy, const void* d_copy, size_t copy_bytes, hipStream_t st, unsigned long long* d_err_defer) {
  return msm_core(d_scalars, d_bases, d_inf, n, nullptr, 0, d_out_xy, d_out_inf, st, d_out_enc, h_copy, d_copy, copy_bytes, d_err_defer);
}

}

using namespace dvp;

extern "C" int dvp_msm_affine_dev(const void* d_scalars, const void* d_bases_xy, const void* d_bases_inf, size_t n,
                                  void* d_out_xy, void* d_out_inf, void* stream) {
  if ((n && (!d_scalars || !d_bases_xy)) || !d_out_xy || !d_out_inf) return DVP_EINVAL;
  return msm_affine_dev(d_scalars, d_bases_xy, d_bases_inf, n, d_out_xy, d_out_inf, (hipStream_t)stream);
}

extern "C" int dvp_points_sum_dev(const void* d_records, uint32_t n, void* d_out_xy, void* d_out_inf, void* stream) {
  if (!d_records || !n || !d_out_xy || !d_out_inf) return DVP_EINVAL;
  return msm_sum_points_dev(d_records, 80, (const char*)d_records + 64, n, 20, d_out_xy, d_out_inf, (hipStream_t)stream);
}

extern "C" int dvp_debug_wave_trace(void* d_buf, uint32_t n_records) {
  {
    std::lock_guard<std::mutex> g(g_wave_trace_mu);
    g_wave_trace_cap = d_buf ? n_records : 0;
    g_wave_trace_buf = (unsigned long long*)d_buf;
    g_wave_trace_tag.store(0);
  }
  DVP_HIP(hipDeviceSynchronize());
  return DVP_OK;
}

extern "C" int dvp_ubench_gf_mul(int reps, double* products_per_s) {
  if (reps < 1 || !products_per_s) return DVP_EINVAL;
  int dev = 0, n_cu = 256;
  DVP_HIP(hipGetDevice(&dev));
  DVP_HIP(hipDeviceGetAttribute(&n_cu, hipDeviceAttributeMultiprocessorCount, dev));
  const int blocks = n_cu * 3 * 8;
  DevBuf out;
  DVP_TRY(out.alloc((size_t)blocks * EC_TPB * sizeof(Gf)));
  hipEvent_t e0, e1;
  DVP_HIP(hipEventCreate(&e0));
  DVP_HIP(hipEventCreate(&e1));
  float best = 1e30f;
  for (int it = 0; it < 3; ++it) {
    DVP_HIP(hipEventRecord(e0, 0));
    hipLaunchKernelGGL(k_ubench_mul, dim3(blocks), dim3(EC_TPB), EC_LDS, 0, out.as<Gf>(), reps);
    DVP_HIP(hipEventRecord(e1, 0));
    DVP_HIP(hipEventSynchronize(e1));
    float ms = 0;
    DVP_HIP(hipEventElapsedTime(&ms, e0, e1));
    if (ms < best) best = ms;
  }
  (void)hipEventDestroy(e0);
  (void)hipEventDestroy(e1);
  DVP_HIP(hipGetLastError());
  *products_per_s = (double)blocks * EC_TPB * reps / (best * 1e-3);
  return DVP_OK;
}

__device__ __forceinline__ uint64_t ubench_mix(uint64_t x) {
  x ^= x >> 33; x *= 0xff51afd7ed558ccdull; x ^= x >> 33; x *= 0xc4ceb9fe1a85ec53ull; x ^= x >> 33;
  return x;
}
__global__ void __launch_bounds__(256) k_ubench_gather(const uint4* __restrict__ t, uint64_t nlines, int per, uint32_t seed, uint32_t* __restrict__ out) {
  const uint64_t tid = blockIdx.x * (uint64_t)blockDim.x + threadIdx.x;
  uint4 acc = make_uint4(0, 0, 0, 0);
#pragma unroll 4
  for (int k = 0; k < per; ++k) {
    const uint64_t idx = ubench_mix(tid * (uint64_t)per + k + ((uint64_t)seed << 40)) % nlines;
    const uint4* p = t + idx * 4;
    const uint4 a = p[0], b = p[1], c = p[2], d = p[3];
    acc.x ^= a.x ^ b.x ^ c.x ^ d.x; acc.y ^= a.y ^ b.y ^ c.y ^ d.y; acc.z ^= a.z ^ b.z ^ c.z ^ d.z; acc.w ^= a.w ^ b.w ^ c.w ^ d.w;
  }
  if ((acc.x ^ acc.y ^ acc.z ^ acc.w) == 0x12345678u) out[0] = 1;
}
extern "C" int dvp_ubench_gather(const void* d_table, size_t table_bytes, int reps, double* gathers_per_s) {
  if (reps < 1 || reps > 64 || !gathers_per_s || table_bytes < (1u << 20)) return DVP_EINVAL;
  int dev = 0, n_cu = 256;
  DVP_HIP(hipGetDevice(&dev));
  DVP_HIP(hipDeviceGetAttribute(&n_cu, hipDeviceAttributeMultiprocessorCount, dev));
  DevBuf own, out;
  if (!d_table) {
    DVP_TRY(own.alloc(table_bytes));
    DVP_HIP(hipMemset(own.p, 0x5a, table_bytes));
    d_table = own.p;
  }
  DVP_TRY(out.alloc(16));
  const int per = 32;
  const uint32_t blocks = (uint32_t)n_cu * 3 * 8;
  const uint64_t nlines = table_bytes / 64;
  hipEvent_t e0, e1;
  DVP_HIP(hipEventCreate(&e0));
  DVP_HIP(hipEventCreate(&e1));
  hipLaunchKernelGGL(k_ubench_gather, dim3(blocks), dim3(256), 0, 0, (const uint4*)d_table, nlines, per, 1u, out.as<uint32_t>());
  DVP_HIP(hipEventRecord(e0, 0));
  for (int r = 0; r < reps; ++r)
    hipLaunchKernelGGL(k_ubench_gather, dim3(blocks), dim3(256), 0, 0, (const uint4*)d_table, nlines, per, 2u + (uint32_t)r, out.as<uint32_t>());
  DVP_HIP(hipEventRecord(e1, 0));
  DVP_HIP(hipEventSynchronize(e1));
  float ms = 0;
  DVP_HIP(hipEventElapsedTime(&ms, e0, e1));
  (void)hipEventDestroy(e0);
  (void)hipEventDestroy(e1);
  DVP_HIP(hipGetLastError());
  *gathers_per_s = (double)reps * blocks * 256.0 * per / (ms * 1e-3);
  return DVP_OK;
}


extern "C" int dvp_debug_recode_signed(const uint64_t* scalars, size_t n, int c, uint32_t* out_words, int* windows) {
  if (!windows || c < 8 || c > FX_C_MAX + 1 || n > (1u << 24)) return DVP_EINVAL;
  MsmFixedCtx plan;
  plan.set_c_signed(c);
  if (plan.c != c) return DVP_EINVAL;
  *windows = plan.W;
  if (!out_words) return DVP_OK;
  if (!scalars || !n) return DVP_EINVAL;
  DevBuf ds, dw, de;
  DVP_TRY(ds.alloc(n * 32));
  DVP_TRY(dw.alloc((size_t)*windows * n * 4));
  DVP_TRY(de.alloc(8));
  DVP_HIP(hipMemcpy(ds.p, scalars, n * 32, hipMemcpyHostToDevice));
  DVP_HIP(hipMemset(de.p, 0xff, 8));
  hipLaunchKernelGGL(k_recode_signed, dim3(cdiv(n, 256)), dim3(256), 0, 0, ds.as<uint32_t>(), (const uint8_t*)nullptr, (uint32_t)n, c, *windows, plan.n_narrow,
                     dw.as<uint32_t>(), de.as<unsigned long long>());
  DVP_HIP(hipGetLastError());
  DVP_HIP(hipMemcpy(out_words, dw.p, (size_t)*windows * n * 4, hipMemcpyDeviceToHost));
  unsigned long long e = 0;
  DVP_HIP(hipMemcpy(&e, de.p, 8, hipMemcpyDeviceToHost));
  if (e != ~0ull) {
    g_last_error_index = (int64_t)(e & 0xffffffffull);
    return DVP_EINVAL;
  }
  return DVP_OK;
}

extern "C" int dvp_msm_affine(const uint64_t* scalars, const uint64_t* bases_xy, const uint8_t* bases_inf, size_t n,
                              uint64_t out_xy[8], int* out_is_infinity) {
  if ((n && (!scalars || !bases_xy)) || !out_xy || !out_is_infinity) return DVP_EINVAL;
  DevBuf ds, db, di, dout;
  DVP_TRY(ds.alloc(n * 32));
  DVP_TRY(db.alloc(n * 64));
  DVP_TRY(dout.alloc(64 + 16));
  if (n) {
    DVP_HIP(hipMemcpy(ds.p, scalars, n * 32, hipMemcpyHostToDevice));
    DVP_HIP(hipMemcpy(db.p, bases_xy, n * 64, hipMemcpyHostToDevice));
  }
  if (bases_inf && n) {
    DVP_TRY(di.alloc(n));
    DVP_HIP(hipMemcpy(di.p, bases_inf, n, hipMemcpyHostToDevice));
  }
  DVP_TRY(msm_affine_dev(ds.p, db.p, di.p, n, dout.p, (char*)dout.p + 64, 0));
  uint32_t inf;
  DVP_HIP(hipMemcpy(out_xy, dout.p, 64, hipMemcpyDeviceToHost));
  DVP_HIP(hipMemcpy(&inf, (char*)dout.p + 64, 4, hipMemcpyDeviceToHost));
  *out_is_infinity = (int)inf;
  return DVP_OK;
}

struct dvp_msm_ctx {
  MsmFixedCtx* fx = nullptr;
  uint8_t* d_inf = nullptr;
  size_t n = 0;
};

extern "C" void dvp_msm_ctx_destroy(dvp_msm_ctx* c);
extern "C" int dvp_msm_ctx_create(const uint64_t* bases_xy, const uint8_t* bases_inf, size_t n, size_t range_hint, dvp_msm_ctx** out) {
  if (!bases_xy || !out || !n || n >= ((size_t)1 << 27)) return DVP_EINVAL;
  if (!range_hint || range_hint > n) range_hint = n;
  DevBuf db;
  DVP_TRY(db.alloc(n * sizeof(Aff)));
  DVP_HIP(hipMemcpy(db.p, bases_xy, n * sizeof(Aff), hipMemcpyHostToDevice));
  dvp_msm_ctx* c = new dvp_msm_ctx();
  c->n = n;
  auto fail = [&](int rc) { dvp_msm_ctx_destroy(c); return rc; };
  hipError_t e = hipMalloc((void**)&c->d_inf, n);
  if (e == hipSuccess) e = bases_inf ? hipMemcpy(c->d_inf, bases_inf, n, hipMemcpyHostToDevice) : hipMemset(c->d_inf, 0, n);
  if (e != hipSuccess) return fail(hip_fail(e, "dvp_msm_ctx_create", __FILE__, __LINE__));
  int rc = msm_fixed_create(db.as<Aff>(), (uint32_t)n, range_hint, &c->fx);
  if (rc != DVP_OK) return fail(rc);
  *out = c;
  return DVP_OK;
}
extern "C" void dvp_msm_ctx_destroy(dvp_msm_ctx* c) {
  if (!c) return;
  msm_fixed_destroy(c->fx);
  if (c->d_inf) (void)hipFree(c->d_inf);
  delete c;
}
extern "C" int dvp_msm_ctx_plan(const dvp_msm_ctx* c, int* c_bits, int* windows) {
  if (!c || !c_bits || !windows) return DVP_EINVAL;
  return msm_fixed_info(c->fx, c_bits, windows);
}
extern "C" uint64_t dvp_msm_ctx_table_bytes(const dvp_msm_ctx* c, int* signed_windows) { return c ? msm_fixed_table_bytes(c->fx, signed_windows) : 0; }
extern "C" int dvp_msm_ctx_run_dev(dvp_msm_ctx* c, const void* d_scalars, size_t lo, size_t hi, void* d_out_xy, void* d_out_inf, void* stream) {
  if (!c || !d_scalars || !d_out_xy || !d_out_inf || lo > hi || hi > c->n) return DVP_EINVAL;
  return msm_fixed_dev(c->fx, d_scalars, c->d_inf + lo, (uint32_t)lo, (uint32_t)hi, d_out_xy, d_out_inf, (hipStream_t)stream);
}
extern "C" int dvp_msm_ctx_run(dvp_msm_ctx* c, const uint64_t* scalars, size_t lo, size_t hi, uint64_t out_xy[8], int* out_is_infinity) {
  if (!c || !scalars || !out_xy || !out_is_infinity || lo > hi || hi > c->n) return DVP_EINVAL;
  DevBuf ds, dout;
  DVP_TRY(ds.alloc((hi - lo) * 32));
  DVP_TRY(dout.alloc(80));
  if (hi > lo) DVP_HIP(hipMemcpy(ds.p, scalars, (hi - lo) * 32, hipMemcpyHostToDevice));
  DVP_TRY(msm_fixed_dev(c->fx, ds.p, c->d_inf + lo, (uint32_t)lo, (uint32_t)hi, dout.p, (char*)dout.p + 64, 0));
  uint32_t inf;
  DVP_HIP(hipMemcpy(out_xy, dout.p, 64, hipMemcpyDeviceToHost));
  DVP_HIP(hipMemcpy(&inf, (char*)dout.p + 64, 4, hipMemcpyDeviceToHost));
  *out_is_infinity = (int)inf;
  return DVP_OK;
}
```

### include/dvpari_internal.h

```cpp
#ifndef DVPARI_INTERNAL_H
#define DVPARI_INTERNAL_H

#include "dvpari.h"

#ifdef __cplusplus
extern "C" {
#endif

int dvp_tune_set(const char* name, long long value);
int dvp_tune_get(const char* name, long long* value);
void dvp_tune_reset(void);

void dvp_profile_enable(int on);
void dvp_profile_reset(void);
int dvp_profile_read(const char* name, double* total_ms, uint64_t* launches);
int dvp_profile_round0_shapes(uint64_t* pairs, double* total_ms, uint64_t* launches, int cap);

int dvp_ubench_gf_mul(int reps, double* products_per_s);
int dvp_ubench_fr_mul(int reps, double* muladds_per_s);
int dvp_debug_wave_trace(void* d_buf, uint32_t n_records);
int dvp_ubench_gather(const void* d_table, size_t table_bytes, int reps, double* gathers_per_s);
int dvp_prover_msm_table_ptr(const dvp_prover* p, int which, const void** d_table, uint64_t* bytes);

int dvp_debug_recode_signed(const uint64_t* scalars, size_t n, int c_bits, uint32_t* out_words, int* windows);

int dvp_setup_scalars(const uint64_t tau[4], const uint64_t delta[4], const uint64_t epsilon[4], uint32_t log2_m, uint32_t n_public,
                      uint32_t n_rows, uint32_t n_wires, const uint64_t* coeffs, uint32_t n_coeffs, const uint32_t* const row_ptr[3],
                      const uint32_t* const wire_ids[3], const uint32_t* const coeff_ids[3], uint64_t* out_scalars, size_t out_cap);

int dvp_setup_cache_dir_ex(const uint64_t tau[4], const uint64_t delta[4], const uint64_t epsilon[4], const char* cache_dir,
                           uint32_t n_public, int write_precomputes, uint64_t* out_scalars, size_t out_cap, uint32_t* out_n_wires,
                           uint32_t* out_log2_m);

int dvp_prover_debug_transcript_dev(dvp_prover* p, const uint8_t commit_p[30], const uint64_t* public_inputs, uint32_t n_public,
                                    uint64_t out_alpha[4], uint64_t out_neg_z_alpha[4]);

int dvp_prover_debug_read(dvp_prover* p, const char* name, uint64_t* out, size_t n_elems);

int dvp_debug_ecfft_matrices(dvp_ecfft* ctx, int to_even, int which, uint64_t* out);
int dvp_debug_ecfft_layer(const dvp_ecfft* ctx, uint32_t d, uint64_t* out);

#ifdef __cplusplus
}
#endif
#endif
```

Baseline: 56.02 million constraints/s.

## Compact affine round descriptors so odd leftovers are copied instead of occupying slots

Adds a compact descriptor mode, on by default, for affine bucket-reduction rounds after the first. Each descriptor now carries an explicit (input, output) pair, and odd-count leftover points go into a tail list. The round kernel copies those leftovers directly, so the batched-inversion slots cover only real pairs. This is meant to cut wasted slot work, prefix storage and thread count per round, at the cost of doubled descriptor size and scattered output writes. A debug entry point for inspecting the round plan is also added.

```diff
diff --git a/dv-pari_amd/_native.py b/dv-pari_amd/_native.py
--- a/dv-pari_amd/_native.py
+++ b/dv-pari_amd/_native.py
@@ -71,6 +71,8 @@
     "dvp_msm_ctx_plan": (C.c_int, [vp, C.POINTER(C.c_int), C.POINTER(C.c_int)]),
     "dvp_msm_ctx_table_bytes": (C.c_uint64, [vp, C.POINTER(C.c_int)]),
     "dvp_debug_recode_signed": (C.c_int, [vp, C.c_size_t, C.c_int, vp, C.POINTER(C.c_int)]),
+    "dvp_debug_round_plan": (C.c_int, [vp, C.c_uint32, C.c_int, C.c_int, C.c_int, C.c_uint32, vp, C.c_size_t, C.POINTER(C.c_uint32),
+                                       C.POINTER(C.c_uint32), C.POINTER(C.c_uint32)]),
     "dvp_msm_ctx_run": (C.c_int, [vp, u64p, sz, sz, u64p, C.POINTER(C.c_int)]),
     "dvp_msm_ctx_run_dev": (C.c_int, [vp, vp, sz, sz, vp, vp, vp]),
     "dvp_msm_xsk233": (C.c_int, [u8p, u8p, sz, u8p]),
diff --git a/dv-pari_amd/csrc/capi.cpp b/dv-pari_amd/csrc/capi.cpp
--- a/dv-pari_amd/csrc/capi.cpp
+++ b/dv-pari_amd/csrc/capi.cpp
@@ -64,6 +64,7 @@
   t.msm_aff_min = geti("DVP_MSM_AFF_MIN", t.msm_aff_min);
   t.msm_hex_max = geti("DVP_MSM_HEX_MAX", t.msm_hex_max);
   t.msm_round_pipeline = geti("DVP_MSM_ROUND_PIPELINE", t.msm_round_pipeline);
+  t.msm_round_compact = geti("DVP_MSM_ROUND_COMPACT", t.msm_round_compact);
   t.msm_sort_fused = geti("DVP_MSM_SORT_FUSED", t.msm_sort_fused);
   t.msm_bucket_pairs_max = geti("DVP_MSM_BUCKET_PAIRS_MAX", t.msm_bucket_pairs_max);
   t.msm_aff_bmax = geti("DVP_MSM_AFF_BMAX", t.msm_aff_bmax);
@@ -102,7 +103,7 @@
   dvp::Tune& t = dvp::tune();
   struct { const char* n; long long* v; } tab[] = {
       {"DVP_MSM_C", &t.msm_c}, {"DVP_MSM_K", &t.msm_k}, {"DVP_MSM_FIXED_C", &t.msm_fixed_c}, {"DVP_FX_HI", &t.fx_hi},
-      {"DVP_MSM_PROJ", &t.msm_proj}, {"DVP_MSM_AFF_MIN", &t.msm_aff_min}, {"DVP_MSM_HEX_MAX", &t.msm_hex_max}, {"DVP_MSM_ROUND_PIPELINE", &t.msm_round_pipeline}, {"DVP_MSM_SORT_FUSED", &t.msm_sort_fused}, {"DVP_MSM_BUCKET_PAIRS_MAX", &t.msm_bucket_pairs_max}, {"DVP_MSM_AFF_BMAX", &t.msm_aff_bmax}, {"DVP_MSM_AFF_BMIN", &t.msm_aff_bmin}, {"DVP_ECFFT_RADIX4", &t.ecfft_radix4}, {"DVP_ECFFT_FOLD", &t.ecfft_fold}, {"DVP_MSM_ACCUM_FAST", &t.msm_accum_fast}, {"DVP_MSM_TAIL_GROUPS", &t.msm_tail_groups}, {"DVP_MSM_ACCUM_HEX_MAX", &t.msm_accum_hex_max}, {"DVP_GF_INV_TABS", &t.gf_inv_tabs}, {"DVP_MSM_WS_SLOTS", &t.msm_ws_slots}, {"DVP_MSM_GATE_MIN", &t.msm_gate_min}, {"DVP_MSM_AFF_TPB", &t.msm_aff_tpb}, {"DVP_CACHE_REPLICAS", &t.cache_replicas},
+      {"DVP_MSM_PROJ", &t.msm_proj}, {"DVP_MSM_AFF_MIN", &t.msm_aff_min}, {"DVP_MSM_HEX_MAX", &t.msm_hex_max}, {"DVP_MSM_ROUND_PIPELINE", &t.msm_round_pipeline}, {"DVP_MSM_ROUND_COMPACT", &t.msm_round_compact}, {"DVP_MSM_SORT_FUSED", &t.msm_sort_fused}, {"DVP_MSM_BUCKET_PAIRS_MAX", &t.msm_bucket_pairs_max}, {"DVP_MSM_AFF_BMAX", &t.msm_aff_bmax}, {"DVP_MSM_AFF_BMIN", &t.msm_aff_bmin}, {"DVP_ECFFT_RADIX4", &t.ecfft_radix4}, {"DVP_ECFFT_FOLD", &t.ecfft_fold}, {"DVP_MSM_ACCUM_FAST", &t.msm_accum_fast}, {"DVP_MSM_TAIL_GROUPS", &t.msm_tail_groups}, {"DVP_MSM_ACCUM_HEX_MAX", &t.msm_accum_hex_max}, {"DVP_GF_INV_TABS", &t.gf_inv_tabs}, {"DVP_MSM_WS_SLOTS", &t.msm_ws_slots}, {"DVP_MSM_GATE_MIN", &t.msm_gate_min}, {"DVP_MSM_AFF_TPB", &t.msm_aff_tpb}, {"DVP_CACHE_REPLICAS", &t.cache_replicas},
       {"DVP_MSM_QUAD_MAX", &t.msm_quad_max}, {"DVP_MSM_ACCUM_QUAD_MAX", &t.msm_accum_quad_max}, {"DVP_MSM_FIXED_MIN", &t.msm_fixed_min}, {"DVP_HORNER_MAX_PUB", &t.horner_max_pub}, {"DVP_FR_BI_SHAPE", &t.fr_bi_shape},
       {"DVP_MSM_ALIGNED_SIGNED", &t.msm_aligned_signed}, {"DVP_PROVE_HOST_TRANSCRIPT", &t.prove_host_transcript}};
   for (auto& e : tab)
diff --git a/dv-pari_amd/csrc/common.h b/dv-pari_amd/csrc/common.h
--- a/dv-pari_amd/csrc/common.h
+++ b/dv-pari_amd/csrc/common.h
@@ -82,6 +82,7 @@
   long long msm_bucket_pairs_max = 12;
   long long msm_sort_fused = 1;
   long long msm_round_pipeline = 2;
+  long long msm_round_compact = 1;
   long long msm_hex_max = -1;
   long long msm_quad_max = 0;
   long long msm_fixed_min = 1ll << 16;
diff --git a/dv-pari_amd/csrc/msm.hip b/dv-pari_amd/csrc/msm.hip
--- a/dv-pari_amd/csrc/msm.hip
+++ b/dv-pari_amd/csrc/msm.hip
@@ -1076,7 +1076,13 @@
 struct DescPlan {
   unsigned long long at[40];
 };
-template <int LPK>
+__device__ __forceinline__ void round_desc_compact(uint2* __restrict__ d2, uint32_t pairs_total, uint32_t c, uint32_t o, uint32_t oo, uint32_t lane,
+                                                   uint32_t lpk) {
+  const uint32_t np = c >> 1, q = o - oo;
+  for (uint32_t j = lane; j < np; j += lpk) d2[q + j] = make_uint2(o + 2 * j, oo + j);
+  if ((c & 1u) && lane == np % lpk) d2[pairs_total + (oo - q)] = make_uint2(o + c - 1, oo + np);
+}
+template <int LPK, bool COMPACT>
 __global__ void __launch_bounds__(1024)
 k_round_desc_all(const uint32_t* __restrict__ rp, uint32_t nkeys, int R, DescPlan plan, uint32_t* __restrict__ desc) {
   const uint32_t gid = blockIdx.x * blockDim.x + threadIdx.x;
@@ -1103,12 +1109,17 @@
       if (r >= R) break;
       const uint32_t nout = (cr[q] + 1) >> 1;
       uint32_t* d = desc + plan.at[r];
+      if (COMPACT) {
+        const uint32_t* c = rp + (size_t)(2 * (r - 1)) * stride;
+        round_desc_compact((uint2*)d, c[stride + nkeys] - c[3 * stride + nkeys], cr[q], o[q], oo[q], lane, LPK);
+        continue;
+      }
       for (uint32_t j = lane; j < nout; j += LPK) d[oo[q] + j] = (o[q] + 2 * j) | ((2 * j + 1 < cr[q]) ? DESC_PAIR : 0u);
     }
   }
 }
 
-template <int LPK>
+template <int LPK, bool COMPACT>
 __global__ void __launch_bounds__(256)
 k_round_desc(const uint32_t* __restrict__ cnt, const uint32_t* __restrict__ off, const uint32_t* __restrict__ ooff ,
              uint32_t nkeys, uint32_t* __restrict__ desc) {
@@ -1116,7 +1127,25 @@
   const uint32_t key = gid / LPK, lane = gid % LPK;
   if (key >= nkeys) return;
   const uint32_t c = cnt[key], o = off[key], oo = ooff[key], nout = (c + 1) >> 1;
+  if (COMPACT) {
+    round_desc_compact((uint2*)desc, off[nkeys] - ooff[nkeys], c, o, oo, lane, LPK);
+    return;
+  }
   for (uint32_t j = lane; j < nout; j += LPK) desc[oo + j] = (o + 2 * j) | ((2 * j + 1 < c) ? DESC_PAIR : 0u);
+}
+
+static int launch_round_desc_all(int lpk, bool compact, const uint32_t* rp, uint32_t nk, int R, const DescPlan& plan, uint32_t* desc, hipStream_t s) {
+#define DVP_DESC_ALL(LPK)                                                                                                             \
+  do {                                                                                                                                \
+    if (compact)                                                                                                                      \
+      hipLaunchKernelGGL((k_round_desc_all<LPK, true>), dim3(cdiv((size_t)nk * LPK, 1024)), dim3(1024), 0, s, rp, nk, R, plan, desc);  \
+    else                                                                                                                              \
+      hipLaunchKernelGGL((k_round_desc_all<LPK, false>), dim3(cdiv((size_t)nk * LPK, 1024)), dim3(1024), 0, s, rp, nk, R, plan, desc); \
+  } while (0)
+  if (lpk == 64) DVP_DESC_ALL(64); else if (lpk == 16) DVP_DESC_ALL(16); else DVP_DESC_ALL(4);
+#undef DVP_DESC_ALL
+  DVP_HIP(hipGetLastError());
+  return DVP_OK;
 }
 
 #ifndef AFF_PRIO
@@ -1133,7 +1162,7 @@
   }
 }
 constexpr uint32_t AFF_BMAX = 136;
-__device__ __forceinline__ uint32_t aff_slots_per_thread(uint32_t total, uint32_t cap, uint32_t bmax_bmin) {
+__host__ __device__ __forceinline__ uint32_t aff_slots_per_thread(uint32_t total, uint32_t cap, uint32_t bmax_bmin) {
   const uint32_t bmax = bmax_bmin & 0xffu, bmin = (bmax_bmin >> 8) & 0xffu;
   const uint32_t units = (total + cap - 1) / cap;
   const uint32_t R = (units + bmax - 1) / bmax;
@@ -1144,10 +1173,10 @@
   unsigned long long* buf;
   uint32_t cap, tag;
 };
-template <bool FIRST, bool TRACE = false>
+template <bool FIRST, bool TRACE = false, bool COMPACT = false>
 __global__ void __launch_bounds__(EC_TPB) __attribute__((amdgpu_waves_per_eu(3, 3)))
 k_affine_round(const Aff* __restrict__ pts, const uint2* __restrict__ desc, const uint32_t* __restrict__ total_ptr ,
-               uint32_t cap, uint32_t bmax, GfSqrTables T, Gf* __restrict__ prefix, Aff* __restrict__ out, uint32_t sign_mask, WaveTrace wt) {
+               const uint32_t* __restrict__ in_total_ptr , uint32_t cap, uint32_t bmax, GfSqrTables T, Gf* __restrict__ prefix, Aff* __restrict__ out, uint32_t sign_mask, WaveTrace wt) {
   extern __shared__ char lds_raw[];
   unsigned long long tr_t0 = 0, tr_c0 = 0, tr_t1 = 0, tr_t2 = 0;
   if (TRACE) { tr_t0 = wall_clock64(); tr_c0 = clock64(); }
@@ -1162,10 +1191,22 @@
     if (v & sm) y = gf_add(y, x);
     return y;
   };
-  const uint32_t total = *total_ptr;
+  static_assert(!(FIRST && COMPACT), "the first round reads the sorted items as its descriptors");
+  const uint32_t tid = blockIdx.x * blockDim.x + threadIdx.x;
+  uint32_t total = *total_ptr;
+  if (COMPACT) {
+    const uint32_t n_out = total, n_in = *in_total_ptr;
+    total = n_in - n_out;
+    const uint4* src = (const uint4*)pts;
+    uint4* dst = (uint4*)out;
+    for (uint32_t i = tid; i < n_out - total; i += gridDim.x * blockDim.x) {
+      const uint2 l = desc[total + i];
+      const uint4 v0 = src[4 * (size_t)l.x], v1 = src[4 * (size_t)l.x + 1], v2 = src[4 * (size_t)l.x + 2], v3 = src[4 * (size_t)l.x + 3];
+      dst[4 * (size_t)l.y] = v0; dst[4 * (size_t)l.y + 1] = v1; dst[4 * (size_t)l.y + 2] = v2; dst[4 * (size_t)l.y + 3] = v3;
+    }
+  }
   const int B = (int)aff_slots_per_thread(total, cap, bmax);
   const uint32_t nthr = (total + B - 1) / B;
-  const uint32_t tid = blockIdx.x * blockDim.x + threadIdx.x;
   if (tid >= nthr) return;
   const uint2 none = make_uint2(AFF_NONE, AFF_NONE);
   auto ld_desc = [&](int k) -> uint2 {
@@ -1176,15 +1217,20 @@
       if (ok) v = desc[sk];
       return v;
     }
+    if (COMPACT) {
+      const uint32_t a = desc[ok ? sk : 0u].x;
+      return make_uint2(ok ? a : AFF_NONE, AFF_NONE);
+    }
     const uint32_t d = ((const uint32_t*)desc)[ok ? sk : 0u], a = d & ~DESC_PAIR;
     return make_uint2(ok ? a : AFF_NONE, (ok && (d & DESC_PAIR)) ? a + 1 : AFF_NONE);
   };
+  auto dq = [&](const uint2& d) -> uint32_t { return COMPACT ? (d.x != AFF_NONE ? d.x + 1 : AFF_NONE) : d.y; };
   const Gf one = gf_one();
   Gf run = one;
   {
     uint2 d0 = ld_desc(0), d1 = ld_desc(1);
     Gf xa = gf_zero(), xb = gf_zero();
-    if (d0.y != AFF_NONE) { xa = ldx(d0.x); xb = ldx(d0.y); }
+    if (dq(d0) != AFF_NONE) { xa = ldx(d0.x); xb = ldx(dq(d0)); }
 #pragma unroll 1
     for (int k = 0; k < B; ++k) {
 #if AFF_PRIO
@@ -1192,12 +1238,12 @@
 #endif
       const uint2 d2 = ld_desc(k + 2);
       Gf nxa = gf_zero(), nxb = gf_zero();
-      if (d1.y != AFF_NONE) { nxa = ldx(d1.x); nxb = ldx(d1.y); }
+      if (dq(d1) != AFF_NONE) { nxa = ldx(d1.x); nxb = ldx(dq(d1)); }
       Gf den = one;
-      if (d0.y != AFF_NONE && !gf_is_zero(xa) && !gf_is_zero(xb)) {
+      if (dq(d0) != AFF_NONE && !gf_is_zero(xa) && !gf_is_zero(xb)) {
         Gf dd = gf_add(xa, xb);
         if (!gf_is_zero(dd)) den = dd;
-        else if (gf_eq(ldy(d0.x, xa), ldy(d0.y, xb))) den = xa;
+        else if (gf_eq(ldy(d0.x, xa), ldy(dq(d0), xb))) den = xa;
       }
       prefix[(size_t)k * nthr + tid] = run;
       run = gf_mul(run, den, L);
@@ -1211,11 +1257,11 @@
     uint2 e0 = ld_desc(B - 1), e1 = ld_desc(B - 2);
     Gf px = gf_zero(), qx = gf_zero(), pre = one;
     if (e0.x != AFF_NONE) px = ldx(e0.x);
-    if (e0.y != AFF_NONE) { qx = ldx(e0.y); pre = prefix[(size_t)(B - 1) * nthr + tid]; }
+    if (dq(e0) != AFF_NONE) { qx = ldx(dq(e0)); pre = prefix[(size_t)(B - 1) * nthr + tid]; }
 #if AFF_XY
     Gf py = gf_zero(), qy = gf_zero();
     if (e0.x != AFF_NONE) py = ldy(e0.x, px);
-    if (e0.y != AFF_NONE) qy = ldy(e0.y, qx);
+    if (dq(e0) != AFF_NONE) qy = ldy(dq(e0), qx);
 #endif
 #pragma unroll 1
     for (int k = B - 1; k >= 0; --k) {
@@ -1223,22 +1269,24 @@
       aff_set_prio(wslot + (uint32_t)k);
 #endif
       const uint2 e2 = ld_desc(k - 2);
+      uint32_t oidx = 0;
+      if (COMPACT) oidx = desc[e0.x != AFF_NONE ? (uint32_t)k * nthr + tid : 0u].y;
 #if AFF_XY
       Gf npx = gf_zero(), nqx = gf_zero(), npy = gf_zero(), nqy = gf_zero(), npre = one;
       if (e1.x != AFF_NONE) { npx = ldx(e1.x); npy = ldy(e1.x, npx); }
-      if (e1.y != AFF_NONE) { nqx = ldx(e1.y); nqy = ldy(e1.y, nqx); npre = prefix[(size_t)(k - 1) * nthr + tid]; }
+      if (dq(e1) != AFF_NONE) { nqx = ldx(dq(e1)); nqy = ldy(dq(e1), nqx); npre = prefix[(size_t)(k - 1) * nthr + tid]; }
 #else
       Gf py = gf_zero(), qy = gf_zero();
       if (e0.x != AFF_NONE) py = ldy(e0.x, px);
-      if (e0.y != AFF_NONE) qy = ldy(e0.y, qx);
+      if (dq(e0) != AFF_NONE) qy = ldy(dq(e0), qx);
       Gf npx = gf_zero(), nqx = gf_zero(), npre = one;
       if (e1.x != AFF_NONE) npx = ldx(e1.x);
-      if (e1.y != AFF_NONE) { nqx = ldx(e1.y); npre = prefix[(size_t)(k - 1) * nthr + tid]; }
+      if (dq(e1) != AFF_NONE) { nqx = ldx(dq(e1)); npre = prefix[(size_t)(k - 1) * nthr + tid]; }
 #endif
       if (e0.x != AFF_NONE) {
-        const uint32_t sidx = (uint32_t)k * nthr + tid;
+        const uint32_t sidx = COMPACT ? oidx : (uint32_t)k * nthr + tid;
         Gf ox = px, oy = py;
-        if (e0.y != AFF_NONE) {
+        if (dq(e0) != AFF_NONE) {
           if (gf_is_zero(px)) { ox = qx; oy = qy; }
           else if (!gf_is_zero(qx)) {
             Gf dd = gf_add(px, qx);
@@ -1754,7 +1802,8 @@
                           (const void*)k_accum_affine_fast<false, true>, (const void*)k_accum_affine_rest<true>, (const void*)k_accum_affine_rest<false>,
                           (const void*)k_tail_groups, (const void*)k_merge<1, false>, (const void*)k_merge<4, false>, (const void*)k_merge<16, false>, (const void*)k_merge<1, true>, (const void*)k_merge<4, true>, (const void*)k_merge<16, true>,
                           (const void*)k_affine_round<true, false>, (const void*)k_affine_round<false, false>, (const void*)k_affine_round<true, true>,
-                          (const void*)k_affine_round<false, true>, (const void*)k_sum_points, (const void*)k_tail<false>, (const void*)k_tail<true>,
+                          (const void*)k_affine_round<false, true>, (const void*)k_affine_round<false, false, true>,
+                          (const void*)k_affine_round<false, true, true>, (const void*)k_sum_points, (const void*)k_tail<false>, (const void*)k_tail<true>,
                           (const void*)k_bucket_pairs, (const void*)k_bucket_rest};
       for (const void* f : ec)
         if (attr_err == hipSuccess) attr_err = hipFuncSetAttribute(f, hipFuncAttributeMaxDynamicSharedMemorySize, EC_LDS_Q);
@@ -1821,12 +1870,14 @@
   const bool pipelined = affine_mode && tn.msm_round_pipeline != 0 && ra_plan >= 2 && e_est >= 4 * (size_t)p.nkeys;
   const bool side_stream = pipelined && tn.msm_round_pipeline == 1;
   std::vector<size_t> desc_at((size_t)ra_plan + 1, 0);
-  size_t desc_n = affA_n + 64;
+  const bool compact = tn.msm_round_compact != 0;
+  const size_t desc_w = compact ? 2 : 1;
+  size_t desc_n = desc_w * (affA_n + 64);
   if (pipelined) {
     size_t cap_r = p.e_max + p.nkeys, at = 0;
     for (int r = 0; r < ra_plan; ++r) {
       const size_t out_max = cap_r / 2 + p.nkeys + 1;
-      if (r >= 1) { desc_at[r] = at; at += out_max + 64; }
+      if (r >= 1) { desc_at[r] = at; at += desc_w * (out_max + 64); }
       cap_r = out_max;
     }
     if (at > desc_n) desc_n = at;
@@ -1878,7 +1929,13 @@
   auto bookkeep = [&](int r, const uint32_t* ic, const uint32_t* io, uint32_t* oc, uint32_t* oo, uint32_t* dsc, hipStream_t s, uint32_t* bs) -> int {
     DVP_TRY(scan_exclusive_div(ic, 2u, oc, oo, nk, bs, s));
     const size_t per_key = (e_est >> (r + 1)) / nk;
-#define DVP_DESC_LAUNCH(LPK) hipLaunchKernelGGL((k_round_desc<LPK>), dim3(cdiv((size_t)nk * LPK, 256)), dim3(256), 0, s, ic, io, oo, nk, dsc)
+#define DVP_DESC_LAUNCH(LPK)                                                                                                      \
+  do {                                                                                                                            \
+    if (compact)                                                                                                                  \
+      hipLaunchKernelGGL((k_round_desc<LPK, true>), dim3(cdiv((size_t)nk * LPK, 256)), dim3(256), 0, s, ic, io, oo, nk, dsc);     \
+    else                                                                                                                          \
+      hipLaunchKernelGGL((k_round_desc<LPK, false>), dim3(cdiv((size_t)nk * LPK, 256)), dim3(256), 0, s, ic, io, oo, nk, dsc);    \
+  } while (0)
     if (per_key >= 48) DVP_DESC_LAUNCH(64); else if (per_key >= 8) DVP_DESC_LAUNCH(16); else DVP_DESC_LAUNCH(4);
 #undef DVP_DESC_LAUNCH
     return DVP_OK;
@@ -1914,12 +1971,7 @@
     DescPlan plan;
     for (int q = 0; q < 40; ++q) plan.at[q] = q < ra_plan ? desc_at[q] : 0;
     const size_t per_key = (e_est >> 2) / nk;
-    if (per_key >= 48)
-      hipLaunchKernelGGL((k_round_desc_all<64>), dim3(cdiv((size_t)nk * 64, 1024)), dim3(1024), 0, bk, rp, nk, ra_plan, plan, gdesc);
-    else if (per_key >= 8)
-      hipLaunchKernelGGL((k_round_desc_all<16>), dim3(cdiv((size_t)nk * 16, 1024)), dim3(1024), 0, bk, rp, nk, ra_plan, plan, gdesc);
-    else
-      hipLaunchKernelGGL((k_round_desc_all<4>), dim3(cdiv((size_t)nk * 4, 1024)), dim3(1024), 0, bk, rp, nk, ra_plan, plan, gdesc);
+    DVP_TRY(launch_round_desc_all(per_key >= 48 ? 64 : per_key >= 8 ? 16 : 4, compact, rp, nk, ra_plan, plan, gdesc, bk));
     if (side_stream) DVP_HIP(hipEventRecord(g_ws.ev_side[0], g_ws.side));
     DVP_HIP(hipGetLastError());
     prepared = ra_plan;
@@ -2013,22 +2065,26 @@
   uint32_t wt_cap = 0;
   wave_trace_snapshot(&wt_buf, &wt_cap);
   const bool wt_on = wt_buf != nullptr;
-  auto launch_round = [&](int r, const uint32_t* d_total, const uint2* dsc) -> int {
+  auto launch_round = [&](int r, const uint32_t* d_total, const uint32_t* d_in_total, const uint2* dsc) -> int {
     size_t out_max = cap / 2 + nk + 1;
     Aff* outp = (r & 1) ? affB : affA;
-    const uint32_t r_max = cdiv(cdiv(out_max, aff_cap), aff_bmax_only);
+    const uint32_t r_max = cdiv(cdiv(compact && r > 0 ? cap / 2 + 1 : out_max, aff_cap), aff_bmax_only);
     const uint32_t grid = r_max * (aff_cap / aff_tpb) + 1;
     {
       ProfScope ps0(r == 0 ? PROF_MSM_ACCUM_AFFINE : -1, st, (uint64_t)n);
       WaveTrace wt{wt_buf, wt_cap, g_wave_trace_tag.fetch_add(wt_on ? 1u : 0u)};
       if (r == 0 && wt.buf)
-        hipLaunchKernelGGL((k_affine_round<true, true>), dim3(grid), dim3(aff_tpb), aff_lds, st, pts_in, dsc, d_total, aff_cap, aff_bmax, Tsq, prefix, outp, sign_mask, wt);
+        hipLaunchKernelGGL((k_affine_round<true, true>), dim3(grid), dim3(aff_tpb), aff_lds, st, pts_in, dsc, d_total, d_in_total, aff_cap, aff_bmax, Tsq, prefix, outp, sign_mask, wt);
       else if (r == 0)
-        hipLaunchKernelGGL((k_affine_round<true, false>), dim3(grid), dim3(aff_tpb), aff_lds, st, pts_in, dsc, d_total, aff_cap, aff_bmax, Tsq, prefix, outp, sign_mask, wt);
+        hipLaunchKernelGGL((k_affine_round<true, false>), dim3(grid), dim3(aff_tpb), aff_lds, st, pts_in, dsc, d_total, d_in_total, aff_cap, aff_bmax, Tsq, prefix, outp, sign_mask, wt);
+      else if (compact && wt.buf)
+        hipLaunchKernelGGL((k_affine_round<false, true, true>), dim3(grid), dim3(aff_tpb), aff_lds, st, pts_in, dsc, d_total, d_in_total, aff_cap, aff_bmax, Tsq, prefix, outp, 0u, wt);
+      else if (compact)
+        hipLaunchKernelGGL((k_affine_round<false, false, true>), dim3(grid), dim3(aff_tpb), aff_lds, st, pts_in, dsc, d_total, d_in_total, aff_cap, aff_bmax, Tsq, prefix, outp, 0u, wt);
       else if (wt.buf)
-        hipLaunchKernelGGL((k_affine_round<false, true>), dim3(grid), dim3(aff_tpb), aff_lds, st, pts_in, dsc, d_total, aff_cap, aff_bmax, Tsq, prefix, outp, 0u, wt);
+        hipLaunchKernelGGL((k_affine_round<false, true>), dim3(grid), dim3(aff_tpb), aff_lds, st, pts_in, dsc, d_total, d_in_total, aff_cap, aff_bmax, Tsq, prefix, outp, 0u, wt);
       else
-        hipLaunchKernelGGL((k_affine_round<false, false>), dim3(grid), dim3(aff_tpb), aff_lds, st, pts_in, dsc, d_total, aff_cap, aff_bmax, Tsq, prefix, outp, 0u, wt);
+        hipLaunchKernelGGL((k_affine_round<false, false>), dim3(grid), dim3(aff_tpb), aff_lds, st, pts_in, dsc, d_total, d_in_total, aff_cap, aff_bmax, Tsq, prefix, outp, 0u, wt);
       ps0.stop();
     }
     pts_in = outp;
@@ -2038,7 +2094,7 @@
   auto run_round = [&](int r) -> int {
     if (pipelined) {
       if (r == 0 && side_stream) DVP_HIP(hipStreamWaitEvent(st, g_ws.ev_side[0], 0));
-      DVP_TRY(launch_round(r, ro(r + 1) + nk, r == 0 ? (const uint2*)items : (const uint2*)(const void*)(gdesc + desc_at[r])));
+      DVP_TRY(launch_round(r, ro(r + 1) + nk, ro(r) + nk, r == 0 ? (const uint2*)items : (const uint2*)(const void*)(gdesc + desc_at[r])));
       return DVP_OK;
     }
     const int nxt = (cur + 1) % 3;
@@ -2047,7 +2103,7 @@
         hipLaunchKernelGGL(k_round0_offsets, dim3(cdiv(nk + 1, 256)), dim3(256), 0, st, pc[cur], po[cur], nk, pc[nxt], po[nxt]);
     } else
       DVP_TRY(bookkeep(r, pc[cur], po[cur], pc[nxt], po[nxt], gdesc, st, bsum));
-    DVP_TRY(launch_round(r, po[nxt] + nk, r == 0 ? (const uint2*)items : (const uint2*)(const void*)gdesc));
+    DVP_TRY(launch_round(r, po[nxt] + nk, po[cur] + nk, r == 0 ? (const uint2*)items : (const uint2*)(const void*)gdesc));
     cur = nxt;
     return DVP_OK;
   };
@@ -2456,6 +2512,63 @@
   return DVP_OK;
 }
 
+extern "C" int dvp_debug_round_plan(const uint32_t* counts, uint32_t nkeys, int round, int flavour, int compact, uint32_t cap, uint32_t* out_words,
+                                    size_t out_cap, uint32_t* n_slots, uint32_t* n_left, uint32_t* slots_per_thread) {
+  if (!counts || !nkeys || nkeys > (1u << 22) || round < 1 || round > 30 || flavour < 0 || flavour > 1 || !cap || !n_slots || !n_left || !slots_per_thread)
+    return DVP_EINVAL;
+  size_t entries = 0;
+  for (uint32_t k = 0; k < nkeys; ++k) entries += counts[k];
+  if (entries >= ((size_t)1 << 28)) return DVP_EINVAL;
+  const int R = round + 1;
+  const size_t stride = (size_t)nkeys + 1, desc_w = compact ? 2 : 1, area = desc_w * (entries / 2 + stride + 64);
+  const uint32_t nb = cdiv(nkeys, SCAN_BLK);
+  DevBuf dc, drp, dbs, dd;
+  DVP_TRY(dc.alloc(stride * 4));
+  DVP_TRY(drp.alloc((size_t)R * 2 * stride * 4));
+  DVP_TRY(dbs.alloc(((size_t)(R + 1) * nb + 8) * 4));
+  DVP_TRY(dd.alloc((flavour == 0 ? (size_t)R : 1) * area * 4));
+  DVP_HIP(hipMemcpy(dc.p, counts, (size_t)nkeys * 4, hipMemcpyHostToDevice));
+  uint32_t* rp = drp.as<uint32_t>();
+  const uint32_t* o_in = rp + (size_t)(2 * (round - 1) + 1) * stride;
+  const uint32_t* desc = dd.as<uint32_t>();
+  if (flavour == 0) {
+    hipLaunchKernelGGL(k_mscan_local, dim3(nb), dim3(SCAN_TPB), 0, 0, dc.as<uint32_t>(), nkeys, R, rp, dbs.as<uint32_t>());
+    hipLaunchKernelGGL(k_mscan_bsums, dim3(R), dim3(SCAN_TPB), 0, 0, dbs.as<uint32_t>(), nb, nkeys, rp, (uint32_t*)nullptr, (uint32_t*)nullptr);
+    hipLaunchKernelGGL(k_mscan_add, dim3(nb), dim3(SCAN_TPB), 0, 0, rp, dbs.as<uint32_t>(), nkeys, R, dc.as<uint32_t>(), (uint32_t*)nullptr, (uint32_t*)nullptr);
+    DescPlan plan;
+    for (int q = 0; q < 40; ++q) plan.at[q] = q < R ? (size_t)q * area : 0;
+    DVP_TRY(launch_round_desc_all(4, compact != 0, rp, nkeys, R, plan, dd.as<uint32_t>(), 0));
+    desc += plan.at[round];
+  } else {
+    const uint32_t* ic = dc.as<uint32_t>();
+    for (int r = 1; r <= R; ++r) {
+      uint32_t* c = rp + (size_t)(2 * (r - 1)) * stride;
+      DVP_TRY(scan_exclusive_div(ic, 2u, c, c + stride, nkeys, dbs.as<uint32_t>(), 0));
+      ic = c;
+    }
+    const uint32_t* c = rp + (size_t)(2 * (round - 1)) * stride;
+    if (compact)
+      hipLaunchKernelGGL((k_round_desc<4, true>), dim3(cdiv((size_t)nkeys * 4, 256)), dim3(256), 0, 0, c, c + stride, c + 3 * stride, nkeys, dd.as<uint32_t>());
+    else
+      hipLaunchKernelGGL((k_round_desc<4, false>), dim3(cdiv((size_t)nkeys * 4, 256)), dim3(256), 0, 0, c, c + stride, c + 3 * stride, nkeys, dd.as<uint32_t>());
+  }
+  DVP_HIP(hipGetLastError());
+  uint32_t n_in = 0, n_out = 0;
+  DVP_HIP(hipMemcpy(&n_in, o_in + nkeys, 4, hipMemcpyDeviceToHost));
+  DVP_HIP(hipMemcpy(&n_out, o_in + 2 * stride + nkeys, 4, hipMemcpyDeviceToHost));
+  *n_slots = compact ? n_in - n_out : n_out;
+  *n_left = compact ? 2 * n_out - n_in : 0;
+  const Tune tn = tune();
+  const uint32_t bmax = tn.msm_aff_bmax >= 1 && tn.msm_aff_bmax <= 255 ? (uint32_t)tn.msm_aff_bmax : AFF_BMAX;
+  const uint32_t bmin = tn.msm_aff_bmin >= 1 && (uint32_t)tn.msm_aff_bmin <= bmax ? (uint32_t)tn.msm_aff_bmin : 1u;
+  *slots_per_thread = aff_slots_per_thread(*n_slots, cap, bmax | (bmin << 8));
+  if (!out_words) return DVP_OK;
+  const size_t words = desc_w * ((size_t)*n_slots + *n_left);
+  if (words > out_cap) return DVP_EINVAL;
+  if (words) DVP_HIP(hipMemcpy(out_words, desc, words * 4, hipMemcpyDeviceToHost));
+  return DVP_OK;
+}
+
 extern "C" int dvp_msm_affine(const uint64_t* scalars, const uint64_t* bases_xy, const uint8_t* bases_inf, size_t n,
                               uint64_t out_xy[8], int* out_is_infinity) {
   if ((n && (!scalars || !bases_xy)) || !out_xy || !out_is_infinity) return DVP_EINVAL;
diff --git a/include/dvpari_internal.h b/include/dvpari_internal.h
--- a/include/dvpari_internal.h
+++ b/include/dvpari_internal.h
@@ -24,6 +24,9 @@
 
 int dvp_debug_recode_signed(const uint64_t* scalars, size_t n, int c_bits, uint32_t* out_words, int* windows);
 
+int dvp_debug_round_plan(const uint32_t* counts, uint32_t nkeys, int round, int flavour, int compact, uint32_t cap, uint32_t* out_words,
+                         size_t out_cap, uint32_t* n_slots, uint32_t* n_left, uint32_t* slots_per_thread);
+
 int dvp_setup_scalars(const uint64_t tau[4], const uint64_t delta[4], const uint64_t epsilon[4], uint32_t log2_m, uint32_t n_public,
                       uint32_t n_rows, uint32_t n_wires, const uint64_t* coeffs, uint32_t n_coeffs, const uint32_t* const row_ptr[3],
                       const uint32_t* const wire_ids[3], const uint32_t* const coeff_ids[3], uint64_t* out_scalars, size_t out_cap);
```

Result: no change. 56.10 million constraints/s, median of 5 (+0.1%).
